# yester31/Monocular_Depth_Estimation_TRT

Measured on AMD Instinct MI355X. Metric: depth FPS (images/s) at 518x518 fp16, DA-V2 ViT-S, MI355X, higher is better.
Workload: dtype fp16; 1 GPU; Depth Anything V2 vits 518x518 metric head, forward, batch 48 per GPU, inputs resident in HBM, hipGraph replay; encoder=vits, batch_per_gpu=48, global_batch=48, parallelism=replica x1 (batch shards, no collectives), weights=synthetic seeded (seed 1234), fan-in scaled, physical_gpus=1

## Files before the change

### include/mde.h

```cpp
#ifndef MDE_H_
#define MDE_H_

#include <stddef.h>
#include <stdint.h>

#ifdef __cplusplus
extern "C" {
#endif

#define MDE_ABI_VERSION 11

typedef enum {
  MDE_OK = 0,
  MDE_ERR_ARG = 1,
  MDE_ERR_FILE = 2,
  MDE_ERR_FORMAT = 3,
  MDE_ERR_HIP = 4,
  MDE_ERR_NAME = 5,
  MDE_ERR_SHAPE = 6,
  MDE_ERR_STATE = 7
} mde_status;

typedef enum { MDE_FLOAT32 = 0, MDE_FLOAT16 = 1, MDE_UINT8 = 5 } mde_dtype;

typedef struct mde_engine mde_engine;
typedef struct mde_context mde_context;

typedef struct {
  char name[64];
  int32_t dtype;
  int32_t is_input;
  int32_t rank;
  int64_t dims[8];
} mde_io_desc;

typedef struct {
  char encoder[16];
  int32_t embed_dim, depth, num_heads, mlp_hidden, patch;
  int32_t img_h, img_w, features, head_hidden, metric;
  int32_t out_channels[4], taps[4];
  float max_depth, ln_eps;
  int32_t max_batch_hint;
  int64_t weight_bytes;
  int32_t input_format;
  int32_t family;
} mde_engine_info;

typedef void (*mde_layer_cb)(const char* layer_name, float ms, void* user);

int mde_version(void);
const char* mde_last_error(void);
int mde_tuning_set(const char* name, int value);
int mde_tuning_get(const char* name, int* value);
int mde_debug_last_gemm_route(char* buf, size_t n);

int mde_engine_load(const char* packed_path, int device, mde_engine** out);
int mde_engine_load_memory(const void* data, size_t nbytes, int device, mde_engine** out);
int mde_engine_destroy(mde_engine* eng);
int mde_engine_get_info(const mde_engine* eng, mde_engine_info* out);
int mde_engine_num_io(const mde_engine* eng, int* n);
int mde_engine_io_desc(const mde_engine* eng, int index, mde_io_desc* out);
int mde_engine_profile_shape(const mde_engine* eng, const char* name, int which, int64_t* dims, int* rank);

int mde_context_create(mde_engine* eng, int max_batch, mde_context** out);
int mde_context_destroy(mde_context* ctx);
int mde_context_set_tensor_address(mde_context* ctx, const char* name, void* device_ptr);
int mde_context_set_input_shape(mde_context* ctx, const char* name, const int64_t* dims, int rank);
int mde_context_get_tensor_shape(const mde_context* ctx, const char* name, int64_t* dims, int* rank);
int mde_context_enqueue(mde_context* ctx, void* stream);
int mde_context_set_graph_mode(mde_context* ctx, int enable);
int mde_context_set_profiler(mde_context* ctx, mde_layer_cb cb, void* user);
int mde_context_workspace_bytes(const mde_context* ctx, size_t* bytes);

int mde_rt_device_count(int* n);
int mde_rt_set_device(int device);
int mde_rt_device_name(int device, char* buf, int buflen);
int mde_rt_malloc(void** ptr, size_t bytes);
int mde_rt_free(void* ptr);
int mde_rt_malloc_host(void** ptr, size_t bytes);
int mde_rt_free_host(void* ptr);
int mde_rt_memcpy_htod_async(void* dst, const void* src, size_t bytes, void* stream);
int mde_rt_memcpy_dtoh_async(void* dst, const void* src, size_t bytes, void* stream);
int mde_rt_memcpy_dtod_async(void* dst, const void* src, size_t bytes, void* stream);
int mde_rt_memset_async(void* dst, int value, size_t bytes, void* stream);
int mde_rt_stream_create(void** stream);
int mde_rt_stream_destroy(void* stream);
int mde_rt_stream_synchronize(void* stream);
int mde_rt_device_synchronize(void);
int mde_rt_event_create(void** event);
int mde_rt_event_destroy(void* event);
int mde_rt_event_record(void* event, void* stream);
int mde_rt_event_elapsed_ms(float* ms, void* start, void* end);

int mde_op_layernorm_f16(const void* x_f16, void* y_f16, const float* gamma, const float* beta, int rows, int dim,
                         float eps, int tokens, int skip_cls, void* stream);
int mde_op_layernorm(const float* x, void* y_f16, const float* gamma, const float* beta, int rows, int dim,
                     float eps, int tokens, int skip_cls, void* stream);
int mde_op_linear(const void* a_f16, int lda, const void* w_f16, int ldw, int m, int n, int k,
                  const float* bias, int act, void* out_f16, int ldo, void* stream);
int mde_op_linear_residual(const void* a_f16, int lda, const void* w_f16, int ldw, int m, int n, int k,
                           const float* bias, const float* layer_scale, float* x32, int ldx, void* stream);
int mde_op_qkv(const void* a_f16, const void* w_f16, int ldw, const float* bias, int batch, int tokens,
               int heads, int tokens_pad, float q_scale, void* q_f16, void* k_f16, void* vt_f16, void* stream);
int mde_op_linear_residual_f16(const void* a_f16, int lda, const void* w_f16, int ldw, int m, int n, int k,
                               const float* bias, const float* layer_scale, void* xh_f16, int ldx, float* ln_partials,
                               void* stream);
int mde_op_linear_lnfold(const void* x_f16, const float* ln_partials, float eps, const void* wg_f16, int ldw,
                         const float* c1, const float* c2, int m, int n, int k, int act, void* out_f16, int ldo,
                         void* stream);
int mde_op_qkv_lnfold(const void* x_f16, const float* ln_partials, float eps, const void* wg_f16, int ldw,
                      const float* c1, const float* c2, int batch, int tokens, int heads, int tokens_pad,
                      float q_scale, void* q_f16, void* k_f16, void* vt_f16, void* stream);
int mde_op_attention(const void* q_f16, const void* k_f16, const void* vt_f16, void* o_f16, int batch, int heads,
                     int tokens, int tokens_pad, int ldo, void* stream);
int mde_op_attention_ws(const void* q_f16, const void* k_f16, const void* vt_f16, void* o_f16, int batch, int heads,
                        int tokens, int tokens_pad, int ldo, void* ws, size_t ws_bytes, void* stream);
size_t mde_op_attention_ws_bytes(int batch, int heads, int tokens);
int mde_op_attention_cfg(const void* q_f16, const void* k_f16, const void* vt_f16, void* o_f16, int batch, int heads,
                         int tokens, int tokens_pad, int ldo, const char* cfg, void* ws, size_t ws_bytes,
                         void* stream);
int mde_op_linear32(const float* a, int lda, const float* w, int ldw, int m, int n, int k, const float* bias, int act,
                    float* out, int ldo, void* stream);
int mde_op_linear_residual32(const float* a, int lda, const float* w, int ldw, int m, int n, int k,
                             const float* bias, const float* layer_scale, float* x32, int ldx, void* stream);
int mde_op_qkv32(const float* a, const float* w, int ldw, const float* bias, int batch, int tokens, int heads,
                 int tokens_pad, float q_scale, float* q, float* k, float* v, void* stream);
int mde_op_attention32(const float* q, const float* k, const float* v, float* o, int batch, int heads, int tokens,
                       int tokens_pad, int ldo, void* stream);
int mde_op_conv3x3_32(const float* in, int batch, int h, int w, int cin, const float* wt, int ldw, int cout,
                      int stride, int relu_in, const float* bias, int act, const float* res0, const float* res1,
                      float* out, void* stream);
int mde_op_conv_transpose32(const float* in, int batch, int h, int w, int cin, const float* wt, int ldw, int cout,
                            int stride, const float* bias, float* out, void* stream);
int mde_op_resize32(const float* in, int batch, int h, int w, int c, int oh, int ow, float* out, void* stream);
int mde_op_patch_embed(const float* img, int batch, int h, int w, const void* w_f16, int ldw, const float* bias,
                       const float* pos_patch, const float* cls_pos, int dim, void* patch_scratch_f16,
                       float* x32, void* stream);
int mde_op_conv3x3(const void* in_f16, int batch, int h, int w, int cin, const void* w_f16, int ldw, int cout,
                   int stride, int relu_in, const float* bias, int act, const void* res0_f16,
                   const void* res1_f16, void* out_f16, void* stream);
int mde_op_conv3x3_ws(const void* in_f16, int batch, int h, int w, int cin, const void* w_f16, int ldw, int cout,
                      int stride, int relu_in, const float* bias, int act, const void* res0_f16,
                      const void* res1_f16, void* out_f16, float* ws, size_t ws_floats, int* slices, void* stream);
int mde_op_linear_ws(const void* a_f16, int lda, const void* w_f16, int ldw, int m, int n, int k, const float* bias,
                     int act, void* out_f16, int ldo, float* ws, size_t ws_floats, int* slices, void* stream);
int mde_op_conv3x3_up(const void* in_f16, int batch, int sh, int sw, int cin, int uh, int uw, const void* w_f16,
                      int ldw, int cout, const float* bias, int act, void* out_f16, void* stream);
int mde_op_conv_transpose(const void* in_f16, int batch, int h, int w, int cin, const void* w_f16, int ldw,
                          int cout, int stride, const float* bias, void* out_f16, void* stream);
int mde_op_resize_bilinear(const void* in_f16, int batch, int ih, int iw, int c, int oh, int ow, void* out_f16,
                           void* stream);
int mde_op_depth_head(const void* in_f16, int batch, int sh, int sw, int cin, int uh, int uw, const void* w_f16,
                      int ldw, const float* bias, const float* w2, float b2, int metric, float max_depth,
                      float* out_f32, void* stream);
int mde_op_linear_res(const void* a_f16, int lda, const void* w_f16, int ldw, int m, int n, int k, const float* bias,
                      int act, const void* res0_f16, int res0_rows, int res0_relu, const void* res1_f16,
                      void* out_f16, int ldo, float* ws, size_t ws_floats, int* slices, int* tile_cnt,
                      int tile_cnt_cap, size_t slot_floats, void* stream);
int mde_op_conv3x3_res(const void* in_f16, int batch, int h, int w, int cin, const void* w_f16, int ldw, int cout,
                       int stride, int relu_in, const float* bias, int act, const void* res0_f16, int res0_relu,
                       const void* res1_f16, const void* res1_up_f16, int res1_uh, int res1_uw, void* out_f16,
                       float* ws, size_t ws_floats, int* slices, int* tile_cnt, int tile_cnt_cap, size_t slot_floats,
                       void* stream);
int mde_op_linear_lnfold_tok(const void* x_f16, const float* ln_partials, float eps, const void* wg_f16, int ldw,
                             const float* c1, const float* c2, int seqs, int tokens, int n, int k, int act,
                             void* out_f16, int ldo, void* stream);
int mde_op_depth_head_pe(const void* in_f16, int batch, int sh, int sw, int cin, int uh, int uw, const void* w_f16,
                         int ldw, const float* bias, const float* w2, float b2, int metric, float max_depth,
                         const void* hpe_f16, int hpe_pix, float* out_f32, void* stream);
int mde_op_conv_transpose_ld(const void* in_f16, int batch, int h, int w, int cin, const void* w_f16, int ldw,
                             int cout, int stride, const float* bias, void* out_f16, int ldo, void* stream);
int mde_op_linear_residual_split(const void* a_f16, int lda, const void* w_f16, int ldw, int m, int n, int k,
                                 const float* bias, const float* layer_scale, float* x32, void* xh_f16, int ldx,
                                 float* ln_partials, int splitk, float* ws, size_t ws_floats, int* tile_cnt,
                                 int tile_cnt_cap, size_t slot_floats, void* stream);
int mde_op_patch_prep_u8(const unsigned char* img_u8, int batch, int h, int w, float scale, const float* mean3,
                         const float* std3, void* patches_f16, void* stream);
int mde_op_depth_postprocess(const float* depth, int batch, int ih, int iw, float* out, int oh, int ow, float lo,
                             float hi, void* stream);
int mde_op_resize_u8(const unsigned char* src, int batch, int sh, int sw, int pitch, int swap_rb,
                     unsigned char* dst_u8, int oh, int ow, void* stream);
int mde_op_resize_u8_norm(const unsigned char* src, int batch, int sh, int sw, int pitch, int swap_rb,
                          const float* lut3x256, float* dst_f32_nchw, int oh, int ow, void* stream);
int mde_op_dp_preprocess(const unsigned char* src, int batch, int sh, int sw, int pitch, int swap_rb,
                         const float* lut256, float* dst_f32_nchw, int oh, int ow, void* stream);
int mde_op_dp_postprocess(const float* inv, int batch, int ih, int iw, const float* fov_deg, float f_px,
                          float* f_px_out, float* depth, int oh, int ow, void* stream);
size_t mde_op_point_cloud_ws_bytes(int batch, int h, int w, int step);
int mde_op_point_cloud(const float* depth, int batch, int h, int w, int step, const unsigned char* photo, int pitch,
                       int swap_rb, const float* f_px_dev, float fx, float fy, float cx, float cy, int compact,
                       float z_lo, float z_hi, void* records, size_t records_bytes, int* counts, void* ws,
                       size_t ws_bytes, void* stream);
#define MDE_DEPTH_EVAL_TILE 1024
size_t mde_op_depth_eval_ws_bytes(int batch, int h, int w);
int mde_op_depth_eval(const float* pred, const float* gt, const unsigned char* mask, int batch, int h, int w,
                      int policy, int pred_is_inverse, int fit_finite_only, float max_depth, double* out, void* ws,
                      size_t ws_bytes, void* stream);
int mde_op_dp_pyramid_patches(const float* img, int batch, int size, void* patches_f16, void* stream);
int mde_op_merge_tokens(const float* x32, int batch, int tokens, int dim, int n, int g, int pad, int base,
                        const float* gamma, const float* beta, float eps, void* out_f16, void* stream);
int mde_op_qk_norm_rope(void* q_f16, void* k_f16, const float* q_gamma, const float* q_beta, const float* k_gamma,
                        const float* k_beta, int bh, int tokens, int tokens_pad, int frame_tokens, int npre,
                        int grid_w, const float* rope_cos, const float* rope_sin, float q_scale, float eps,
                        void* stream);
int mde_op_tap_concat_ln(const float* xa, const float* xb, int nseq, int tokens, int npre, int dim,
                         const float* gamma, const float* beta, float eps, void* out_f16, void* stream);
#ifdef __cplusplus
}
#endif

#endif
```

### monocular_depth_estimation_trt_amd/_lib.py

```python

from __future__ import annotations

import contextlib
import ctypes as C
import os
import threading

HERE = os.path.dirname(os.path.abspath(__file__))
LIB_PATH = os.path.join(HERE, "libmde_hip.so")


def use_library(path: str) -> None:
    global LIB_PATH
    if _lib is not None and os.path.abspath(path) != os.path.abspath(LIB_PATH):
        raise RuntimeError(f"libmde_hip already loaded from {LIB_PATH}")
    LIB_PATH = path

c_void_p, c_int, c_float, c_size_t, c_char_p = C.c_void_p, C.c_int, C.c_float, C.c_size_t, C.c_char_p
c_int64 = C.c_int64
P = C.POINTER

MDE_OK = 0
STATUS = {1: "MDE_ERR_ARG", 2: "MDE_ERR_FILE", 3: "MDE_ERR_FORMAT", 4: "MDE_ERR_HIP", 5: "MDE_ERR_NAME",
          6: "MDE_ERR_SHAPE", 7: "MDE_ERR_STATE"}


class mde_io_desc(C.Structure):
    _fields_ = [("name", C.c_char * 64), ("dtype", C.c_int32), ("is_input", C.c_int32),
                ("rank", C.c_int32), ("dims", C.c_int64 * 8)]


class mde_engine_info(C.Structure):
    _fields_ = [("encoder", C.c_char * 16),
                ("embed_dim", C.c_int32), ("depth", C.c_int32), ("num_heads", C.c_int32),
                ("mlp_hidden", C.c_int32), ("patch", C.c_int32),
                ("img_h", C.c_int32), ("img_w", C.c_int32), ("features", C.c_int32),
                ("head_hidden", C.c_int32), ("metric", C.c_int32),
                ("out_channels", C.c_int32 * 4), ("taps", C.c_int32 * 4),
                ("max_depth", C.c_float), ("ln_eps", C.c_float),
                ("max_batch_hint", C.c_int32), ("weight_bytes", C.c_int64),
                ("input_format", C.c_int32), ("family", C.c_int32)]


LAYER_CB = C.CFUNCTYPE(None, c_char_p, c_float, c_void_p)

PROTOTYPES = {
    "mde_version": [],
    "mde_last_error": [],
    "mde_tuning_set": [c_char_p, c_int],
    "mde_tuning_get": [c_char_p, P(c_int)],
    "mde_debug_last_gemm_route": [c_char_p, c_size_t],
    "mde_engine_load": [c_char_p, c_int, P(c_void_p)],
    "mde_engine_load_memory": [c_void_p, c_size_t, c_int, P(c_void_p)],
    "mde_engine_destroy": [c_void_p],
    "mde_engine_get_info": [c_void_p, P(mde_engine_info)],
    "mde_engine_num_io": [c_void_p, P(c_int)],
    "mde_engine_io_desc": [c_void_p, c_int, P(mde_io_desc)],
    "mde_engine_profile_shape": [c_void_p, c_char_p, c_int, P(c_int64), P(c_int)],
    "mde_context_create": [c_void_p, c_int, P(c_void_p)],
    "mde_context_destroy": [c_void_p],
    "mde_context_set_tensor_address": [c_void_p, c_char_p, c_void_p],
    "mde_context_set_input_shape": [c_void_p, c_char_p, P(c_int64), c_int],
    "mde_context_get_tensor_shape": [c_void_p, c_char_p, P(c_int64), P(c_int)],
    "mde_context_enqueue": [c_void_p, c_void_p],
    "mde_context_set_graph_mode": [c_void_p, c_int],
    "mde_context_set_profiler": [c_void_p, LAYER_CB, c_void_p],
    "mde_context_workspace_bytes": [c_void_p, P(c_size_t)],
    "mde_rt_device_count": [P(c_int)],
    "mde_rt_set_device": [c_int],
    "mde_rt_device_name": [c_int, c_char_p, c_int],
    "mde_rt_malloc": [P(c_void_p), c_size_t],
    "mde_rt_free": [c_void_p],
    "mde_rt_malloc_host": [P(c_void_p), c_size_t],
    "mde_rt_free_host": [c_void_p],
    "mde_rt_memcpy_htod_async": [c_void_p, c_void_p, c_size_t, c_void_p],
    "mde_rt_memcpy_dtoh_async": [c_void_p, c_void_p, c_size_t, c_void_p],
    "mde_rt_memcpy_dtod_async": [c_void_p, c_void_p, c_size_t, c_void_p],
    "mde_rt_memset_async": [c_void_p, c_int, c_size_t, c_void_p],
    "mde_rt_stream_create": [P(c_void_p)],
    "mde_rt_stream_destroy": [c_void_p],
    "mde_rt_stream_synchronize": [c_void_p],
    "mde_rt_device_synchronize": [],
    "mde_rt_event_create": [P(c_void_p)],
    "mde_rt_event_destroy": [c_void_p],
    "mde_rt_event_record": [c_void_p, c_void_p],
    "mde_rt_event_elapsed_ms": [P(c_float), c_void_p, c_void_p],
    "mde_op_layernorm": [c_void_p, c_void_p, c_void_p, c_void_p, c_int, c_int, c_float, c_int, c_int, c_void_p],
    "mde_op_layernorm_f16": [c_void_p, c_void_p, c_void_p, c_void_p, c_int, c_int, c_float, c_int, c_int, c_void_p],
    "mde_op_linear": [c_void_p, c_int, c_void_p, c_int, c_int, c_int, c_int, c_void_p, c_int, c_void_p, c_int,
                      c_void_p],
    "mde_op_linear_residual": [c_void_p, c_int, c_void_p, c_int, c_int, c_int, c_int, c_void_p, c_void_p,
                               c_void_p, c_int, c_void_p],
    "mde_op_qkv": [c_void_p, c_void_p, c_int, c_void_p, c_int, c_int, c_int, c_int, c_float, c_void_p, c_void_p,
                   c_void_p, c_void_p],
    "mde_op_linear_residual_f16": [c_void_p, c_int, c_void_p, c_int, c_int, c_int, c_int, c_void_p, c_void_p,
                                   c_void_p, c_int, c_void_p, c_void_p],
    "mde_op_linear_lnfold": [c_void_p, c_void_p, c_float, c_void_p, c_int, c_void_p, c_void_p, c_int, c_int, c_int,
                             c_int, c_void_p, c_int, c_void_p],
    "mde_op_qkv_lnfold": [c_void_p, c_void_p, c_float, c_void_p, c_int, c_void_p, c_void_p, c_int, c_int, c_int,
                          c_int, c_float, c_void_p, c_void_p, c_void_p, c_void_p],
    "mde_op_attention_ws": [c_void_p, c_void_p, c_void_p, c_void_p, c_int, c_int, c_int, c_int, c_int, c_void_p,
                            c_size_t, c_void_p],
    "mde_op_attention_ws_bytes": [c_int, c_int, c_int],
    "mde_op_attention_cfg": [c_void_p, c_void_p, c_void_p, c_void_p, c_int, c_int, c_int, c_int, c_int, c_char_p,
                             c_void_p, c_size_t, c_void_p],
    "mde_op_attention": [c_void_p, c_void_p, c_void_p, c_void_p, c_int, c_int, c_int, c_int, c_int, c_void_p],
    "mde_op_linear32": [c_void_p, c_int, c_void_p, c_int, c_int, c_int, c_int, c_void_p, c_int, c_void_p, c_int,
                        c_void_p],
    "mde_op_linear_residual32": [c_void_p, c_int, c_void_p, c_int, c_int, c_int, c_int, c_void_p, c_void_p,
                                 c_void_p, c_int, c_void_p],
    "mde_op_qkv32": [c_void_p, c_void_p, c_int, c_void_p, c_int, c_int, c_int, c_int, c_float, c_void_p, c_void_p,
                     c_void_p, c_void_p],
    "mde_op_attention32": [c_void_p, c_void_p, c_void_p, c_void_p, c_int, c_int, c_int, c_int, c_int, c_void_p],
    "mde_op_conv3x3_32": [c_void_p, c_int, c_int, c_int, c_int, c_void_p, c_int, c_int, c_int, c_int, c_void_p,
                          c_int, c_void_p, c_void_p, c_void_p, c_void_p],
    "mde_op_conv_transpose32": [c_void_p, c_int, c_int, c_int, c_int, c_void_p, c_int, c_int, c_int, c_void_p,
                                c_void_p, c_void_p],
    "mde_op_resize32": [c_void_p, c_int, c_int, c_int, c_int, c_int, c_int, c_void_p, c_void_p],
    "mde_op_patch_embed": [c_void_p, c_int, c_int, c_int, c_void_p, c_int, c_void_p, c_void_p, c_void_p, c_int,
                           c_void_p, c_void_p, c_void_p],
    "mde_op_conv3x3": [c_void_p, c_int, c_int, c_int, c_int, c_void_p, c_int, c_int, c_int, c_int, c_void_p,
                       c_int, c_void_p, c_void_p, c_void_p, c_void_p],
    "mde_op_conv3x3_ws": [c_void_p, c_int, c_int, c_int, c_int, c_void_p, c_int, c_int, c_int, c_int, c_void_p,
                          c_int, c_void_p, c_void_p, c_void_p, c_void_p, c_size_t, P(c_int), c_void_p],
    "mde_op_linear_ws": [c_void_p, c_int, c_void_p, c_int, c_int, c_int, c_int, c_void_p, c_int, c_void_p, c_int,
                         c_void_p, c_size_t, P(c_int), c_void_p],
    "mde_op_conv3x3_up": [c_void_p, c_int, c_int, c_int, c_int, c_int, c_int, c_void_p, c_int, c_int, c_void_p,
                          c_int, c_void_p, c_void_p],
    "mde_op_conv_transpose": [c_void_p, c_int, c_int, c_int, c_int, c_void_p, c_int, c_int, c_int, c_void_p,
                              c_void_p, c_void_p],
    "mde_op_resize_bilinear": [c_void_p, c_int, c_int, c_int, c_int, c_int, c_int, c_void_p, c_void_p],
    "mde_op_depth_head": [c_void_p, c_int, c_int, c_int, c_int, c_int, c_int, c_void_p, c_int, c_void_p,
                          c_void_p, c_float, c_int, c_float, c_void_p, c_void_p],
    "mde_op_linear_res": [c_void_p, c_int, c_void_p, c_int, c_int, c_int, c_int, c_void_p, c_int, c_void_p, c_int,
                          c_int, c_void_p, c_void_p, c_int, c_void_p, c_size_t, P(c_int), c_void_p, c_int, c_size_t,
                          c_void_p],
    "mde_op_conv3x3_res": [c_void_p, c_int, c_int, c_int, c_int, c_void_p, c_int, c_int, c_int, c_int, c_void_p,
                           c_int, c_void_p, c_int, c_void_p, c_void_p, c_int, c_int, c_void_p, c_void_p, c_size_t,
                           P(c_int), c_void_p, c_int, c_size_t, c_void_p],
    "mde_op_linear_lnfold_tok": [c_void_p, c_void_p, c_float, c_void_p, c_int, c_void_p, c_void_p, c_int, c_int,
                                 c_int, c_int, c_int, c_void_p, c_int, c_void_p],
    "mde_op_depth_head_pe": [c_void_p, c_int, c_int, c_int, c_int, c_int, c_int, c_void_p, c_int, c_void_p,
                             c_void_p, c_float, c_int, c_float, c_void_p, c_int, c_void_p, c_void_p],
    "mde_op_conv_transpose_ld": [c_void_p, c_int, c_int, c_int, c_int, c_void_p, c_int, c_int, c_int, c_void_p,
                                 c_void_p, c_int, c_void_p],
    "mde_op_linear_residual_split": [c_void_p, c_int, c_void_p, c_int, c_int, c_int, c_int, c_void_p, c_void_p,
                                     c_void_p, c_void_p, c_int, c_void_p, c_int, c_void_p, c_size_t, c_void_p,
                                     c_int, c_size_t, c_void_p],
    "mde_op_patch_prep_u8": [c_void_p, c_int, c_int, c_int, c_float, c_void_p, c_void_p, c_void_p, c_void_p],
    "mde_op_dp_pyramid_patches": [c_void_p, c_int, c_int, c_void_p, c_void_p],
    "mde_op_merge_tokens": [c_void_p, c_int, c_int, c_int, c_int, c_int, c_int, c_int, c_void_p, c_void_p, c_float,
                            c_void_p, c_void_p],
    "mde_op_depth_postprocess": [c_void_p, c_int, c_int, c_int, c_void_p, c_int, c_int, c_float, c_float,
                                 c_void_p],
    "mde_op_resize_u8": [c_void_p, c_int, c_int, c_int, c_int, c_int, c_void_p, c_int, c_int, c_void_p],
    "mde_op_resize_u8_norm": [c_void_p, c_int, c_int, c_int, c_int, c_int, c_void_p, c_void_p, c_int, c_int,
                              c_void_p],
    "mde_op_dp_preprocess": [c_void_p, c_int, c_int, c_int, c_int, c_int, c_void_p, c_void_p, c_int, c_int,
                             c_void_p],
    "mde_op_dp_postprocess": [c_void_p, c_int, c_int, c_int, c_void_p, c_float, c_void_p, c_void_p, c_int, c_int,
                              c_void_p],
    "mde_op_point_cloud_ws_bytes": [c_int, c_int, c_int, c_int],
    "mde_op_point_cloud": [c_void_p, c_int, c_int, c_int, c_int, c_void_p, c_int, c_int, c_void_p, c_float, c_float,
                           c_float, c_float, c_int, c_float, c_float, c_void_p, c_size_t, c_void_p, c_void_p,
                           c_size_t, c_void_p],
    "mde_op_depth_eval_ws_bytes": [c_int, c_int, c_int],
    "mde_op_depth_eval": [c_void_p, c_void_p, c_void_p, c_int, c_int, c_int, c_int, c_int, c_int, c_float, c_void_p,
                          c_void_p, c_size_t, c_void_p],
    "mde_op_qk_norm_rope": [c_void_p] * 6 + [c_int] * 6 + [c_void_p, c_void_p, c_float, c_float, c_void_p],
    "mde_op_tap_concat_ln": [c_void_p, c_void_p, c_int, c_int, c_int, c_int, c_void_p, c_void_p, c_float, c_void_p,
                             c_void_p],
}
_RESTYPE = {"mde_last_error": c_char_p, "mde_op_attention_ws_bytes": c_size_t,
             "mde_op_point_cloud_ws_bytes": c_size_t, "mde_op_depth_eval_ws_bytes": c_size_t}

_lib = None
_lock = threading.Lock()


class MDEError(RuntimeError):

    def __init__(self, fn: str, code: int, msg: str):
        self.code = code
        super().__init__(f"{fn} failed ({STATUS.get(code, code)}): {msg}")


def hip_runtimes() -> list:
    paths = set()
    try:
        with open("/proc/self/maps") as f:
            for line in f:
                parts = line.split(None, 5)
                if len(parts) == 6 and "libamdhip64" in os.path.basename(parts[5].strip()):
                    paths.add(os.path.realpath(parts[5].strip()))
    except OSError:
        return []
    return sorted(paths)


def check_single_runtime() -> None:
    rts = hip_runtimes()
    if len(rts) > 1:
        raise ImportError(
            "two HIP runtimes are loaded in this process (" + ", ".join(rts) + "): libmde_hip.so was loaded "
            "before PyTorch's bundled HIP runtime.  Import torch (and call torch.cuda.is_available()) before "
            "loading libmde_hip.so, or do not load torch in a process that uses libmde_hip.so directly.")


def lib() -> C.CDLL:
    global _lib
    if _lib is not None:
        return _lib
    with _lock:
        if _lib is None:
            if not os.path.exists(LIB_PATH):
                raise ImportError(
                    f"libmde_hip.so not found at {LIB_PATH}. Build it first: "
                    f"python -c 'import __graft_entry__ as g; g.build()' (or "
                    f"python -m monocular_depth_estimation_trt_amd._build). There is no CPU fallback.")
            try:
                import torch
                torch.cuda.is_available()
            except ImportError:
                pass
            L = C.CDLL(LIB_PATH)
            check_single_runtime()
            for name, args in PROTOTYPES.items():
                f = getattr(L, name)
                f.argtypes = args
                f.restype = _RESTYPE.get(name, c_int)
            _lib = L
    return _lib


def last_error() -> str:
    m = lib().mde_last_error()
    return m.decode(errors="replace") if m else ""


def call(name: str, *args) -> None:
    rc = getattr(lib(), name)(*args)
    if rc != MDE_OK:
        raise MDEError(name, rc, last_error())


TUNING = ("splitk", "lnfold", "conv_narrow", "upconv", "gemm256", "deep64", "w8small", "conv_persist", "panel",
          "panel32", "narrow_resid", "attn16", "splitk_fused", "attn_tail", "resize_fold")
TUNING_DEFAULT = {"panel32": 0, "splitk_fused": 0, "attn_tail": 2}


def get_tuning(name: str) -> int:
    v = c_int()
    call("mde_tuning_get", name.encode(), C.byref(v))
    return v.value


def set_tuning(name: str, value: int) -> None:
    rc = lib().mde_tuning_set(name.encode(), int(value))
    if rc != MDE_OK:
        raise ValueError(f"mde_tuning_set({name!r}, {value}) failed ({STATUS.get(rc, rc)}): "
                         f"known switches {TUNING}")


@contextlib.contextmanager
def tuning(**switches):
    old = {k: get_tuning(k) for k in switches}
    try:
        for k, v in switches.items():
            set_tuning(k, v)
        yield
    finally:
        for k, v in old.items():
            set_tuning(k, v)


def last_gemm_route() -> dict:
    buf = C.create_string_buffer(256)
    call("mde_debug_last_gemm_route", buf, len(buf))
    fields = dict(f.split("=", 1) for f in buf.value.decode().split())
    return {k: v if k == "kind" else int(v) for k, v in fields.items()}


def exported_symbols():
    return list(PROTOTYPES)
```

### monocular_depth_estimation_trt_amd/csrc/conv.hip

```cpp
#include <cstdlib>
#include <type_traits>

#include "mde_device.h"
#include "mde_ops.h"
#include "tile_epilogue.h"
#include "tuning.h"

#ifndef MDE_EPI_LDS
#define MDE_EPI_LDS 1
#endif
#ifndef MDE_UP_BLEND_F16
#define MDE_UP_BLEND_F16 1
#endif
#ifndef MDE_CONVP_RELU_PASS
#define MDE_CONVP_RELU_PASS 1
#endif
#ifndef MDE_CONV_BRES
#define MDE_CONV_BRES 2
#endif

namespace mde {

namespace {

__device__ __attribute__((aligned(64))) f16 g_zero_conv[64];

MDE_DEV void glds16c(const void* src, void* lds_wave_base) {
  __builtin_amdgcn_global_load_lds(src, lds_wave_base, 16, 0, 0);
}
MDE_DEV void wait_vmc() { asm volatile("s_waitcnt vmcnt(0)" ::: "memory"); }
MDE_DEV void glds16_asm(const void* src, unsigned lds_dst) {
  unsigned keep;
  asm volatile("s_mov_b32 %0, m0\n\ts_mov_b32 m0, %2\n\ts_nop 0\n\tglobal_load_lds_dwordx4 %1, off\n\ts_mov_b32 m0, %0"
               : "=&s"(keep)
               : "v"(src), "s"(lds_dst)
               : "memory");
}
MDE_DEV void lds_sync() {
  asm volatile("s_waitcnt lgkmcnt(0)" ::: "memory");
  __builtin_amdgcn_s_barrier();
  asm volatile("" ::: "memory");
}

typedef f16 f16x2c __attribute__((ext_vector_type(2)));

template <int J>
MDE_DEV f16x2c lerp2(const f16x8& a, const f16x8& b, f16x2c w2) {
  const f16x2c a2 = __builtin_shufflevector(a, a, 2 * J, 2 * J + 1);
  const f16x2c b2 = __builtin_shufflevector(b, b, 2 * J, 2 * J + 1);
  unsigned dd;
  asm("v_pk_add_f16 %0, %1, %2 neg_lo:[0,1] neg_hi:[0,1]"
      : "=v"(dd)
      : "v"(__builtin_bit_cast(unsigned, b2)), "v"(__builtin_bit_cast(unsigned, a2)));
  return a2 + __builtin_bit_cast(f16x2c, dd) * w2;
}

MDE_DEV f16x8 lerp8(const f16x8& a, const f16x8& b, f16 w) {
  const f16x2c w2 = {w, w};
  const f16x2c r0 = lerp2<0>(a, b, w2), r1 = lerp2<1>(a, b, w2), r2 = lerp2<2>(a, b, w2), r3 = lerp2<3>(a, b, w2);
  return __builtin_shufflevector(__builtin_shufflevector(r0, r1, 0, 1, 2, 3), __builtin_shufflevector(r2, r3, 0, 1, 2, 3),
                                 0, 1, 2, 3, 4, 5, 6, 7);
}

template <int CK>
MDE_DEV int cpch(int pix, int lc) {
  if constexpr (CK == 64) return lc ^ (pix & 7);
  else return lc ^ ((pix >> 1) & 3);
}

constexpr int TH = 8, TW = 16;

template <int BN, int WM, int WN, int CK, int S, bool UP, int EM, bool BRES = false, int TY = TH>
__global__ void __launch_bounds__(WM * WN * 64)
    __attribute__((amdgpu_waves_per_eu((WM * WN == 4 || WM * WN == 8) && !UP ? 4 : 1))) conv3_kernel(const GemmParams p) {
  constexpr int NW = WM * WN, NT = NW * 64;
  constexpr int BM = TY * TW;
  constexpr int TM = BM / (WM * 16), TN = BN / (WN * 16);
  static_assert(TM * WM * 16 == BM && TN * WN * 16 == BN, "tile");
  static_assert(EM != E_HEAD || (BN == 32 && WN == 1), "head epilogue");
  constexpr int ROWB = CK * 2, CH = CK / 8, RWP = 64 / CH;
  constexpr int PH = (TY - 1) * S + 3, PW = (TW - 1) * S + 3, PHW = PH * PW;
  constexpr int PINS = (PHW + RWP - 1) / RWP;
  constexpr int PPAD = PINS * RWP;
  constexpr int PATCH = PPAD * ROWB;
  constexpr int BSTAGE = BN * ROWB;
  constexpr int BINS = BN / RWP;
  static_assert(BINS * RWP == BN, "B tile rows");
  constexpr int MAIN = PATCH + (BRES ? 9 : 2) * BSTAGE, EPI = MDE_EPI_LDS ? BM * BN * 4 : 0;
  __shared__ __attribute__((aligned(16))) char smem[MAIN > EPI ? MAIN : EPI];
  char* sP = smem;
  char* sB0 = smem + PATCH;

  const int tid = threadIdx.x, lane = tid & 63;
  const int wave = __builtin_amdgcn_readfirstlane(tid >> 6);
  const int wm = wave / WN, wn = wave - (wave / WN) * WN;

  const int Ho = p.oh, Wo = p.ow;
  const int tiles_x = (Wo + TW - 1) / TW, tiles_y = (Ho + TY - 1) / TY;
  const int ntn = (p.N + BN - 1) / BN;
  int bid = xcd_remap(blockIdx.x, gridDim.x);
  const int tn = bid % ntn;
  bid /= ntn;
  const int tx = bid % tiles_x;
  bid /= tiles_x;
  const int ty = bid % tiles_y;
  const int b = bid / tiles_y;
  const int n0 = tn * BN;
  const int IH = UP ? p.uh : p.ch, IW = UP ? p.uw : p.cw;
  const int iy0 = ty * TY * S - 1, ix0 = tx * TW * S - 1;
  const f16* img = reinterpret_cast<const f16*>(p.A) + (size_t)b * p.ch * p.cw * p.cc;

  const int lrow = lane / CH;
  const int lch = cpch<CK>(lrow, lane % CH);
  const f16* wbase = reinterpret_cast<const f16*>(p.W) + (size_t)(n0 + lrow) * p.ldw + lch * 8;

  float usy = 0.f, usx = 0.f;
  if constexpr (UP) {
    usy = ac_scale(p.ch, p.uh);
    usx = ac_scale(p.cw, p.uw);
  }

  auto load_patch = [&](int chunk) {
    const int cbase = chunk * CK;
    if constexpr (!UP) {
      for (int q = wave; q < PINS; q += NW) {
        const int pp = q * RWP + lrow;
        const int py = pp / PW, px = pp - (pp / PW) * PW;
        const int iy = iy0 + py, ix = ix0 + px;
        const bool ok = pp < PHW && iy >= 0 && iy < IH && ix >= 0 && ix < IW;
        const f16* src = ok ? img + ((size_t)iy * p.cw + ix) * p.cc + cbase + lch * 8 : g_zero_conv;
        glds16c(src, sP + q * RWP * ROWB);
      }
    } else {
      const unsigned rowstride = (unsigned)p.cw * (unsigned)p.cc;
      constexpr int CG = CH < 4 ? CH : 4, NG = CH / CG;
      for (int it = tid; it < PHW * NG; it += NT) {
        const int pp = it / NG, g0 = (it - (it / NG) * NG) * CG;
        const int py = pp / PW, px = pp - (pp / PW) * PW;
        const int iy = iy0 + py, ix = ix0 + px;
        const bool inside = iy >= 0 && iy < IH && ix >= 0 && ix < IW;
        int y0 = 0, y1 = 0, x0 = 0, x1 = 0;
        float ly0 = 0.f, ly1 = 0.f, lx0 = 0.f, lx1 = 0.f;
        if (inside) {
          ac_index(usy, iy, p.ch, y0, y1, ly0, ly1);
          ac_index(usx, ix, p.cw, x0, x1, lx0, lx1);
        }
        const unsigned r0 = (unsigned)y0 * rowstride + (unsigned)cbase, r1 = (unsigned)y1 * rowstride + (unsigned)cbase;
        const unsigned o0 = (unsigned)x0 * (unsigned)p.cc, o1 = (unsigned)x1 * (unsigned)p.cc;
#pragma unroll
        for (int q = 0; q < CG; ++q) {
          const int lc = g0 + q;
          f16x8 v = zero8();
          if (inside) {
            const f16x8 a = *reinterpret_cast<const f16x8*>(img + (r0 + o0 + lc * 8));
            const f16x8 bq = *reinterpret_cast<const f16x8*>(img + (r0 + o1 + lc * 8));
            const f16x8 c = *reinterpret_cast<const f16x8*>(img + (r1 + o0 + lc * 8));
            const f16x8 d = *reinterpret_cast<const f16x8*>(img + (r1 + o1 + lc * 8));
#if MDE_UP_BLEND_F16
            v = lerp8(lerp8(a, bq, (f16)lx1), lerp8(c, d, (f16)lx1), (f16)ly1);
#else
#pragma unroll
            for (int j = 0; j < 8; ++j)
              v[j] = (f16)(ly0 * (lx0 * (float)a[j] + lx1 * (float)bq[j]) + ly1 * (lx0 * (float)c[j] + lx1 * (float)d[j]));
#endif
          }
          if (p.relu_in) v = relu8(v);
          *reinterpret_cast<f16x8*>(sP + pp * ROWB + cpch<CK>(pp, lc) * 16) = v;
        }
// ... 5 lines not shown
    const int k0 = t * p.cc + chunk * CK;
    char* dst = sB0 + buf * BSTAGE;
    for (int q = wave; q < BINS; q += NW) glds16c(wbase + (size_t)q * RWP * p.ldw + k0, dst + q * RWP * ROWB);
  };

  auto relu_patch = [&] {
    if constexpr (!UP) {
      if (p.relu_in) {
        for (int c = tid; c < PATCH / 16; c += NT) {
          f16x8* q = reinterpret_cast<f16x8*>(sP + c * 16);
          *q = relu8(*q);
        }
      }
    }
  };
  f32x4 acc[TM][TN];
#pragma unroll
  for (int i = 0; i < TM; ++i)
#pragma unroll
    for (int j = 0; j < TN; ++j) acc[i][j] = f32x4{0.f, 0.f, 0.f, 0.f};

  const int nchunk = p.cc / CK;
  const int nsteps = 9 * nchunk;
  if constexpr (BRES) {
    load_patch(0);
#pragma unroll
    for (int t = 0; t < 9; ++t) load_b(t, t);
    wait_vmc();
    __syncthreads();
    if (!UP && p.relu_in) {
      relu_patch();
      __syncthreads();
    }
#pragma unroll
    for (int t = 0; t < 9; ++t) {
      const char* sB = sB0 + t * BSTAGE;
      const int ky = t / 3, kx = t - (t / 3) * 3;
#pragma unroll
      for (int s = 0; s < CK / 32; ++s) {
        const int lc = 4 * s + (lane >> 4);
        f16x8 fa[TM], fb[TN];
#pragma unroll
        for (int i = 0; i < TM; ++i) {
          const int pp = ((wm * TM + i) * S + ky) * PW + (lane & 15) * S + kx;
          fa[i] = *reinterpret_cast<const f16x8*>(sP + pp * ROWB + cpch<CK>(pp, lc) * 16);
        }
#pragma unroll
        for (int j = 0; j < TN; ++j) {
          const int r = wn * TN * 16 + j * 16 + (lane & 15);
          fb[j] = *reinterpret_cast<const f16x8*>(sB + r * ROWB + cpch<CK>(r, lc) * 16);
        }
#pragma unroll
        for (int i = 0; i < TM; ++i)
#pragma unroll
          for (int j = 0; j < TN; ++j) acc[i][j] = mfma16x16x32(fb[j], fa[i], acc[i][j]);
      }
    }
    __syncthreads();
  }
  for (int chunk = 0; chunk < (BRES ? 0 : nchunk); ++chunk) {
    if (chunk > 0) __syncthreads();
    load_patch(chunk);
    const int step0 = chunk * 9;
    load_b(step0, step0 & 1);
    wait_vmc();
    __syncthreads();
    if (!UP && p.relu_in) {
      relu_patch();
      __syncthreads();
    }
    for (int t = 0; t < 9; ++t) {
      const int step = step0 + t;
      if (t + 1 < 9) load_b(step + 1, (step + 1) & 1);
      const char* sB = sB0 + (step & 1) * BSTAGE;
      const int ky = t / 3, kx = t - (t / 3) * 3;
#pragma unroll
      for (int s = 0; s < CK / 32; ++s) {
        const int lc = 4 * s + (lane >> 4);
        f16x8 fa[TM], fb[TN];
#pragma unroll
        for (int i = 0; i < TM; ++i) {
          const int py = wm * TM + i;
          const int pp = (py * S + ky) * PW + (lane & 15) * S + kx;
          fa[i] = *reinterpret_cast<const f16x8*>(sP + pp * ROWB + cpch<CK>(pp, lc) * 16);
        }
#pragma unroll
        for (int j = 0; j < TN; ++j) {
          const int r = wn * TN * 16 + j * 16 + (lane & 15);
          fb[j] = *reinterpret_cast<const f16x8*>(sB + r * ROWB + cpch<CK>(r, lc) * 16);
        }
#pragma unroll
        for (int i = 0; i < TM; ++i)
#pragma unroll
          for (int j = 0; j < TN; ++j) acc[i][j] = mfma16x16x32(fb[j], fa[i], acc[i][j]);
      }
      wait_vmc();
      __syncthreads();
    }
  }
  (void)nsteps;

  int mrow[TM];
#pragma unroll
  for (int i = 0; i < TM; ++i) {
    const int oy = ty * TY + wm * TM + i, ox = tx * TW + (lane & 15);
    mrow[i] = (oy < Ho && ox < Wo) ? ((b * Ho + oy) * Wo + ox) : -1;
  }
#if MDE_EPI_LDS
  if (!store_tile_lds<EM, TM, TN, 0, true>(
          p, acc,
          [&](int row) {
            const int oy = ty * TY + wm * TM + (row >> 4), ox = tx * TW + (row & 15);
            return (oy < Ho && ox < Wo) ? ((b * Ho + oy) * Wo + ox) : -1;
          },
          n0 + wn * TN * 16, lane, smem + wave * (TM * 16) * (TN * 16) * 4))
#endif
    store_tile<EM, TM, TN, true>(p, acc, mrow, n0 + wn * TN * 16 + (lane >> 4) * 4, lane);
}

template <int BN, int WM, int WN, int CK, int S, bool UP, int EM, int TY = TH>
hipError_t run_conv(const GemmParams& p, hipStream_t st) {
  const long long blocks =
      (long long)p.cb * ((p.oh + TY - 1) / TY) * ((p.ow + TW - 1) / TW) * ((p.N + BN - 1) / BN);
  if (blocks <= 0) return hipSuccess;
  constexpr bool BRES_OK = BN == 32 && (CK == 32 ? MDE_CONV_BRES >= 1 : MDE_CONV_BRES >= 2);
  if (BRES_OK && p.cc == CK)
    hipLaunchKernelGGL((conv3_kernel<BN, WM, WN, CK, S, UP, EM, BRES_OK, TY>), dim3((unsigned)blocks),
                       dim3(WM * WN * 64), 0, st, p);
  else
    hipLaunchKernelGGL((conv3_kernel<BN, WM, WN, CK, S, UP, EM, false, TY>), dim3((unsigned)blocks),
                       dim3(WM * WN * 64), 0, st, p);
  return hipGetLastError();
}

bool conv_narrow_tiles() { return knob(KNOB_CONV_NARROW) != 0; }

template <int CK, int S, bool UP, int EM>
hipError_t conv_tiles(const GemmParams& p, hipStream_t st) {
  if constexpr (EM == E_HEAD) {
    return run_conv<32, 4, 1, CK, S, UP, EM>(p, st);
  } else {
    if (p.N <= 32) return run_conv<32, 4, 1, CK, S, UP, EM>(p, st);
    if (p.N <= 64) {
      const long long wg64 = (long long)p.cb * ((p.oh + TH - 1) / TH) * ((p.ow + TW - 1) / TW);
      if (!UP && p.N == 64 && conv_narrow_tiles() && wg64 < 256) return run_conv<32, 4, 1, CK, S, UP, EM>(p, st);
      return run_conv<64, 4, 1, CK, S, UP, EM>(p, st);
    }
    const long long wg128 = (long long)p.cb * ((p.oh + TH - 1) / TH) * ((p.ow + TW - 1) / TW) * ((p.N + 127) / 128);
    if (!UP && conv_narrow_tiles() && wg128 < 512) return run_conv<64, 4, 1, CK, S, UP, EM>(p, st);
    return run_conv<128, 2, 2, CK, S, UP, EM>(p, st);
  }
}

template <int TYP, int MODE>
__global__ void __launch_bounds__(TYP * 32) __attribute__((amdgpu_waves_per_eu(1)))
conv64p_kernel(const GemmParams p) {
  constexpr int NW = TYP / 2, NT = NW * 64, TM = 2, TN = 4;
  constexpr int ROWB = 128, RWP = 8;
  constexpr int PH = TYP + 2, PW = TW + 2, PHW = PH * PW;
  constexpr int PINS = (PHW + RWP - 1) / RWP;
  constexpr int PATCH = PINS * RWP * ROWB;
  constexpr int WOFF = 2 * PATCH;
  constexpr int WB = 9 * 64 * ROWB;
  constexpr int EPIW = 16 * 64 * 4;
  constexpr int NRES = MODE == 3 ? 0 : MODE;
  constexpr bool F16STAGE = MODE == 0 || MODE == 3;
  static_assert(NW * EPIW <= PATCH, "epilogue staging fits the consumed patch buffer");
  static_assert(PATCH + ((TM + 1) * PW + 2) * ROWB < 65536 && 7 * 8192 + 3 * 2048 < 65536, "ds_read immediate offsets");
  static_assert(PW % 8 == 2, "pixel row stride = 2 mod 8 (the swizzle table below)");
  __shared__ __attribute__((aligned(16))) char smem[2 * PATCH + WB];

  const int tid = threadIdx.x, lane = tid & 63;
  const int wave = __builtin_amdgcn_readfirstlane(tid >> 6);
  const int Ho = p.oh, Wo = p.ow;
  const int tiles_x = (Wo + TW - 1) / TW, tiles_y = (Ho + TYP - 1) / TYP;
  const int ntiles = p.cb * tiles_x * tiles_y;
  const int x8 = blockIdx.x & 7, g8 = (int)gridDim.x >> 3;
  int t = (int)((long long)x8 * ntiles / 8) + (int)(blockIdx.x >> 3);
  const int tend = (int)((long long)(x8 + 1) * ntiles / 8);
  if (t >= tend) return;

  const int lrow = lane >> 3;
  const int lch = cpch<64>(lrow, lane & 7);
  const size_t imgsz = (size_t)p.ch * p.cw * 64;

  for (int q = wave; q < 9 * 64 / RWP; q += NW) {
    const int tap = q >> 3, n = (q & 7) * RWP + lrow;
    glds16c(reinterpret_cast<const f16*>(p.W) + (size_t)n * p.ldw + tap * 64 + lch * 8, smem + WOFF + q * RWP * ROWB);
  }
  auto load_patch = [&](int tt, int buf, auto asm_tag) {
    const int tx = tt % tiles_x, r = tt / tiles_x;
    const int ty = r % tiles_y, b = r / tiles_y;
    const int iy0 = ty * TYP - 1, ix0 = tx * TW - 1;
    const f16* img = reinterpret_cast<const f16*>(p.A) + (size_t)b * imgsz;
    char* dst = smem + buf * PATCH;
    for (int q = wave; q < PINS; q += NW) {
      const int pp = q * RWP + lrow;
      const int py = pp / PW, px = pp - (pp / PW) * PW;
      const int iy = iy0 + py, ix = ix0 + px;
      const bool ok = pp < PHW && iy >= 0 && iy < p.ch && ix >= 0 && ix < p.cw;
      const f16* src = ok ? img + ((size_t)iy * p.cw + ix) * 64 + lch * 8 : g_zero_conv;
      if constexpr (decltype(asm_tag)::value)
        glds16_asm(src, __builtin_amdgcn_readfirstlane((unsigned)(uintptr_t)(dst + q * RWP * ROWB)));
      else
        glds16c(src, dst + q * RWP * ROWB);
    }
  };
  auto relu_patch = [&](int buf) {
    for (int c = tid; c < PATCH / 16; c += NT) {
      f16x8* q = reinterpret_cast<f16x8*>(smem + buf * PATCH + c * 16);
      *q = relu8(*q);
    }
  };

  int pa[8][2], wa[2], wa8[2];
  {
    const int u = 2 * wave * TM + (lane & 15);
    const int rowbase = ((wave * TM) * PW + (lane & 15)) * ROWB;
#pragma unroll
    for (int e = 0; e < 8; ++e)
#pragma unroll
      for (int s2 = 0; s2 < 2; ++s2) pa[e][s2] = rowbase + ((((4 * s2 + (lane >> 4)) ^ ((u + e) & 7))) << 4);
#pragma unroll
    for (int s2 = 0; s2 < 2; ++s2) {
      wa[s2] = WOFF + (lane & 15) * ROWB + (((4 * s2 + (lane >> 4)) ^ (lane & 7)) << 4);
      wa8[s2] = wa[s2] + 8 * 64 * ROWB;
    }
  }

  const int rr = lane >> 3, c8 = lane & 7;
  float4 bias[TN];
#pragma unroll
  for (int j = 0; j < TN; ++j)
    bias[j] = p.bias ? *reinterpret_cast<const float4*>(p.bias + j * 16 + (lane >> 4) * 4) : float4{0.f, 0.f, 0.f, 0.f};

  load_patch(t, 0, std::false_type{});
  wait_vmc();
  __syncthreads();
  if constexpr (MODE == 0) {
    if (MDE_CONVP_RELU_PASS) relu_patch(0);
    lds_sync();
  }

  auto step = [&](auto buf_tag) -> bool {
    constexpr int BUF = decltype(buf_tag)::value;
    const int tn = t + g8;
    if (tn < tend) load_patch(tn, BUF ^ 1, std::true_type{});

    const int tx = t % tiles_x, r = t / tiles_x;
    const int ty = r % tiles_y, b = r / tiles_y;
    int mo[4];
#pragma unroll
    for (int it = 0; it < 4; ++it) {
      const int row = it * 8 + rr;
      const int oy = ty * TYP + wave * TM + (row >> 4), ox = tx * TW + (row & 15);
      mo[it] = (oy < Ho && ox < Wo) ? ((b * Ho + oy) * Wo + ox) : -1;
    }
    f16x8 res[NRES > 0 ? NRES : 1][4];
    if constexpr (NRES > 0) {
#pragma unroll
      for (int it = 0; it < 4; ++it) {
        const size_t o = (size_t)(mo[it] < 0 ? 0 : mo[it]) * p.ldo + c8 * 8;
        res[0][it] = *reinterpret_cast<const f16x8*>(reinterpret_cast<const f16*>(p.res0) + o);
        if constexpr (NRES > 1) res[1][it] = *reinterpret_cast<const f16x8*>(reinterpret_cast<const f16*>(p.res1) + o);
      }
    }
    __builtin_amdgcn_sched_barrier(0);

    f32x4 acc[TM][TN];
#pragma unroll
    for (int i = 0; i < TM; ++i)
#pragma unroll
      for (int j = 0; j < TN; ++j) acc[i][j] = f32x4{0.f, 0.f, 0.f, 0.f};
#pragma unroll
    for (int tap = 0; tap < 9; ++tap) {
      const int ky = tap / 3, kx = tap - (tap / 3) * 3;
#pragma unroll
      for (int s2 = 0; s2 < 2; ++s2) {
        f16x8 fa[TM], fb[TN];
#pragma unroll
        for (int i = 0; i < TM; ++i) {
          const int e = 2 * (i + ky) + kx;
          fa[i] = *reinterpret_cast<const f16x8*>(smem + pa[e & 7][s2] + (BUF * PATCH + ((i + ky) * PW + kx) * ROWB));
          if constexpr (MODE == 0 && !MDE_CONVP_RELU_PASS) fa[i] = relu8(fa[i]);
        }
#pragma unroll
        for (int j = 0; j < TN; ++j)
          fb[j] = *reinterpret_cast<const f16x8*>(smem + (tap < 8 ? wa[s2] + tap * 64 * ROWB : wa8[s2]) + j * 16 * ROWB);
#pragma unroll
        for (int i = 0; i < TM; ++i)
#pragma unroll
          for (int j = 0; j < TN; ++j) acc[i][j] = mfma16x16x32(fb[j], fa[i], acc[i][j]);
      }
    }
    __builtin_amdgcn_sched_barrier(0);
    wait_vmc();
    lds_sync();
    if constexpr (MODE == 0) {
      if (MDE_CONVP_RELU_PASS && tn < tend) relu_patch(BUF ^ 1);
    }

    char* stage = smem + BUF * PATCH + wave * EPIW;
    f16* const out = reinterpret_cast<f16*>(p.out16);
    if constexpr (F16STAGE) {
#pragma unroll
      for (int i = 0; i < TM; ++i)
#pragma unroll
        for (int j = 0; j < TN; ++j) {
          const float4 bn = bias[j];
          const float v0 = acc[i][j][0] + bn.x, v1 = acc[i][j][1] + bn.y;
          const float v2 = acc[i][j][2] + bn.z, v3 = acc[i][j][3] + bn.w;
          const f16x4 h = MODE == 0 ? f16x4{(f16)(v0 > 0.f ? v0 : 0.f), (f16)(v1 > 0.f ? v1 : 0.f),
                                            (f16)(v2 > 0.f ? v2 : 0.f), (f16)(v3 > 0.f ? v3 : 0.f)}
                                    : f16x4{(f16)v0, (f16)v1, (f16)v2, (f16)v3};
          const int row = i * 16 + (lane & 15), q = j * 4 + (lane >> 4);
          *reinterpret_cast<f16x4*>(stage + row * 128 + ((((q >> 1) ^ (row & 7)) << 4) | ((q & 1) << 3))) = h;
        }
      asm volatile("s_waitcnt lgkmcnt(0)" ::: "memory");
      __builtin_amdgcn_wave_barrier();
#pragma unroll
      for (int it = 0; it < 4; ++it) {
        const int row = it * 8 + rr;
        const f16x8 h = *reinterpret_cast<const f16x8*>(stage + row * 128 + ((c8 ^ (row & 7)) << 4));
        if (mo[it] >= 0) *reinterpret_cast<f16x8*>(out + (size_t)mo[it] * p.ldo + c8 * 8) = h;
      }
    } else {
#pragma unroll
      for (int i = 0; i < TM; ++i) {
        if (i > 0) __builtin_amdgcn_wave_barrier();
#pragma unroll
        for (int j = 0; j < TN; ++j) {
          const float4 bn = bias[j];
          const f32x4 v = {acc[i][j][0] + bn.x, acc[i][j][1] + bn.y, acc[i][j][2] + bn.z, acc[i][j][3] + bn.w};
          const int row = lane & 15, q = j * 4 + (lane >> 4);
          *reinterpret_cast<f32x4*>(stage + row * 256 + ((q ^ (row & 7)) << 4)) = v;
        }
        asm volatile("s_waitcnt lgkmcnt(0)" ::: "memory");
        __builtin_amdgcn_wave_barrier();
#pragma unroll
        for (int h2 = 0; h2 < 2; ++h2) {
          const int it = i * 2 + h2, row = h2 * 8 + rr;
          const f32x4 a = *reinterpret_cast<const f32x4*>(stage + row * 256 + (((2 * c8) ^ (row & 7)) << 4));
          const f32x4 bb = *reinterpret_cast<const f32x4*>(stage + row * 256 + (((2 * c8 + 1) ^ (row & 7)) << 4));
          float v[8] = {a[0], a[1], a[2], a[3], bb[0], bb[1], bb[2], bb[3]};
          const f16x8 r0 = res[0][it];
          if (p.res0_relu) {
#pragma unroll
            for (int e = 0; e < 8; ++e) v[e] += fmaxf((float)r0[e], 0.f);
          } else {
#pragma unroll
            for (int e = 0; e < 8; ++e) v[e] += (float)r0[e];
          }
          if constexpr (NRES > 1) {
            const f16x8 r1 = res[NRES - 1][it];
#pragma unroll
            for (int e = 0; e < 8; ++e) v[e] += (float)r1[e];
          }
          f16x8 h;
#pragma unroll
          for (int e = 0; e < 8; ++e) h[e] = (f16)v[e];
          if (mo[it] >= 0) *reinterpret_cast<f16x8*>(out + (size_t)mo[it] * p.ldo + c8 * 8) = h;
        }
      }
    }
    if (tn >= tend) return true;
    lds_sync();
    t = tn;
    return false;
  };
  for (;;) {
    if (step(std::integral_constant<int, 0>{})) break;
    if (step(std::integral_constant<int, 1>{})) break;
  }
}

int conv64p_mode(const GemmParams& p) {
  const int mode = knob(KNOB_CONV_PERSIST);
  if (!mode || p.amode != A_CONV3 || p.emode != E_STORE || p.stride != 1 || p.N != 64 || p.cc != 64 ||
      p.ch != p.oh || p.cw != p.ow || p.ldo < 64 || (p.ldo & 7) || p.res0_rows > 0)
    return -1;
  const bool r1 = p.res1 || p.res1_up;
  int m;
  if (p.relu_in && p.act == ACT_RELU && !p.res0 && !r1) m = 0;
  else if (!p.relu_in && p.act == ACT_NONE && !p.res0 && !r1) m = 3;
  else if (!p.relu_in && p.act == ACT_NONE && p.res0) m = r1 ? 2 : 1;
  else return -1;
  const int typ = mode == 2 ? 8 : 16;
  const long long tiles = (long long)p.cb * ((p.oh + typ - 1) / typ) * ((p.ow + TW - 1) / TW);
  if (tiles < 4 * 256 || tiles >= (1ll << 31)) return -1;
  return m;
}

bool conv64p_launch(const GemmParams& p, hipStream_t st, hipError_t& err) {
  const int m = conv64p_mode(p);
  if (m < 0) return false;
  const int typ = knob(KNOB_CONV_PERSIST) == 2 ? 8 : 16;
  const dim3 grid(256), block(typ * 32);
  if (typ == 16) {
    if (m == 0) hipLaunchKernelGGL((conv64p_kernel<16, 0>), grid, block, 0, st, p);
    else if (m == 1) hipLaunchKernelGGL((conv64p_kernel<16, 1>), grid, block, 0, st, p);
    else if (m == 2) hipLaunchKernelGGL((conv64p_kernel<16, 2>), grid, block, 0, st, p);
    else hipLaunchKernelGGL((conv64p_kernel<16, 3>), grid, block, 0, st, p);
  } else {
    if (m == 0) hipLaunchKernelGGL((conv64p_kernel<8, 0>), grid, block, 0, st, p);
    else if (m == 1) hipLaunchKernelGGL((conv64p_kernel<8, 1>), grid, block, 0, st, p);
    else if (m == 2) hipLaunchKernelGGL((conv64p_kernel<8, 2>), grid, block, 0, st, p);
    else hipLaunchKernelGGL((conv64p_kernel<8, 3>), grid, block, 0, st, p);
  }
  err = hipGetLastError();
  return true;
}

constexpr int UTH = 16, UTW = 16;
constexpr int UPH = UTH + 2, UPW = UTW + 2;
constexpr int USR = 12;
constexpr int UPATCH = UPH * UPW * 64, UHBUF = USR * UPW * 64;
MDE_DEV int uoff(int row, int col, int lc) { return row * (UPW * 64) + col * 64 + ((lc ^ ((col >> 1) & 3)) << 4); }

template <int NCH, int EM, bool PERSIST>
__global__ void __launch_bounds__(512) __attribute__((amdgpu_waves_per_eu(NCH == 1 ? 6 : 4)))
upconv_kernel(const GemmParams p) {
  static_assert(EM == E_STORE || EM == E_HEAD, "upconv epilogues");
  constexpr int NT = 512, TM = 2, TN = 2;
  constexpr bool SW = NCH > 1;
  constexpr int WROWS = 9 * (SW ? 1 : NCH) * 32;
  __shared__ __attribute__((aligned(16))) char smem[UPATCH + UHBUF + WROWS * 64 + 256];
  char* const sP = smem;
  char* const sH = smem + UPATCH;
  char* const sW = sH + UHBUF;
  float* const sBias = reinterpret_cast<float*>(sW + WROWS * 64);

  const int tid = threadIdx.x, lane = tid & 63;
  const int wave = __builtin_amdgcn_readfirstlane(tid >> 6);
  const int Ho = p.oh, Wo = p.ow;
  const int tiles_x = (Wo + UTW - 1) / UTW, tiles_y = (Ho + UTH - 1) / UTH;
  const int ntiles = p.cb * tiles_x * tiles_y;
  int t, tstep, tend;
  if constexpr (PERSIST) {
    const int x = blockIdx.x & 7, g8 = (int)gridDim.x >> 3;
    t = (int)((long long)x * ntiles / 8) + (int)(blockIdx.x >> 3);
    tend = (int)((long long)(x + 1) * ntiles / 8);
    tstep = g8;
  } else {
    t = xcd_remap(blockIdx.x, gridDim.x);
    tend = t + 1;
    tstep = 1;
  }
  if (t >= tend) return;
  const float usy = ac_scale(p.ch, p.uh), usx = ac_scale(p.cw, p.uw);
  const unsigned rowstride = (unsigned)p.cw * (unsigned)p.cc;

  if constexpr (!SW) {
    const int lrow = lane >> 2, lch = cpch<32>(lrow, lane & 3);
    for (int q = wave; q < WROWS / 16; q += 8) {
      const int tc = q >> 1, n = (q & 1) * 16 + lrow;
      const int tp = tc / NCH, c = tc - (tc / NCH) * NCH;
      glds16c(reinterpret_cast<const f16*>(p.W) + (size_t)n * p.ldw + tp * p.cc + c * 32 + lch * 8, sW + q * 16 * 64);
    }
  }

  if (tid < 64) {
    const float* src = tid < 32 ? p.bias : p.w2;
    sBias[tid] = (src && (tid < 32 || EM == E_HEAD)) ? src[tid & 31] : 0.f;
  }

  struct Geo {
    int b, ty, tx, iy0, ix0, sy0, nsr;
  };
  auto geo = [&](int tt) {
    Geo g;
    g.tx = tt % tiles_x;
    const int r = tt / tiles_x;
    g.ty = r % tiles_y;
    g.b = r / tiles_y;
    g.iy0 = g.ty * UTH - 1;
    g.ix0 = g.tx * UTW - 1;
    int a0, a1, b0, b1;
    float l0, l1;
    ac_index(usy, g.iy0 < 0 ? 0 : g.iy0, p.ch, a0, a1, l0, l1);
    const int last = g.iy0 + UPH - 1 < p.uh - 1 ? g.iy0 + UPH - 1 : p.uh - 1;
    ac_index(usy, last, p.ch, b0, b1, l0, l1);
    g.sy0 = a0;
    g.nsr = b1 - a0 + 1 < USR ? b1 - a0 + 1 : USR;
    return g;
  };

  constexpr int CL = UPW * 4, RG = NT / CL;
  static_assert(RG * 2 >= USR && RG * 3 >= UPH, "row groups cover the H rows (2 each) and the patch rows (3)");
  constexpr int HI = 2;
  f16x8 ha[HI], hb[HI];
  f16 hw = (f16)0.0f;
  bool hs[HI], hin = false;
  auto h_issue = [&](const Geo& g, int c, int tid) {
    const f16* img = reinterpret_cast<const f16*>(p.A) + (size_t)g.b * p.ch * p.cw * p.cc;
    const int cl = tid % CL, rg = tid / CL;
    const int lc = cl & 3, col = cl >> 2;
    const int ix = g.ix0 + col;
    hin = rg < RG && ix >= 0 && ix < p.uw;
    int x0 = 0, x1 = 0;
    float lx0, lx1 = 0.f;
    if (hin) ac_index(usx, ix, p.cw, x0, x1, lx0, lx1);
    hw = (f16)lx1;
    const unsigned o0 = (unsigned)x0 * (unsigned)p.cc + (unsigned)(c * 32 + lc * 8);
    const unsigned o1 = (unsigned)x1 * (unsigned)p.cc + (unsigned)(c * 32 + lc * 8);
#pragma unroll
    for (int k = 0; k < HI; ++k) {
      const int sr = rg + k * RG;
      hs[k] = rg < RG && sr < g.nsr;
      const unsigned r = (unsigned)(g.sy0 + (hin && hs[k] ? sr : 0)) * rowstride;
      ha[k] = *reinterpret_cast<const f16x8*>(img + (r + o0));
      hb[k] = *reinterpret_cast<const f16x8*>(img + (r + o1));
    }
  };
  auto h_commit = [&](int tid) {
    const int cl = tid % CL, rg = tid / CL;
    const int lc = cl & 3, col = cl >> 2;
#pragma unroll
    for (int k = 0; k < HI; ++k) {
      if (hs[k]) {
        *reinterpret_cast<f16x8*>(sH + uoff(rg + k * RG, col, lc)) =
            hin ? lerp8(ha[k], hb[k], hw) : zero8();
      }
    }
  };

  f32x4 acc[TM][TN];
#pragma unroll
  for (int i = 0; i < TM; ++i)
#pragma unroll
    for (int j = 0; j < TN; ++j) acc[i][j] = f32x4{0.f, 0.f, 0.f, 0.f};

  Geo g = geo(t);
  int c = 0;
  h_issue(g, 0, tid);
  for (;;) {
    int vt;
    asm volatile("v_mov_b32 %0, %1" : "=v"(vt) : "v"(tid));
    const int vl = vt & 63;
    wait_vmc();
    h_commit(vt);
    __syncthreads();
    if constexpr (SW) {
      const int lrow = vl >> 2, lch = cpch<32>(lrow, vl & 3);
      for (int q = wave; q < WROWS / 16; q += 8) {
        const int n = (q & 1) * 16 + lrow;
        glds16_asm(reinterpret_cast<const f16*>(p.W) + (size_t)n * p.ldw + (q >> 1) * p.cc + c * 32 + lch * 8,
                   __builtin_amdgcn_readfirstlane((unsigned)(uintptr_t)(sW + q * 16 * 64)));
      }
    }
    int tn = t, cn = c + 1;
    if (cn == NCH) {
      cn = 0;
      tn = t + tstep;
    }
    Geo gn = g;
    if (tn < tend) {
      gn = geo(tn);
      h_issue(gn, cn, vt);
    }
    {
// ... 31 lines not shown
#pragma unroll
        for (int i = 0; i < TM; ++i) {
          fa[i] = *reinterpret_cast<const f16x8*>(sP + uoff(wave * TM + i + ky, (lane & 15) + kx, lc));
        }
#pragma unroll
        for (int j = 0; j < TN; ++j) {
          const int r = j * 16 + (lane & 15);
          fb[j] = *reinterpret_cast<const f16x8*>(sW + ((SW ? tp : tp * NCH + c) * 32 + r) * 64 + cpch<32>(r, lc) * 16);
        }
#pragma unroll
        for (int i = 0; i < TM; ++i)
#pragma unroll
          for (int j = 0; j < TN; ++j) acc[i][j] = mfma16x16x32(fb[j], fa[i], acc[i][j]);
        if constexpr (PERSIST) __builtin_amdgcn_sched_barrier(0);
      }
    }
    if (c == NCH - 1) {
#pragma unroll
      for (int i = 0; i < TM; ++i) {
        const int oy = g.ty * UTH + wave * TM + i, ox = g.tx * UTW + (vl & 15);
        const int m = (oy < Ho && ox < Wo) ? ((g.b * Ho + oy) * Wo + ox) : -1;
        if constexpr (EM == E_HEAD) {
          auto hidden = [&](auto pe_tag) {
            constexpr bool PE = decltype(pe_tag)::value;
            float part = 0.f;
#pragma unroll
            for (int j = 0; j < TN; ++j) {
              const int n0 = j * 16 + (vl >> 4) * 4;
              const float4 bn = *reinterpret_cast<const float4*>(sBias + n0);
              const float4 w2 = *reinterpret_cast<const float4*>(sBias + 32 + n0);
              float h0 = acc[i][j][0] + bn.x, h1 = acc[i][j][1] + bn.y;
              float h2 = acc[i][j][2] + bn.z, h3 = acc[i][j][3] + bn.w;
              if constexpr (PE) {
                float pv[4] = {0.f, 0.f, 0.f, 0.f};
                if (m >= 0) {
                  const f16x4 q = *reinterpret_cast<const f16x4*>(reinterpret_cast<const f16*>(p.hpe) +
                                                                  (size_t)(m % p.hpe_pix) * 32 + n0);
#pragma unroll
                  for (int r = 0; r < 4; ++r) pv[r] = (float)q[r];
                }
                h0 += pv[0];
                h1 += pv[1];
                h2 += pv[2];
                h3 += pv[3];
              }
              part = fmaf(h0 > 0.f ? h0 : 0.f, w2.x, part);
              part = fmaf(h1 > 0.f ? h1 : 0.f, w2.y, part);
              part = fmaf(h2 > 0.f ? h2 : 0.f, w2.z, part);
              part = fmaf(h3 > 0.f ? h3 : 0.f, w2.w, part);
            }
            return part;
          };
          float part = p.hpe ? hidden(std::true_type{}) : hidden(std::false_type{});
          part += __shfl_xor(part, 16, 64);
          part += __shfl_xor(part, 32, 64);
          if ((vl >> 4) == 0 && m >= 0) {
            const float z = part + p.b2;
            p.out32[m] = p.head_metric == 2 ? __expf(z)
                         : p.head_metric ? p.max_depth / (1.f + __expf(-z)) : (z > 0.f ? z : 0.f);
          }
        } else {
          if (m < 0) continue;
#pragma unroll
          for (int j = 0; j < TN; ++j) {
            const int n0 = j * 16 + (vl >> 4) * 4;
            const float4 bn = *reinterpret_cast<const float4*>(sBias + n0);
            float v[4] = {acc[i][j][0] + bn.x, acc[i][j][1] + bn.y, acc[i][j][2] + bn.z, acc[i][j][3] + bn.w};
            if (p.act == ACT_RELU) {
#pragma unroll
              for (int r = 0; r < 4; ++r) v[r] = v[r] > 0.f ? v[r] : 0.f;
            } else if (p.act == ACT_GELU) {
#pragma unroll
              for (int r = 0; r < 4; ++r) v[r] = gelu_erf(v[r]);
            }
            const f16x4 h = {(f16)v[0], (f16)v[1], (f16)v[2], (f16)v[3]};
            *reinterpret_cast<f16x4*>(reinterpret_cast<f16*>(p.out16) + (size_t)m * p.ldo + n0) = h;
          }
        }
      }
#pragma unroll
      for (int i = 0; i < TM; ++i)
#pragma unroll
        for (int j = 0; j < TN; ++j) acc[i][j] = f32x4{0.f, 0.f, 0.f, 0.f};
    }
    if (tn >= tend) break;
    t = tn;
    c = cn;
    g = gn;
  }
}

bool upconv_enabled() { return knob(KNOB_UPCONV) != 0; }

bool upconv_eligible(const GemmParams& p) {
#pragma clang fp contract(off)
  if (p.amode != A_CONV3_UP || p.N != 32 || p.stride != 1 || (p.cc & 31) || p.cc > 128) return false;
  if (p.emode != E_STORE && p.emode != E_HEAD) return false;
  if (p.emode == E_STORE && ((p.ldo & 3) || p.res0 || p.res1)) return false;
  if (p.uh < 2 || p.uw < 1 || p.ch < 1 || p.cw < 1 || p.oh != p.uh) return false;
  if (!upconv_enabled()) return false;
  const float sy = (float)(p.ch - 1) / (float)(p.uh - 1);
  const int tiles_y = (p.oh + UTH - 1) / UTH;
  for (int ty = 0; ty < tiles_y; ++ty) {
    const int iy0 = ty * UTH - 1;
    const int first = iy0 < 0 ? 0 : iy0;
    const int last = iy0 + UPH - 1 < p.uh - 1 ? iy0 + UPH - 1 : p.uh - 1;
    const int a0 = (int)(sy * (float)first);
    const int l0 = (int)(sy * (float)last);
    const int b1 = l0 + (l0 < p.ch - 1 ? 1 : 0);
    if (b1 - a0 + 1 > USR) return false;
  }
  return true;
}

template <int NCH>
int upconv_grid() {
  constexpr int lds = UPATCH + UHBUF + 9 * (NCH > 1 ? 1 : NCH) * 32 * 64;
  const int per_cu = 163840 / lds < 4 ? 163840 / lds : 4;
  return 256 * (per_cu > 0 ? per_cu : 1);
}
template <int NCH, int EM>
void launch_upconv_n(const GemmParams& p, long long tiles, hipStream_t st) {
  const int grid = upconv_grid<NCH>();
  if (tiles > grid)
    hipLaunchKernelGGL((upconv_kernel<NCH, EM, true>), dim3((unsigned)grid), dim3(512), 0, st, p);
  else
    hipLaunchKernelGGL((upconv_kernel<NCH, EM, false>), dim3((unsigned)tiles), dim3(512), 0, st, p);
}

template <int EM>
hipError_t launch_upconv(const GemmParams& p, hipStream_t st) {
  const long long tiles = (long long)p.cb * ((p.oh + UTH - 1) / UTH) * ((p.ow + UTW - 1) / UTW);
  if (tiles <= 0) return hipSuccess;
  if (tiles >= (1ll << 31)) return hipErrorInvalidValue;
  switch (p.cc / 32) {
    case 1: launch_upconv_n<1, EM>(p, tiles, st); break;
    case 2: launch_upconv_n<2, EM>(p, tiles, st); break;
    case 3: launch_upconv_n<3, EM>(p, tiles, st); break;
    case 4: launch_upconv_n<4, EM>(p, tiles, st); break;
    default: return hipErrorInvalidValue;
  }
  return hipGetLastError();
}

}

bool conv_direct_supported(const GemmParams& p) {
  if (p.cc % 32) return false;
  if (p.amode == A_CONV3_UP) return p.stride == 1;
  return p.stride == 1 || p.stride == 2;
}

bool conv3_takes_res1_up(const GemmParams& p) {
  return knob(KNOB_RESIZE_FOLD) && p.amode == A_CONV3 && p.emode == E_STORE && p.stride == 1 && p.N <= 64 &&
         conv_direct_supported(p) && conv64p_mode(p) < 0 && p.ldo == p.N && (p.N & 7) == 0 && p.res1_uh > 0 &&
         p.res1_uw > 0;
}

hipError_t launch_conv3(const GemmParams& p, hipStream_t st) {
  if (p.M <= 0 || p.N <= 0) return hipSuccess;
  if (!conv_direct_supported(p) || (p.N & 7) || (p.ldw & 63) || p.ldw < 9 * p.cc) return hipErrorInvalidValue;
  const bool up = p.amode == A_CONV3_UP;
  if (up && upconv_eligible(p)) return p.emode == E_HEAD ? launch_upconv<E_HEAD>(p, st) : launch_upconv<E_STORE>(p, st);
  const bool ck64 = (p.cc % 64) == 0 && p.stride == 1;
  if (p.emode == E_HEAD) {
    if (p.N != 32 || p.stride != 1) return hipErrorInvalidValue;
    if (up) return ck64 ? conv_tiles<64, 1, true, E_HEAD>(p, st) : conv_tiles<32, 1, true, E_HEAD>(p, st);
    return ck64 ? conv_tiles<64, 1, false, E_HEAD>(p, st) : conv_tiles<32, 1, false, E_HEAD>(p, st);
  }
  if (p.emode != E_STORE) return hipErrorInvalidValue;
  hipError_t err;
  if (!up && conv64p_launch(p, st, err)) return err;
  if (up) return ck64 ? conv_tiles<64, 1, true, E_STORE>(p, st) : conv_tiles<32, 1, true, E_STORE>(p, st);
  if (p.stride == 2) return conv_tiles<32, 2, false, E_STORE>(p, st);
  return ck64 ? conv_tiles<64, 1, false, E_STORE>(p, st) : conv_tiles<32, 1, false, E_STORE>(p, st);
}

}
```

### monocular_depth_estimation_trt_amd/csrc/engine.hip

```cpp
#include <hip/hip_runtime.h>

#include <algorithm>
#include <cstdio>
#include <cstring>

#include "engine_internal.h"

using namespace mde;

namespace {
thread_local std::string g_err;
}

int mde::fail(int code, const std::string& msg) {
  g_err = msg;
  return code;
}

int mde::hip_fail(hipError_t e, const char* what) {
  g_err = std::string(what) + ": " + hipGetErrorString(e);
  return MDE_ERR_HIP;
}

namespace {
// ... 105 lines not shown
  if (!bad.empty()) {
    delete e;
    return fail(MDE_ERR_FORMAT, bad);
  }
  hipError_t he = hipSetDevice(device);
  if (he != hipSuccess) {
    delete e;
    return hip_fail(he, "hipSetDevice");
  }
  e->wbytes = hd.data_bytes;
  he = hipMalloc(&e->wmem, std::max<size_t>(hd.data_bytes, 256));
  if (he != hipSuccess) {
    delete e;
    return hip_fail(he, "hipMalloc(weights)");
  }
  he = hipMemcpy(e->wmem, data + hd.data_offset, hd.data_bytes, hipMemcpyHostToDevice);
  if (he != hipSuccess) {
    hipFree(e->wmem);
    delete e;
    return hip_fail(he, "hipMemcpy(weights)");
  }
  for (auto& kv : e->t) kv.second.ptr = (uint8_t*)e->wmem + (uintptr_t)kv.second.ptr;
  *out = e;
  return MDE_OK;
}

}

namespace mde {

bool lnfold_off() { return knob(KNOB_LNFOLD) == 0; }

DptMaps plan_dpt_maps(ArenaPlan& a, size_t n, const mde_engine& e) {
  const size_t F = e.F, np = e.np;
  const int* oc = e.cfg.out_channels;
  const size_t s0 = (size_t)(8 * e.ph) * (8 * e.pw), s1 = (size_t)(4 * e.ph) * (4 * e.pw),
               s2 = (size_t)(2 * e.ph) * (2 * e.pw), s3 = np, s4 = (size_t)e.h4 * e.w4;
  const size_t ss[4] = {s1, s2, s3, s4};
  DptMaps m{};
  for (int i = 0; i < 4; ++i) m.pj[i] = a.h(n * np * oc[i]);
  m.l1 = a.h(n * s1 * e.c1p);
  m.l2 = a.h(n * s2 * oc[1]);
  m.l4 = a.h(n * s4 * oc[3]);
  for (int i = 0; i < 4; ++i) m.rn[i] = a.h(n * ss[i] * F);
  m.tb = a.h(n * s1 * F);
  m.sb = a.h(n * s1 * F);
  m.ub = a.h(n * s1 * F);
  m.vb = a.h(n * s1 * F);
  m.p4 = a.h(n * s3 * F);
  m.p3 = a.h(n * s2 * F);
  m.p2 = a.h(n * s1 * F);
  m.c1 = a.h(n * s0 * (F / 2));
  return m;
}

size_t plan_arena_dav2(const mde_engine& e, int B, DAV2Buf* b, uint8_t* base) {
  ArenaPlan a(base);
  const size_t bb = (size_t)B;
  const int D = e.D, F = e.F, np = e.np;
  const int* oc = e.cfg.out_channels;
  const size_t s1 = (size_t)(4 * e.ph) * (4 * e.pw), s2 = (size_t)(2 * e.ph) * (2 * e.pw), s3 = np,
               s4 = (size_t)e.h4 * e.w4;
  const size_t s0 = (size_t)(8 * e.ph) * (8 * e.pw);
  DAV2Buf t{};
  if (e.cfg.enc_f32) {
    const size_t rows = bb * e.T;
    t.X = a.f(rows * D);
    t.P32 = a.f(bb * np * 672);
    t.Hn32 = a.f(rows * D);
    t.Q32 = a.f(bb * e.H * e.Tpad * 64);
    t.K32 = a.f(bb * e.H * e.Tpad * 64);
    t.V32 = a.f(bb * e.H * e.Tpad * 64);
    t.O32 = a.f(rows * D);
    t.Mh32 = a.f(rows * e.cfg.mlp_hidden);
  }
  t.P = e.cfg.enc_f32 ? nullptr : a.h(bb * np * 672);
  if (e.cfg.enc_f32) {
    t.Xh = nullptr;
  } else if (e.cfg.resid_f16) {
    t.X = nullptr;
    t.Xh = a.h(bb * e.T * D);
  } else {
    t.X = a.f(bb * e.T * D);
    t.Xh = nullptr;
  }
  const bool h16enc = !e.cfg.enc_f32;
  t.Hn = h16enc ? a.h(bb * e.T * D) : nullptr;
  const bool fold = h16enc && e.cfg.resid_f16 && D % 128 == 0 && D <= 1024 && e.get("pos.cls.st") && !lnfold_off();
  t.st = fold ? a.f(bb * e.T * (D / 16)) : nullptr;
  t.Q = h16enc ? a.h(bb * e.H * e.Tpad * 64) : nullptr;
  t.K = h16enc ? a.h(bb * e.H * e.Tpad * 64) : nullptr;
  t.Vt = h16enc ? a.h(bb * e.H * e.Tpad * 64) : nullptr;
  t.O = h16enc ? a.h(bb * e.T * D) : nullptr;
  t.Mh = h16enc ? a.h(bb * e.T * e.cfg.mlp_hidden) : nullptr;
  const bool fold_taps = fold && e.get("proj0.wf");
  const size_t ss[4] = {s1, s2, s3, s4};
  if (!e.head_f32) {
    for (int i = 0; i < 4; ++i) t.tap[i] = fold_taps ? nullptr : a.h(bb * np * D);
    t.m = plan_dpt_maps(a, bb, e);
  } else {
    const size_t sout = (size_t)e.cfg.img_h * e.cfg.img_w;
    for (int i = 0; i < 4; ++i) t.tap32[i] = a.f(bb * np * D);
    for (int i = 0; i < 4; ++i) t.pj32[i] = a.f(bb * np * oc[i]);
    t.l1_32 = a.f(bb * s1 * oc[0]);
    t.l2_32 = a.f(bb * s2 * oc[1]);
    t.l4_32 = a.f(bb * s4 * oc[3]);
    for (int i = 0; i < 4; ++i) t.rn32[i] = a.f(bb * ss[i] * F);
    t.tb32 = a.f(bb * s1 * F);
    t.sb32 = a.f(bb * s1 * F);
    t.ub32 = a.f(bb * s1 * F);
    t.vb32 = a.f(bb * s1 * F);
    t.p4_32 = a.f(bb * s3 * F);
    t.p3_32 = a.f(bb * s2 * F);
    t.p2_32 = a.f(bb * s1 * F);
    t.up1_32 = a.f(bb * s0 * F);
    t.c1_32 = a.f(bb * s0 * (F / 2));
    t.up2_32 = a.f(bb * sout * (F / 2));
    t.hid32 = a.f(bb * sout * 32);
  }
  t.ws = h16enc && bb * e.T <= 4096 ? a.f(fc2_ws_floats(bb * e.T, D)) : nullptr;
  const int bsplit = std::min<int>(B, (256 + ((e.T + 127) / 128) * e.H - 1) / (((e.T + 127) / 128) * e.H));
  t.aws_bytes = h16enc && bsplit >= 1 ? attention_split_ws_bytes(bsplit, e.H, e.T) : 0;
  t.aws = t.aws_bytes ? a.f(t.aws_bytes / sizeof(float)) : nullptr;
  t.sws = a.f(kSplitWsAlloc);
  if (b) *b = t;
  return a.off;
}

}

namespace {

size_t plan_arena(const mde_engine& e, int B, mde_context* c, uint8_t* base) {
  if (e.family == FAMILY_DEPTH_PRO) return plan_arena_dp(e, B, c ? &c->d : nullptr, base);
  if (e.family == FAMILY_VGGT) return plan_arena_vggt(e, B, c ? &c->v : nullptr, base);
  return plan_arena_dav2(e, B, c ? &c->b : nullptr, base);
}

}

namespace mde {

bool Runner::dpt_fusion(DptMaps& m, int n, int r, bool relu_res, bool fold_resize, const h16* x0_up, int uh, int uw) {
  const std::string p = "rf" + std::to_string(r);
  const int F = c.e->F, h = dpt_h(r - 1), w = dpt_w(r - 1);
  const h16* x0 = r == 4 ? m.rn[3] : r == 3 ? m.p4 : r == 2 ? m.p3 : m.p2;
  const h16* x1 = r == 4 ? nullptr : m.rn[r - 1];
  h16* dst = r == 4 ? m.p4 : r == 3 ? m.p3 : r == 2 ? m.p2 : nullptr;
  const h16* s = x0;
  if (x1) {
    rcu(p + ".rcu1", x1, x0, m.sb, m.tb, n, h, w, F, relu_res, x0_up, uh, uw);
    s = m.sb;
  }
  rcu(p + ".rcu2", s, nullptr, m.ub, m.tb, n, h, w, F, relu_res);
  GemmParams g = dense(m.ub, F, p + ".out.w", n * h * w, F, F);
  g.emode = E_STORE;
  g.bias = w32(p + ".out.b");
  g.out16 = m.vb;
  g.ldo = F;
  gemm((p + ".out").c_str(), g);
  if (!dst) return false;
  if (fold_resize) return true;
  step((p + ".resize").c_str(), [&] { return launch_resize(m.vb, dst, n, h, w, F, dpt_h(r - 2), dpt_w(r - 2), st); });
  return false;
}

void Runner::dpt_resize_layer(DptMaps& m, int n, int i) {
  const mde_engine& e = *c.e;
  const int* oc = e.cfg.out_channels;
  if (i == 0 || i == 1) {
    const char* wn = i == 0 ? "rs0.w" : "rs1.w";
    GemmParams g = gemm_convt(m.pj[i], n, e.ph, e.pw, oc[i], w16(wn), ldw(wn), oc[i], i == 0 ? 4 : 2,
                              i == 0 ? m.l1 : m.l2, i == 0 ? e.c1p : oc[1]);
    g.bias = w32(i == 0 ? "rs0.b" : "rs1.b");
    gemm(i == 0 ? "reassemble0.convT4" : "reassemble1.convT2", g);
  } else if (i == 3) {
    GemmParams g = conv(m.pj[3], n, e.ph, e.pw, oc[3], "rs3.w", oc[3], 2);
    g.bias = w32("rs3.b");
    g.out16 = m.l4;
    gemm("reassemble3.conv_s2", g);
  }
}

void Runner::dpt_layer_rn(DptMaps& m, int n, int i) {
  const mde_engine& e = *c.e;
  const int* oc = e.cfg.out_channels;
  const h16* lay[4] = {m.l1, m.l2, m.pj[2], m.l4};
  const int cin[4] = {e.c1p, oc[1], oc[2], oc[3]};
  GemmParams g = conv(lay[i], n, dpt_h(i), dpt_w(i), cin[i], "rn" + std::to_string(i + 1) + ".w", e.F, 1);
  g.out16 = m.rn[i];
  gemm(("layer" + std::to_string(i + 1) + "_rn").c_str(), g);
}

void Runner::dpt_head_conv1(DptMaps& m, int n) {
  const int F = c.e->F, h = dpt_h(0), w = dpt_w(0);
  GemmParams g = gemm_conv3_up(m.vb, n, h, w, F, 2 * h, 2 * w, w16("head.c1.w"), ldw("head.c1.w"), F / 2);
  g.bias = w32("head.c1.b");
  g.out16 = m.c1;
  g.ldo = F / 2;
  gemm("head.output_conv1", g);
}

void Runner::dpt_head_conv2(DptMaps& m, int n, int metric, float max_depth, const h16* hpe, int hpe_pix, float* out) {
  const mde_engine& e = *c.e;
  const int OH = e.cfg.img_h, OW = e.cfg.img_w;
  GemmParams g = gemm_conv3_up(m.c1, n, 2 * dpt_h(0), 2 * dpt_w(0), e.F / 2, OH, OW, w16("head.c2.w"),
                               ldw("head.c2.w"), e.cfg.head_hidden);
  g.bias = w32("head.c2.b");
  set_head(g, w32("head.c3.w"), e.head_b2, metric, max_depth, hpe, hpe_pix, out);
  gemm("head.output_conv2", g);
}

void Runner::vit_block(const VitBlock& b) {
  const mde_engine& e = *c.e;
  const int D = e.D, T = b.T, rows = b.seqs * T, mlp = e.cfg.mlp_hidden;
  const std::string& p = b.w;
  auto name = [&](const char* s) { return b.name + s; };
  const bool fold = b.st != nullptr;
  auto normed = [&](const char* norm, const char* ln, const char* lin, int N) {
    if (fold) {
      GemmParams g = dense(b.Xh, D, p + lin + ".wf", rows, N, D);
      set_ln_consumer(g, b.st, w32(p + lin + ".c1"), w32(p + lin + ".c2"), rows, b.eps);
      return g;
    }
    step(name(norm).c_str(), [&] {
      return launch_layernorm(b.X, b.Hn, w32(p + ln + ".g"), w32(p + ln + ".b"), rows, D, b.eps, T, 0, st, b.Xh);
    });
    GemmParams g = dense(b.Hn, D, p + lin + ".w", rows, N, D);
    g.bias = w32(p + lin + ".b");
    return g;
  };
  {
    GemmParams g = normed("norm1", "ln1", "qkv", 3 * D);
    set_qkv(g, b.Q, b.K, b.Vt, T, b.Tpad, e.H, b.qscale);
    gemm(name("qkv").c_str(), g);
  }
  if (b.after_qkv) b.after_qkv();
  step(name("attn").c_str(),
       [&] { return launch_attention(b.Q, b.K, b.Vt, b.O, b.seqs, e.H, T, b.Tpad, D, st, b.aws, b.aws_bytes); });
  {
    GemmParams g = dense(b.O, D, p + "proj.w", rows, D, D);
    set_resid(g, w32(p + "proj.b"), w32(p + "ls1"), b.X, b.Xh, D);
    if (fold) set_ln_producer(g, b.st, rows);
    gemm(name("proj").c_str(), g);
  }
  {
    GemmParams g = normed("norm2", "ln2", "fc1", mlp);
    g.emode = E_STORE;
    g.act = ACT_GELU;
    g.out16 = b.Mh;
    g.ldo = mlp;
    gemm(name("fc1").c_str(), g);
  }
  {
    GemmParams g = dense(b.Mh, mlp, p + "fc2.w", rows, D, mlp);
    set_resid(g, w32(p + "fc2.b"), w32(p + "ls2"), b.X, b.Xh, D);
    const long long t64 = (long long)((rows + 63) / 64) * ((D + 63) / 64);
    if (b.ws && (size_t)rows <= b.ws_rows && t64 < 512 && mlp >= 1024 && knob(KNOB_SPLITK))
      set_resid_splitk(g, b.ws, t64 < 256 ? 4 : 2, fc2_ws_floats(rows, D), b.counters, kTileCnt);
    if (fold) set_ln_producer(g, b.st, rows);
    gemm(name("fc2").c_str(), g);
  }
}

void Runner::dav2_head32(int B, float* out) {
  mde_engine& e = *c.e;
  const PackConfig& cf = e.cfg;
  const int D = e.D, np = e.np, F = e.F;
  const int* oc = cf.out_channels;
  DAV2Buf& b = c.b;
  const int hs[4] = {4 * e.ph, 2 * e.ph, e.ph, e.h4};
  const int ws[4] = {4 * e.pw, 2 * e.pw, e.pw, e.w4};
  const float* lay[4] = {b.l1_32, b.l2_32, b.pj32[2], b.l4_32};
  char nm[64];
  for (int i = 0; i < 4; ++i) {
    {
      Gemm32Params g = dense32(b.tap32[i], D, "proj" + std::to_string(i) + ".w32", B * np, oc[i], D);
      g.bias = w32("proj" + std::to_string(i) + ".b");
      g.out32 = b.pj32[i];
      g.ldo = oc[i];
      snprintf(nm, sizeof nm, "reassemble%d.project", i);
      gemm32(nm, g);
    }
    if (i == 0 || i == 1) {
      const int sc = i == 0 ? 4 : 2;
      Gemm32Params g = dense32(b.pj32[i], oc[i], i == 0 ? "rs0.w32" : "rs1.w32", B * np, sc * sc * oc[i], oc[i]);
      g.emode = E_CONVT;
      g.bias = w32(i == 0 ? "rs0.b" : "rs1.b");
      g.out32 = i == 0 ? b.l1_32 : b.l2_32;
      g.s = sc;
      g.cout = oc[i];
      g.ldo = oc[i];
      g.cb = B;
      g.ih = e.ph;
      g.iw = e.pw;
      gemm32(i == 0 ? "reassemble0.convT4" : "reassemble1.convT2", g);
    } else if (i == 3) {
      Gemm32Params g = conv32(b.pj32[3], B, e.ph, e.pw, oc[3], "rs3.w32", oc[3], 2);
      g.bias = w32("rs3.b");
      g.out32 = b.l4_32;
      gemm32("reassemble3.conv_s2", g);
    }
    Gemm32Params g = conv32(lay[i], B, hs[i], ws[i], oc[i], "rn" + std::to_string(i + 1) + ".w32", F, 1);
    g.out32 = b.rn32[i];
    snprintf(nm, sizeof nm, "layer%d_rn", i + 1);
    gemm32(nm, g);
  }
  auto fusion = [&](int r, const float* x0, const float* x1, int h, int w, float* dst, int oh, int ow) {
    const std::string p = "rf" + std::to_string(r);
    const float* s = x0;
    if (x1) {
      rcu32(p + ".rcu1", x1, x0, b.sb32, b.tb32, B, h, w, F);
      s = b.sb32;
// ... 716 lines not shown
```

### monocular_depth_estimation_trt_amd/csrc/engine_internal.h

```cpp
#pragma once
#include <hip/hip_runtime.h>

#include <functional>
#include <map>
#include <string>
#include <tuple>
#include <unordered_map>
#include <utility>
#include <vector>

#include "../../include/mde.h"
#include "gemm_params.h"
#include "mde_ops.h"
#include "pack_format.h"
#include "tuning.h"

namespace mde {

struct DevTensor {
  void* ptr = nullptr;
  int dtype = 0;
  int ndim = 0;
  int dims[4] = {0, 0, 0, 0};
};
// ... 129 lines not shown
namespace mde {

struct ArenaPlan {
  uint8_t* base;
  size_t off = 0;
  explicit ArenaPlan(uint8_t* b) : base(b) {}
  void* take(size_t bytes) {
    void* p = base ? (void*)(base + off) : nullptr;
    off += align_up(bytes, 256);
    return p;
  }
  h16* h(size_t elems) { return (h16*)take(elems * 2); }
  float* f(size_t elems) { return (float*)take(elems * 4); }
};

size_t plan_arena_dav2(const mde_engine& e, int B, DAV2Buf* b, uint8_t* base);
size_t plan_arena_dp(const mde_engine& e, int B, DPBuf* b, uint8_t* base);
size_t plan_arena_vggt(const mde_engine& e, int B, VGBuf* b, uint8_t* base);
DptMaps plan_dpt_maps(ArenaPlan& a, size_t n, const mde_engine& e);
std::string setup_depth_pro(mde_engine* e);
std::string setup_vggt(mde_engine* e);

struct VitBlock {
  std::string w;
  std::string name;
  int seqs = 0, T = 0, Tpad = 0;
  float eps = 1e-6f, qscale = kQScale;
  float* X = nullptr;
  h16* Xh = nullptr;
  h16 *Hn = nullptr, *Q = nullptr, *K = nullptr, *Vt = nullptr, *O = nullptr, *Mh = nullptr;
  float* st = nullptr;
  float* aws = nullptr;
  size_t aws_bytes = 0;
  float* ws = nullptr;
  size_t ws_rows = 0;
  int* counters = nullptr;
  std::function<void()> after_qkv;
};

struct Runner {
  mde_context& c;
  hipStream_t st;
  bool prof;
  hipError_t err = hipSuccess;

  template <class Fn>
  void step(const char* name, Fn&& fn) {
    if (err != hipSuccess) return;
    hipEvent_t e0 = nullptr, e1 = nullptr;
    if (prof) {
      if (c.prof_used >= c.prof_events.size()) {
        hipEvent_t a, b;
        if ((err = hipEventCreate(&a)) != hipSuccess) return;
        if ((err = hipEventCreate(&b)) != hipSuccess) return;
        c.prof_events.push_back({std::string(), {a, b}});
      }
      auto& slot = c.prof_events[c.prof_used++];
      slot.first = name;
      e0 = slot.second.first;
      e1 = slot.second.second;
      if ((err = hipEventRecord(e0, st)) != hipSuccess) return;
    }
    err = fn();
    if (err == hipSuccess && prof) err = hipEventRecord(e1, st);
  }

  const DevTensor& W(const std::string& n) { return *c.e->get(n); }
  const h16* w16(const std::string& n) { return (const h16*)W(n).ptr; }
  const float* w32(const std::string& n) { return (const float*)W(n).ptr; }
  const float* w32_opt(const std::string& n) {
    const DevTensor* t = c.e->get(n);
    return t ? (const float*)t->ptr : nullptr;
  }
  int ldw(const std::string& n) { return W(n).dims[W(n).ndim - 1]; }

  GemmParams dense(const h16* A, int lda, const std::string& w, int M, int N, int K) {
    return gemm_dense(A, lda, w16(w), ldw(w), M, N, K);
  }

  GemmParams conv(const h16* in, int B, int h, int w, int cin, const std::string& wn, int cout, int stride) {
    return gemm_conv3(in, B, h, w, cin, w16(wn), ldw(wn), cout, stride);
  }

  GemmParams convt2(const h16* in, int B, int h, int w, int cin, const std::string& wn, int cout, h16* out,
                    int ldo) {
    return gemm_convt(in, B, h, w, cin, w16(wn), ldw(wn), cout, 2, out, ldo);
  }

  float* split_ws = nullptr;

  Gemm32Params dense32(const float* A, int lda, const std::string& w, int M, int N, int K) {
    Gemm32Params g;
    g.A = A;
    g.lda = lda;
    g.W = w32(w);
    g.ldw = ldw(w);
    g.M = M;
    g.N = N;
    g.K = K;
    return g;
  }
  void gemm32(const char* name, const Gemm32Params& g) {
    step(name, [&] { return launch_gemm32(g, st); });
  }
  Gemm32Params conv32(const float* in, int B, int h, int w, int cin, const std::string& wn, int cout, int stride) {
    Gemm32Params g;
    g.amode = A_CONV3;
    g.emode = E_STORE;
    g.A = in;
    g.cb = B;
    g.ch = h;
    g.cw = w;
    g.cc = cin;
    g.stride = stride;
    g.oh = (h - 1) / stride + 1;
    g.ow = (w - 1) / stride + 1;
    g.W = w32(wn);
    g.ldw = ldw(wn);
    g.M = B * g.oh * g.ow;
    g.N = cout;
    g.K = 9 * cin;
    g.ldo = cout;
    return g;
  }
  void rcu32(const std::string& pfx, const float* x, const float* extra, float* out, float* tmp, int B, int h, int w,
             int F) {
    Gemm32Params g1 = conv32(x, B, h, w, F, pfx + ".c1.w32", F, 1);
    g1.relu_in = 1;
    g1.bias = w32_opt(pfx + ".c1.b");
    g1.act = ACT_RELU;
    g1.out32 = tmp;
    gemm32((pfx + ".c1").c_str(), g1);
    Gemm32Params g2 = conv32(tmp, B, h, w, F, pfx + ".c2.w32", F, 1);
    g2.bias = w32_opt(pfx + ".c2.b");
    g2.res0 = x;
    g2.res1 = extra;
    g2.out32 = out;
    gemm32((pfx + ".c2").c_str(), g2);
  }
  void dav2_head32(int B, float* out);

  void gemm(const char* name, const GemmParams& g) {
    GemmParams q = g;
    if (split_ws && g.emode == E_STORE && !g.partial) {
      q.partial = split_ws;
      q.partial_cap = kSplitWsFloats;
      q.slot_cap = kSplitSlotFloats;
      q.tile_cnt = split_counters(split_ws);
      q.tile_cnt_cap = kTileCnt;
    }
    step(name, [&] { return launch_gemm(q, st); });
  }

  void rcu(const std::string& pfx, const h16* x, const h16* extra, h16* out, h16* tmp, int B, int h, int w, int F,
           bool relu_res = false, const h16* extra_up = nullptr, int uh = 0, int uw = 0) {
    GemmParams g1 = conv(x, B, h, w, F, pfx + ".c1.w", F, 1);
    g1.relu_in = 1;
    g1.bias = w32_opt(pfx + ".c1.b");
    g1.act = ACT_RELU;
    g1.out16 = tmp;
    gemm((pfx + ".c1").c_str(), g1);
    GemmParams g2 = conv(tmp, B, h, w, F, pfx + ".c2.w", F, 1);
    g2.bias = w32_opt(pfx + ".c2.b");
    g2.res0 = x;
    g2.res0_relu = relu_res ? 1 : 0;
    g2.res1 = extra;
    g2.res1_up = extra_up;
    g2.res1_uh = uh;
    g2.res1_uw = uw;
    g2.out16 = out;
    gemm((pfx + ".c2").c_str(), g2);
  }

  void vit_block(const VitBlock& b);

  int dpt_h(int i) const { return i == 0 ? 4 * c.e->ph : i == 1 ? 2 * c.e->ph : i == 2 ? c.e->ph : c.e->h4; }
  int dpt_w(int i) const { return i == 0 ? 4 * c.e->pw : i == 1 ? 2 * c.e->pw : i == 2 ? c.e->pw : c.e->w4; }
  void dpt_resize_layer(DptMaps& m, int n, int i);
  void dpt_layer_rn(DptMaps& m, int n, int i);
  bool dpt_fusion(DptMaps& m, int n, int r, bool relu_res, bool fold_resize, const h16* x0_up = nullptr, int uh = 0,
                  int uw = 0);
  void dpt_head_conv1(DptMaps& m, int n);
  void dpt_head_conv2(DptMaps& m, int n, int metric, float max_depth, const h16* hpe, int hpe_pix, float* out);

  hipError_t forward_dav2(int B, const void* img, float* out);
  hipError_t forward_dp(int B, const float* img, float* out, float* fov);
  void dp_encoder(const std::string& pfx, float* X, const h16* P, int nseq, int hook_seqs);
  hipError_t forward_vggt(int B, const float* img, float* out);
};

int fail(int code, const std::string& msg);
int hip_fail(hipError_t e, const char* what);

}
```

### monocular_depth_estimation_trt_amd/csrc/gemm.hip

```cpp
#include <cstdlib>
#include <cstring>
#include <type_traits>
#include <utility>

#include "gemm_route.h"
#include "mde_device.h"
#include "mde_ops.h"
#include "tile_epilogue.h"
#include "tuning.h"

#ifndef MDE_GEMM_BK
#define MDE_GEMM_BK 64
#endif
#ifndef MDE_XCD_REMAP
#define MDE_XCD_REMAP 1
#endif
#ifndef MDE_EPI_LDS
#define MDE_EPI_LDS 1
#endif
#ifndef MDE_BK32_STAGES
#define MDE_BK32_STAGES 3
#endif
#ifndef MDE_GEMM_STAGES
#define MDE_GEMM_STAGES 2
// ... 435 lines not shown
  bool staged = false;
  if constexpr (EPI_LDS) {
    if constexpr (SG > 2) lds_barrier();
    const int m0w = m0 + wm * TM * 16;
    staged = store_tile_lds<EM, TM, TN, STG_HALF>(
        p, acc, [&](int row) { return m0w + row < p.M ? m0w + row : -1; }, n0 + wn * TN * 16, lane,
        smem + wave * (TM * 16) * (TN * 16) * (STG_HALF ? 2 : 4));
  }
  if (!staged) store_tile<EM, TM, TN>(p, acc, mrow, n0 + wn * TN * 16 + (lane >> 4) * 4, lane, slice);
}


struct TileCfg {
  int bm, bn, wm, wn, bk, stg, modes[3], fsplit[2];
};
enum : int { mS = 1 << E_STORE, mQ = 1 << E_QKV, mR = 1 << E_RESID, mP = 1 << E_PATCH, mC = 1 << E_CONVT,
             mH = 1 << E_HEAD, mX = 1 << E_PARTIAL, mAll = mS | mQ | mR | mP | mC };
enum Tile : int { T128x32, T128x64, T64, T64_DEEP, T32x64_DEEP, T128, T128_BK32, T128_W8, T256x128_BK32, T_COUNT };
constexpr TileCfg kTiles[T_COUNT] = {
    {128, 32, 4, 1, MDE_GEMM_BK, 0, {mS, mS, mS | mH}, {0, 0}},
    {128, 64, 4, 1, MDE_GEMM_BK, 0, {mS | mR, mS, mS}, {0, 0}},
    {64, 64, 2, 2, MDE_GEMM_BK, 0, {mAll | mX, mS | mX, mS}, {mS | mR, mS}},
    {64, 64, 2, 2, MDE_GEMM_BK, 4, {mAll | mX, mX, 0}, {mS | mR, mS}},
    {32, 64, 2, 2, 64, 4, {mR, 0, 0}, {0, 0}},
    {128, 128, 2, 2, MDE_GEMM_BK, 0, {mAll | mX, mS, mS}, {mR, 0}},
    {128, 128, 2, 2, 32, 0, {mS | mQ | mP | mC, 0, 0}, {0, 0}},
    {128, 128, 2, 4, MDE_GEMM_BK, 0, {mS | mQ | mX, 0, 0}, {mR, 0}},
    {256, 128, 4, 2, 32, 0, {mR, 0, 0}, {0, 0}},
};
constexpr int ring_stages(const TileCfg& c) { return c.stg ? c.stg : (c.bk == 32 ? MDE_BK32_STAGES : MDE_GEMM_STAGES); }
constexpr bool tile_has(int t, int am, int em, bool split) {
  if (t < 0 || t >= T_COUNT || am < 0 || am > (split ? A_CONV3 : A_CONV3_UP) || em < 0 || em > E_PARTIAL) return false;
  return ((split ? kTiles[t].fsplit[am] : kTiles[t].modes[am]) >> em) & 1;
}

long long tiles(int M, int N, int bm, int bn) { return (long long)((M + bm - 1) / bm) * ((N + bn - 1) / bn); }

int even_slices(int nk, int S) {
  const int per = (nk + S - 1) / S;
  return (nk + per - 1) / per;
}

constexpr int kBk32Kmax = 768;
constexpr long long kBigTileMin = 240;

bool deep64(long long wgs) { return knob(KNOB_DEEP64) && wgs <= 512; }

bool w8small(long long wgs) { return knob(KNOB_W8SMALL) && wgs < 512; }

bool narrow_resid(const GemmParams& p) {
  if (!knob(KNOB_NARROW_RESID) || p.amode != A_DENSE || p.emode != E_RESID) return false;
  const long long t32 = tiles(p.M, p.N, 32, 64);
  return tiles(p.M, p.N, 64, 64) < 256 && t32 >= 192 && t32 <= 512;
}

Tile pick_tile(const GemmParams& p) {
  const int em = p.emode;
  const bool dense = p.amode == A_DENSE;
  if (em == E_HEAD) return T128x32;
  if (em == E_STORE) {
    if (p.N <= 32) return T128x32;
    if (p.N <= 64) return p.M >= 128 * 256 ? T128x64 : T64;
  }
  const long long big = tiles(p.M, p.N, 128, 128);
  if (dense && em == E_RESID) {
    if (tiles(p.M, p.N, 256, 128) >= 512) return T256x128_BK32;
    if (p.K <= 384 && big >= kBigTileMin) return T128x64;
    if (narrow_resid(p)) return T32x64_DEEP;
  }
  if (big >= kBigTileMin) {
    if (dense && em != E_RESID && p.K <= kBk32Kmax) return T128_BK32;
    return dense && (em == E_STORE || em == E_QKV) && w8small(big) ? T128_W8 : T128;
  }
  return dense && deep64(tiles(p.M, p.N, 64, 64)) ? T64_DEEP : T64;
}

bool prefer_im2col(const GemmParams& p) {
  if (p.amode != A_CONV3 || p.emode != E_STORE) return false;
  if (p.stride == 2) return true;
  const double tiles = (double)((p.oh + 7) / 8 * 8) * (double)((p.ow + 15) / 16 * 16);
  return p.cc >= 256 && (double)p.oh * p.ow < 0.6 * tiles;
}

long long unsplit_wgs_estimate(const GemmParams& p) {
  if (p.amode == A_CONV3 && conv_direct_supported(p) && !prefer_im2col(p)) {
    const int bn = p.N <= 32 ? 32 : (p.N <= 64 ? 64 : 128);
    return (long long)p.cb * ((p.oh + 7) / 8) * ((p.ow + 15) / 16) * ((p.N + bn - 1) / bn);
  }
  const long long big = tiles(p.M, p.N, 128, 128);
  return big >= kBigTileMin ? big : tiles(p.M, p.N, 64, 64);
}

int store_split_slices(const GemmParams& p) {
  if (p.emode != E_STORE || !p.partial || p.partial_cap == 0 || p.lnst_in || p.lnst_out) return 1;
  if (p.amode != A_DENSE && p.amode != A_CONV3) return 1;
  if (p.amode == A_CONV3 && p.stride != 1 && p.stride != 2) return 1;
  if (!knob(KNOB_SPLITK)) return 1;
  const int nk = (p.K + 63) / 64;
  const long long t64 = tiles(p.M, p.N, 64, 64);
  const long long wgs = unsplit_wgs_estimate(p);
  if (nk < 12) return 1;
  int S;
  if (wgs >= 256) {
    if (wgs >= 384 || nk < 48) return 1;
    S = 2;
  } else {
    S = (int)((512 + t64 - 1) / t64);
    if (512 / t64 >= 2) S = (int)(512 / t64);
  }
  S = S < nk / 4 ? S : nk / 4;
  S = S < 16 ? S : 16;
  while (S > 1 && (size_t)S * p.M * p.N > p.partial_cap) --S;
  return S <= 1 ? 1 : even_slices(nk, S);
}

bool fused_split(const GemmParams& p, long long tiles, int S, int BM, int BN) {
  return knob(KNOB_SPLITK_FUSED) && p.tile_cnt && tiles <= p.tile_cnt_cap &&
         (size_t)S * (size_t)tiles * (size_t)BM * BN <= p.slot_cap && ((uintptr_t)p.partial & 15) == 0;
}

bool lnst_valid(const GemmParams& p) {
  if (p.lnst_out && !MDE_EPI_LDS) return false;
  return !((p.lnst_ns * 32 != (p.lnst_out ? p.N : p.K)) ||
           (p.lnst_in && (p.lnst_ns > 32 || (p.lnst_ns & 3) ||
                          p.lnst_rows != (p.a_tok > 1 ? p.M / (p.a_tok - 1) * p.a_tok : p.M) ||
                          (p.a_tok > 1 && p.M % (p.a_tok - 1)))) ||
           (p.lnst_out && p.lnst_rows < (p.emode == E_PATCH ? p.M / p.npatch * p.T : p.M)) ||
           (p.lnst_in && (!p.lnc1 || p.amode != A_DENSE)) || (p.lnst_out && !p.xh));
}

GemmRoute tile_route(int kind, Tile t, int slices, bool fused) {
  const TileCfg& c = kTiles[t];
  return {kind, c.bm, c.bn, c.wm, c.wn, c.bk, ring_stages(c), slices, fused, 0};
}

GemmRoute split_resid_route(const GemmParams& p) {
  const int nk = (p.K + 63) / 64;
  const long long t128 = tiles(p.M, p.N, 128, 128), t64 = tiles(p.M, p.N, 64, 64);
  const bool big = t128 * 4 >= 320 && nk >= 16;
  int S = big ? 4 : (p.splitk < nk ? p.splitk : nk);
  while (!big && S > 2 && t64 * S > 512) --S;
  S = even_slices(nk, S);
  const Tile t = big ? (w8small(t128 * S) ? T128_W8 : T128) : (deep64(t64 * S) ? T64_DEEP : T64);
  return tile_route(ROUTE_SPLIT_RESID, t, S, fused_split(p, big ? t128 : t64, S, kTiles[t].bm, kTiles[t].bn));
}

thread_local GemmRoute t_last_route;

}

hipError_t gemm_route(const GemmParams& p, GemmRoute& r) {
  const auto take = [&r](const GemmRoute& x) { r = x; return hipSuccess; };
  if (p.M <= 0 || p.N <= 0) return take({ROUTE_NONE});
  if (p.res1_up) {
    if (!p.res1 || p.amode != A_CONV3 || p.emode != E_STORE || p.res1_uh <= 0 || p.res1_uw <= 0 || (p.N & 7))
      return hipErrorInvalidValue;
    if (store_split_slices(p) <= 1 && !prefer_im2col(p) && conv3_takes_res1_up(p)) return take({ROUTE_CONV_DIRECT});
    GemmParams q = p;
    q.res1_up = nullptr;
    const hipError_t e = gemm_route(q, r);
    r.resize_first = 1;
    return e;
  }
  if (p.K <= 0 || (p.K & 7) || (p.N & 7) || (p.ldw & 63) || p.ldw < ((p.K + 63) / 64) * 64)
    return hipErrorInvalidValue;
  if (p.amode == A_DENSE && ((p.lda & 7) || p.lda < p.K)) return hipErrorInvalidValue;
  if (p.a_tok == 1 || p.a_tok < 0 || (p.a_tok > 1 && (p.amode != A_DENSE || p.emode != E_STORE || !p.lnst_in)))
    return hipErrorInvalidValue;
  if (p.amode != A_DENSE && (p.cc & 7)) return hipErrorInvalidValue;
  if ((p.emode == E_STORE || p.emode == E_RESID || p.emode == E_PATCH) && (p.ldo & 7)) return hipErrorInvalidValue;
  if (p.emode == E_CONVT && ((p.cout & 7) || (p.ldo & 7) || p.ldo < p.cout || ((uintptr_t)p.out16 & 15)))
    return hipErrorInvalidValue;
  if (p.emode == E_HEAD && (p.N != 32 || p.amode == A_DENSE)) return hipErrorInvalidValue;
  if (const int S = store_split_slices(p); S > 1) {
    if ((p.ldo & 7) || ((uintptr_t)p.partial & 15)) return hipErrorInvalidValue;
    const long long t64 = tiles(p.M, p.N, 64, 64);
    return take(tile_route(ROUTE_SPLIT_STORE, deep64(t64 * S) ? T64_DEEP : T64, S, fused_split(p, t64, S, 64, 64)));
  }
  if (p.amode != A_DENSE && conv_direct_supported(p) && !prefer_im2col(p)) return take({ROUTE_CONV_DIRECT});
  if ((p.emode == E_RESID || p.emode == E_PATCH) && p.xh && ((uintptr_t)p.xh & 15)) return hipErrorInvalidValue;
  if (p.emode == E_RESID && p.splitk > 1 && p.partial && p.amode == A_DENSE && !narrow_resid(p))
    return take(split_resid_route(p));
  const bool lnfold = p.lnst_out || p.lnst_in;
  if (lnfold && !lnst_valid(p)) return hipErrorInvalidValue;
  if (panel_gemm_eligible(p)) return take({ROUTE_PANEL});
  if (!lnfold && gemm256_eligible(p)) return take({ROUTE_GEMM256});
  const Tile t = pick_tile(p);
  if (p.emode == E_PARTIAL || !tile_has(t, p.amode, p.emode, false)) return hipErrorInvalidValue;
  return take(tile_route(ROUTE_TILE, t, 1, false));
}

const GemmRoute& gemm_last_route() { return t_last_route; }

namespace {

template <int N, class F>
hipError_t with_constant(int x, F&& f) {
  if constexpr (N == 0) return hipErrorInvalidValue;
  else return x == N - 1 ? f(std::integral_constant<int, N - 1>{}) : with_constant<N - 1>(x, f);
}

hipError_t launch_tiles(const GemmRoute& r, const GemmParams& p, bool fused, hipStream_t st) {
  int t = 0;
  for (const TileCfg& c : kTiles) {
    if (c.bm == r.bm && c.bn == r.bn && c.wm == r.wm && c.wn == r.wn && c.bk == r.bk && ring_stages(c) == r.stages) break;
    ++t;
  }
  const dim3 grid((unsigned)tiles(p.M, p.N, r.bm, r.bn), (unsigned)r.slices);
  return with_constant<T_COUNT>(t, [&](auto T) {
    return with_constant<A_CONV3_UP + 1>(p.amode, [&](auto AM) {
      return with_constant<E_PARTIAL + 1>(p.emode, [&](auto EM) {
        return with_constant<2>(fused, [&](auto FUSED) {
          constexpr int am = decltype(AM)::value, em = decltype(EM)::value, fs = decltype(FUSED)::value;
          if constexpr (tile_has(decltype(T)::value, am, em, fs)) {
            constexpr TileCfg c = kTiles[decltype(T)::value];
            hipLaunchKernelGGL((gemm_kernel<c.bm, c.bn, c.bk, c.wm, c.wn, am, em, c.stg, fs != 0>), grid,
                               dim3(c.wm * c.wn * 64), 0, st, p);
            return hipGetLastError();
          } else {
            return hipErrorInvalidValue;
          }
        });
      });
    });
  });
}

hipError_t launch_split(const GemmRoute& r, const GemmParams& p, hipStream_t st) {
  if (r.fused) return launch_tiles(r, p, true, st);
  GemmParams q = p;
  q.emode = E_PARTIAL, q.x32 = p.partial, q.ldo = p.N;
  q.bias = q.ls = nullptr, q.lnst_out = nullptr;
  const hipError_t e = launch_tiles(r, q, false, st);
  if (e != hipSuccess) return e;
  if (r.kind == ROUTE_SPLIT_STORE) return launch_splitk_store(p.partial, r.slices, p, st);
  return launch_splitk_resid(p.partial, r.slices, p.M, p.N, p.bias, p.ls, p.x32, p.xh, p.ldo, st, p.lnst_out);
}

}

hipError_t launch_gemm(const GemmParams& p, hipStream_t st) {
  GemmRoute r;
  hipError_t e = gemm_route(p, r);
  if (e != hipSuccess) return e;
  t_last_route = r;
  GemmParams q = p;
  if (r.resize_first) {
    e = launch_resize(p.res1_up, const_cast<h16*>(p.res1), p.cb, p.res1_uh, p.res1_uw, p.N, p.oh, p.ow, st);
    if (e != hipSuccess) return e;
    q.res1_up = nullptr;
  }
  switch (r.kind) {
    case ROUTE_NONE: return hipSuccess;
    case ROUTE_TILE: return launch_tiles(r, q, false, st);
    case ROUTE_SPLIT_STORE:
    case ROUTE_SPLIT_RESID: return launch_split(r, q, st);
    case ROUTE_CONV_DIRECT:
      if (q.res1_up) q.res1 = nullptr;
      return launch_conv3(q, st);
    case ROUTE_PANEL: return launch_panel_gemm(q, st);
    case ROUTE_GEMM256: return launch_gemm256(q, st);
    default: return hipErrorInvalidValue;
  }
}

}
```

### monocular_depth_estimation_trt_amd/csrc/mde_device.h

```cpp
#pragma once
#include <hip/hip_runtime.h>
#include <stdint.h>

namespace mde {

typedef _Float16 f16;
typedef f16 f16x8 __attribute__((ext_vector_type(8)));
typedef f16 f16x4 __attribute__((ext_vector_type(4)));
typedef float f32x4 __attribute__((ext_vector_type(4)));

#define MDE_DEV __device__ __forceinline__

MDE_DEV f32x4 mfma16x16x32(const f16x8& a, const f16x8& b, const f32x4& c) {
  return __builtin_amdgcn_mfma_f32_16x16x32_f16(a, b, c, 0, 0, 0);
}

MDE_DEV float wave_sum(float v) {
#pragma unroll
  for (int o = 32; o >= 1; o >>= 1) v += __shfl_xor(v, o, 64);
  return v;
}

MDE_DEV float gelu_erf(float x) {
  const float xc = __builtin_amdgcn_fmed3f(x, -8.f, 8.f);
  const float x2 = xc * xc;
  const float z = xc * fmaf(fmaf(0.001014263055f, x2, -0.106775724f), x2, -2.301121339f);
  return x * __builtin_amdgcn_rcpf(1.f + __builtin_amdgcn_exp2f(z));
}

typedef float f32x2 __attribute__((ext_vector_type(2)));
MDE_DEV f32x2 gelu_erf2(f32x2 x) {
  const f32x2 xc = {__builtin_amdgcn_fmed3f(x[0], -8.f, 8.f), __builtin_amdgcn_fmed3f(x[1], -8.f, 8.f)};
  const f32x2 x2 = xc * xc;
  const f32x2 c = {0.001014263055f, 0.001014263055f}, b = {-0.106775724f, -0.106775724f},
              a = {-2.301121339f, -2.301121339f};
  const f32x2 z = xc * __builtin_elementwise_fma(__builtin_elementwise_fma(c, x2, b), x2, a);
  const f32x2 d = {1.f + __builtin_amdgcn_exp2f(z[0]), 1.f + __builtin_amdgcn_exp2f(z[1])};
  const f32x2 r = {__builtin_amdgcn_rcpf(d[0]), __builtin_amdgcn_rcpf(d[1])};
  return x * r;
}

MDE_DEV void ln_merge_stats(const float2 (&t)[8], int kp, float invd, float& mean, float& var) {
#pragma clang fp contract(off)
  float s1 = 0.f;
#pragma unroll
  for (int k = 0; k < 8; ++k) s1 = s1 + (k < kp ? t[k].x : 0.f);
  s1 = s1 + __shfl_xor(s1, 16);
  s1 = s1 + __shfl_xor(s1, 32);
  mean = s1 * invd;
  float m2 = 0.f;
#pragma unroll
  for (int k = 0; k < 8; ++k) {
    const float d = t[k].x * (1.f / 32.f) - mean;
    m2 = m2 + (k < kp ? t[k].y + (32.f * d) * d : 0.f);
  }
  m2 = m2 + __shfl_xor(m2, 16);
  m2 = m2 + __shfl_xor(m2, 32);
  var = m2 * invd;
}

MDE_DEV float ac_scale(int in_size, int out_size) {
#pragma clang fp contract(off)
  return out_size > 1 ? (float)(in_size - 1) / (float)(out_size - 1) : 0.f;
}

MDE_DEV void ac_index(float scale, int dst, int in_size, int& i0, int& i1, float& l0, float& l1) {
#pragma clang fp contract(off)
  const float f = scale * (float)dst;
  i0 = (int)f;
  i1 = i0 + (i0 < in_size - 1 ? 1 : 0);
  l1 = f - (float)i0;
  l0 = 1.f - l1;
}

typedef f16 f16x2u __attribute__((ext_vector_type(2)));
MDE_DEV f16x8 upsample8(const f16* __restrict__ in, int b, int ih, int iw, int C, int oh, int ow, int oy, int ox,
                        int c0) {
  int y0, y1, x0, x1;
  float ly0, ly1, lx0, lx1;
  ac_index(ac_scale(ih, oh), oy, ih, y0, y1, ly0, ly1);
  ac_index(ac_scale(iw, ow), ox, iw, x0, x1, lx0, lx1);
  (void)lx0;
  (void)ly0;
  const f16* base = in + (size_t)b * ih * iw * C + c0;
  const f16x8 a = *reinterpret_cast<const f16x8*>(base + ((size_t)y0 * iw + x0) * C);
  const f16x8 bb = *reinterpret_cast<const f16x8*>(base + ((size_t)y0 * iw + x1) * C);
  const f16x8 c = *reinterpret_cast<const f16x8*>(base + ((size_t)y1 * iw + x0) * C);
  const f16x8 d = *reinterpret_cast<const f16x8*>(base + ((size_t)y1 * iw + x1) * C);
  const f16x2u wx1 = {(f16)lx1, (f16)lx1}, wy1 = {(f16)ly1, (f16)ly1};
  f16x8 v;
#pragma unroll
  for (int j = 0; j < 8; j += 2) {
    const f16x2u a2 = {a[j], a[j + 1]}, b2 = {bb[j], bb[j + 1]}, c2 = {c[j], c[j + 1]}, d2 = {d[j], d[j + 1]};
    const f16x2u t0 = a2 + (b2 - a2) * wx1, t1 = c2 + (d2 - c2) * wx1;
    const f16x2u r = t0 + (t1 - t0) * wy1;
    v[j] = r[0];
    v[j + 1] = r[1];
  }
  return v;
}

MDE_DEV int vt_pos(int t) { return (t & ~12) | ((t & 4) << 1) | ((t & 8) >> 1); }

MDE_DEV int xcd_remap(int bid, int nwg) {
  const int q8 = nwg / 8, r8 = nwg % 8, x = bid % 8;
  return (x < r8 ? x * (q8 + 1) : r8 * (q8 + 1) + (x - r8) * q8) + bid / 8;
}

MDE_DEV void tile_of(int bid, int ntm, int ntn, int gm, int& tm, int& tn) {
  if (gm <= 1) {
    tm = bid / ntn;
    tn = bid - tm * ntn;
    return;
  }
  const int per = gm * ntn;
  const int g = bid / per, r = bid - g * per;
  const int mb = g * gm;
  const int gs = ntm - mb < gm ? ntm - mb : gm;
  tn = r / gs;
  tm = mb + (r - tn * gs);
}

MDE_DEV int tile_group_m(int n, int k, int bm) {
  if ((long long)n * k * 2 <= (2ll << 20)) return 1;
  const long long per = (long long)bm * k * 2;
  if (per >= (1ll << 20)) return 1;
  const int g = (int)((2ll << 20) / per);
  return g < 1 ? 1 : (g > 8 ? 8 : g);
}

MDE_DEV f16x8 zero8() {
  f16x8 z;
#pragma unroll
  for (int i = 0; i < 8; ++i) z[i] = (f16)0.0f;
  return z;
}

MDE_DEV f16x8 relu8(f16x8 v) {
#pragma unroll
  for (int i = 0; i < 8; ++i) v[i] = v[i] > (f16)0.0f ? v[i] : (f16)0.0f;
  return v;
}

}
```

### monocular_depth_estimation_trt_amd/csrc/mde_ops.h

```cpp
#pragma once
#include <hip/hip_runtime.h>
#include <stdint.h>

namespace mde {

typedef _Float16 h16;

enum AMode : int {
  A_DENSE = 0,
  A_CONV3 = 1,
  A_CONV3_UP = 2
};

enum EMode : int {
  E_STORE = 0,
  E_QKV = 1,
  E_RESID = 2,
  E_PATCH = 3,
  E_CONVT = 4,
  E_HEAD = 5,
  E_PARTIAL = 6
};

enum Act : int { ACT_NONE = 0, ACT_RELU = 1, ACT_GELU = 2 };

struct GemmParams {
  int amode = A_DENSE, emode = E_STORE;
  int M = 0, N = 0, K = 0;
  const h16* A = nullptr; int lda = 0;
  const h16* W = nullptr; int ldw = 0;
  int cb = 0, ch = 0, cw = 0, cc = 0;
  int uh = 0, uw = 0;
  int oh = 0, ow = 0, stride = 1;
  int relu_in = 0;
  const float* bias = nullptr; int act = ACT_NONE;
  h16* out16 = nullptr; int ldo = 0;
  const h16* res0 = nullptr; const h16* res1 = nullptr;
  int res0_relu = 0; int res0_rows = 0;
  const h16* res1_up = nullptr; int res1_uh = 0, res1_uw = 0;
  float* x32 = nullptr; const float* ls = nullptr;
  h16* xh = nullptr;
  h16 *q = nullptr, *k = nullptr, *vt = nullptr;
  int T = 0, Tpad = 0, heads = 0; float qscale = 1.0f;
  const float* pos = nullptr; int npatch = 0; int tok0 = 1;
  int s = 0, cout = 0, ih = 0, iw = 0;
  const float* w2 = nullptr; float b2 = 0.f; int head_metric = 1; float max_depth = 1.f;
  float* out32 = nullptr;
  const h16* hpe = nullptr; int hpe_pix = 0;
  int splitk = 1; float* partial = nullptr;
  size_t partial_cap = 0;
  int* tile_cnt = nullptr; int tile_cnt_cap = 0; size_t slot_cap = 0;
  float* lnst_out = nullptr;
  const float* lnst_in = nullptr; const float* lnc1 = nullptr;
  int lnst_ns = 0, lnst_rows = 0; float ln_eps = 1e-6f;
  int a_tok = 0;
};

struct Gemm32Params {
  int emode = E_STORE;
  int amode = A_DENSE;
  int M = 0, N = 0, K = 0;
  const float* A = nullptr; int lda = 0;
  const float* W = nullptr; int ldw = 0;
  const float* bias = nullptr; int act = ACT_NONE;
  float* out32 = nullptr; h16* out16 = nullptr; int ldo = 0;
  float* x32 = nullptr; const float* ls = nullptr;
  float *q = nullptr, *k = nullptr, *v = nullptr; int T = 0, Tpad = 0, heads = 0; float qscale = 1.f;
  const float* pos = nullptr; int npatch = 0;
  int cb = 0, ch = 0, cw = 0, cc = 0, stride = 1, oh = 0, ow = 0, relu_in = 0;
  const float* res0 = nullptr; const float* res1 = nullptr;
  int s = 0, cout = 0, ih = 0, iw = 0;
};
hipError_t launch_gemm32(const Gemm32Params& p, hipStream_t st);
hipError_t launch_resize32(const float* in, float* out, int B, int ih, int iw, int C, int oh, int ow, hipStream_t st);
hipError_t launch_head32(const float* hid, const float* w2, float b2, int M, int metric, float max_depth, float* out,
                         hipStream_t st);
hipError_t launch_attention32(const float* q, const float* k, const float* v, float* o, int B, int H, int T,
                              int Tpad, int ldo, hipStream_t st);


hipError_t launch_splitk_resid(const float* P, int S, int M, int N, const float* bias, const float* ls, float* x32,
                               h16* xh, int ldo, hipStream_t st, float* lnst_out = nullptr);

hipError_t launch_splitk_store(const float* P, int S, const GemmParams& p, hipStream_t st);

hipError_t launch_gemm(const GemmParams& p, hipStream_t st);

bool conv_direct_supported(const GemmParams& p);
bool conv3_takes_res1_up(const GemmParams& p);
hipError_t launch_conv3(const GemmParams& p, hipStream_t st);

bool panel_gemm_eligible(const GemmParams& p);
int cu_count();
hipError_t launch_panel_gemm(const GemmParams& p, hipStream_t st);

bool gemm256_eligible(const GemmParams& p);
hipError_t launch_gemm256(const GemmParams& p, hipStream_t st);

hipError_t launch_attention(const h16* q, const h16* k, const h16* vt, h16* o, int B, int H, int T,
                            int Tpad, int ldo, hipStream_t st, float* ws = nullptr, size_t ws_bytes = 0,
                            const char* cfg = nullptr);
size_t attention_split_ws_bytes(int B, int H, int T);

hipError_t launch_layernorm(const float* x, h16* y, const float* g, const float* b, int rows, int D,
                            float eps, int T, int skip_cls, hipStream_t st, const h16* xh = nullptr);

hipError_t launch_patch_prep_u8(const unsigned char* img, h16* P, float* X, const float* cls_pos, int B, int H, int W,
                                int ph, int pw, int T, int D, float scale, const float* mean3, const float* std3,
                                hipStream_t st, h16* Xh = nullptr, float* lnst = nullptr,
                                const float* cls_st = nullptr, float* P32 = nullptr);
hipError_t launch_depth_postprocess(const float* in, int B, int ih, int iw, float* out, int oh, int ow, float lo,
                                    float hi, hipStream_t st);
hipError_t launch_resize_u8(const unsigned char* src, int B, int sh, int sw, int pitch, int swap_rb, const float* lut,
                            void* dst, int oh, int ow, hipStream_t st);
hipError_t launch_dp_preprocess(const unsigned char* src, int B, int sh, int sw, int pitch, int swap_rb,
                                const float* lut, float* dst, int oh, int ow, hipStream_t st);
hipError_t launch_dp_postprocess(const float* inv, int B, int ih, int iw, const float* fov_deg, float f_px,
                                 float* f_px_out, float* out, int oh, int ow, hipStream_t st);
size_t point_cloud_ws_bytes(int B, int h, int w, int step);
hipError_t launch_point_cloud(const float* depth, int B, int h, int w, int step, const unsigned char* photo, int pitch,
                              int swap_rb, const float* f_px_dev, float fx, float fy, float cx, float cy, int compact,
                              float z_lo, float z_hi, void* records, int* counts, void* ws, hipStream_t st);
size_t depth_eval_ws_bytes(int B, int h, int w);
hipError_t launch_depth_eval(const float* pred, const float* gt, const unsigned char* mask, int B, int h, int w,
                             int policy, int pred_is_inverse, int fit_finite_only, float max_depth, double* out,
                             void* ws, hipStream_t st);
hipError_t launch_patch_prep(const float* img, h16* P, float* X, const float* cls_pos, int B, int H,
                             int W, int ph, int pw, int T, int D, hipStream_t st, h16* Xh = nullptr,
                             float* lnst = nullptr, const float* cls_st = nullptr, float* P32 = nullptr);
hipError_t launch_layernorm32(const float* x, float* y, const float* g, const float* b, int rows, int D, float eps,
                              hipStream_t st, int T = 1, int skip_cls = 0);

hipError_t launch_resize(const h16* in, h16* out, int B, int ih, int iw, int C, int oh, int ow,
                         hipStream_t st);

struct DpPyramid {
  int nlev = 0, nseq = 0;
  int first[3] = {0, 0, 0}, n[3] = {0, 0, 0}, stride[3] = {0, 0, 0}, f[3] = {1, 1, 1};
};
struct DpMerge {
  int B = 0, n = 1, G = 0, pad = 0, base = 0, T = 0;
};
hipError_t launch_dp_patch_prep(const float* img, h16* P, int B, int S, int G, const DpPyramid& pyr,
                                hipStream_t st);
hipError_t launch_cls_rows(float* X, const float* cls, int nseq, int T, int D, hipStream_t st);
hipError_t launch_merge_tokens(const float* x, h16* y, const float* g, const float* b, int D, const DpMerge& m,
                               float eps, hipStream_t st);
hipError_t launch_fov_final(const h16* in, const float* w, float bias, int K, int B, float* out, hipStream_t st);

struct RopeGeom {
  int T = 0, Tpad = 0, P = 1, npre = 0, gw = 1;
  float qscale = 1.f, eps = 1e-5f;
};
hipError_t launch_prefix_rows(float* X, const float* pre, int nseq, int T, int npre, int D, int frames, int sets,
                              hipStream_t st);
hipError_t launch_rows_layernorm(float* X, const float* g, const float* b, int nseq, int T, int row0, int D, float eps,
                                 hipStream_t st);
hipError_t launch_qk_norm_rope(h16* q, h16* k, const float* qg, const float* qb, const float* kg, const float* kb,
                               const float* rope_cos, const float* rope_sin, int BH, const RopeGeom& geo,
                               hipStream_t st);
hipError_t launch_tap_concat_ln(const float* xa, const float* xb, h16* y, const float* g, const float* b, int nseq,
                                int T, int npre, int D, float eps, hipStream_t st);

}
```

### monocular_depth_estimation_trt_amd/csrc/ops_abi.hip

```cpp
#include <hip/hip_runtime.h>

#include <cstdio>
#include <string>

#include "engine_internal.h"
#include "gemm_route.h"

using namespace mde;

extern "C" {

static int op_status(hipError_t e, const char* what) {
  if (e == hipErrorInvalidValue) return fail(MDE_ERR_ARG, std::string(what) + ": invalid shape/argument");
  if (e != hipSuccess) return hip_fail(e, what);
  return MDE_OK;
}
#define OP_RET(call, what) return op_status((call), what)

int mde_debug_last_gemm_route(char* buf, size_t n) {
  static const char* const kKind[] = {"none", "tile", "split_store", "split_resid", "conv_direct", "panel", "gemm256"};
  const GemmRoute& r = gemm_last_route();
  if (!buf) return fail(MDE_ERR_ARG, "mde_debug_last_gemm_route: null buffer");
  int len;
  if (r.kind == ROUTE_TILE || r.kind == ROUTE_SPLIT_STORE || r.kind == ROUTE_SPLIT_RESID)
// ... 112 lines not shown
  if (!why && compact) {
    if (!(z_lo <= z_hi)) why = "z_lo > z_hi (or NaN)";
    else if (!ws || ws_bytes < point_cloud_ws_bytes(batch, h, w, step))
      why = "compact mode needs ws of mde_op_point_cloud_ws_bytes()";
  }
  if (why) return fail(MDE_ERR_ARG, std::string("mde_op_point_cloud: ") + why);
  OP_RET(launch_point_cloud(depth, batch, h, w, step, photo, pitch, swap_rb, f_px_dev, fx, fy, cx, cy, compact, z_lo,
                            z_hi, records, counts, ws, (hipStream_t)st),
         "mde_op_point_cloud");
}

namespace {
const char* depth_eval_geometry_error(int batch, int h, int w) {
  if (batch < 1 || h < 1 || w < 1) return "batch and sizes must be positive";
  if ((long long)h * w >= 0x80000000LL - 256) return "a plane of 2^31 - 256 pixels or more";
  if (batch > 65535) return "batch > 65535";
  return nullptr;
}
}

size_t mde_op_depth_eval_ws_bytes(int batch, int h, int w) {
  if (depth_eval_geometry_error(batch, h, w)) return 0;
  return depth_eval_ws_bytes(batch, h, w);
}

int mde_op_depth_eval(const float* pred, const float* gt, const unsigned char* mask, int batch, int h, int w,
                      int policy, int pred_is_inverse, int fit_finite_only, float max_depth, double* out, void* ws,
                      size_t ws_bytes, void* st) {
  const char* why = (!pred || !gt || !mask || !out) ? "null pointer" : depth_eval_geometry_error(batch, h, w);
  if (!why && (policy < 0 || policy > 2)) why = "policy must be 0 (none), 1 (scale) or 2 (scale_shift)";
  if (!why && !(max_depth == max_depth)) why = "max_depth is NaN";
  if (!why && (!ws || ws_bytes < depth_eval_ws_bytes(batch, h, w)))
    why = "needs ws of mde_op_depth_eval_ws_bytes()";
  if (!why && ((reinterpret_cast<uintptr_t>(ws) | reinterpret_cast<uintptr_t>(out)) & 7))
    why = "out and ws must be 8-byte aligned";
  if (why) return fail(MDE_ERR_ARG, std::string("mde_op_depth_eval: ") + why);
  OP_RET(launch_depth_eval(pred, gt, mask, batch, h, w, policy, pred_is_inverse != 0, fit_finite_only != 0, max_depth,
                           out, ws, (hipStream_t)st),
         "mde_op_depth_eval");
}

int mde_op_dp_pyramid_patches(const float* img, int batch, int size, void* patches, void* st) {
  if (!img || !patches || batch < 1 || size != 1536) return fail(MDE_ERR_ARG, "mde_op_dp_pyramid_patches: bad argument");
  DpPyramid pyr;
  pyr.nlev = 3;
  const int f[3] = {1, 2, 4}, n[3] = {5, 3, 1}, stride[3] = {288, 192, 384};
  int first = 0;
  for (int i = 0; i < 3; ++i) {
    pyr.first[i] = first;
    pyr.n[i] = n[i];
    pyr.stride[i] = stride[i];
    pyr.f[i] = f[i];
    first += n[i] * n[i];
  }
  pyr.nseq = first;
  OP_RET(launch_dp_patch_prep(img, (h16*)patches, batch, size, 24, pyr, (hipStream_t)st), "dp_pyramid_patches");
}

int mde_op_merge_tokens(const float* x32, int batch, int tokens, int dim, int n, int g, int pad, int base,
                        const float* gamma, const float* beta, float eps, void* out, void* st) {
  if (!x32 || !out || batch < 1 || (gamma == nullptr) != (beta == nullptr))
    return fail(MDE_ERR_ARG, "mde_op_merge_tokens: bad argument");
  DpMerge m;
  m.B = batch;
  m.n = n;
  m.G = g;
  m.pad = pad;
  m.base = base;
  m.T = tokens;
  OP_RET(launch_merge_tokens(x32, (h16*)out, gamma, beta, dim, m, eps, (hipStream_t)st), "merge_tokens");
}

int mde_op_qk_norm_rope(void* q, void* k, const float* qg, const float* qb, const float* kg, const float* kb, int bh,
                        int tokens, int tokens_pad, int frame_tokens, int npre, int grid_w, const float* rope_cos,
                        const float* rope_sin, float q_scale, float eps, void* st) {
  if (!q || !k || !qg || !qb || !kg || !kb || !rope_cos || !rope_sin) return fail(MDE_ERR_ARG, "null argument");
  RopeGeom geo;
  geo.T = tokens;
  geo.Tpad = tokens_pad;
  geo.P = frame_tokens;
  geo.npre = npre;
  geo.gw = grid_w;
  geo.qscale = q_scale;
  geo.eps = eps;
  OP_RET(launch_qk_norm_rope((h16*)q, (h16*)k, qg, qb, kg, kb, rope_cos, rope_sin, bh, geo, (hipStream_t)st),
         "qk_norm_rope");
}

int mde_op_tap_concat_ln(const float* xa, const float* xb, int nseq, int tokens, int npre, int dim, const float* g,
                         const float* b, float eps, void* out, void* st) {
  if (!xa || !xb || !g || !b || !out || nseq < 0) return fail(MDE_ERR_ARG, "null argument");
  OP_RET(launch_tap_concat_ln(xa, xb, (h16*)out, g, b, nseq, tokens, npre, dim, eps, (hipStream_t)st),
         "tap_concat_ln");
}

int mde_op_layernorm_f16(const void* x, void* y, const float* g, const float* b, int rows, int dim, float eps,
                         int tokens, int skip_cls, void* st) {
  if (!x || !y || !g || !b) return fail(MDE_ERR_ARG, "null argument");
  if (skip_cls && tokens < 2) return fail(MDE_ERR_ARG, "skip_cls needs tokens >= 2");
  OP_RET(launch_layernorm(nullptr, (h16*)y, g, b, rows, dim, eps, tokens > 0 ? tokens : 1, skip_cls, (hipStream_t)st,
                          (const h16*)x),
         "layernorm_f16");
}

int mde_op_layernorm(const float* x, void* y, const float* g, const float* b, int rows, int dim, float eps,
                     int tokens, int skip_cls, void* st) {
  if (!x || !y || !g || !b) return fail(MDE_ERR_ARG, "null argument");
  if (skip_cls && tokens < 2) return fail(MDE_ERR_ARG, "skip_cls needs tokens >= 2");
  OP_RET(launch_layernorm(x, (h16*)y, g, b, rows, dim, eps, tokens > 0 ? tokens : 1, skip_cls, (hipStream_t)st),
         "layernorm");
}

namespace {
const char* fused_split_error(const float* ws, size_t ws_floats, const int* tile_cnt, int tile_cnt_cap,
                              size_t slot_floats, int m, int n) {
  if (!tile_cnt) return nullptr;
  if (!ws || slot_floats > ws_floats) return "fused split-K: slot_floats exceeds the workspace";
  const long long t64 = (long long)((m + 63) / 64) * ((n + 63) / 64);
  if (tile_cnt_cap < t64) return "fused split-K: fewer counters than 64^2 tiles";
  return nullptr;
}

void set_store_split(GemmParams& g, float* ws, size_t ws_floats, int* slices, int* tile_cnt, int tile_cnt_cap,
                     size_t slot_floats) {
  g.partial = ws;
  g.partial_cap = ws_floats;
  g.tile_cnt = tile_cnt;
  g.tile_cnt_cap = tile_cnt_cap;
  g.slot_cap = slot_floats;
  if (slices) *slices = gemm_store_split_slices(g);
}

int linear_store(const char* what, const void* a, int lda, const void* wt, int ldw, int m, int n, int k,
                 const float* bias, int act, const void* res0, int res0_rows, int res0_relu, const void* res1,
                 void* out, int ldo, float* ws, size_t ws_floats, int* slices, int* tile_cnt, int tile_cnt_cap,
                 size_t slot_floats, void* st) {
  if (!a || !wt || !out || (!ws && ws_floats)) return fail(MDE_ERR_ARG, "null argument");
  if (res0_rows < 0 || ((res0_rows > 0 || res0_relu) && !res0)) return fail(MDE_ERR_ARG, "res0 options without res0");
  if (const char* why = fused_split_error(ws, ws_floats, tile_cnt, tile_cnt_cap, slot_floats, m, n))
    return fail(MDE_ERR_ARG, why);
  GemmParams g = gemm_dense((const h16*)a, lda, (const h16*)wt, ldw, m, n, k);
  g.bias = bias;
  g.act = act;
  g.res0 = (const h16*)res0;
  g.res0_rows = res0_rows;
  g.res0_relu = res0_relu ? 1 : 0;
  g.res1 = (const h16*)res1;
  g.out16 = (h16*)out;
  g.ldo = ldo;
  set_store_split(g, ws, ws_floats, slices, tile_cnt, tile_cnt_cap, slot_floats);
  return op_status(launch_gemm(g, (hipStream_t)st), what);
}

int conv3x3_store(const char* what, const void* in, int batch, int h, int w, int cin, const void* wt, int ldw,
                  int cout, int stride, int relu_in, const float* bias, int act, const void* res0, int res0_relu,
                  const void* res1, const void* res1_up, int res1_uh, int res1_uw, void* out, float* ws,
                  size_t ws_floats, int* slices, int* tile_cnt, int tile_cnt_cap, size_t slot_floats, void* st) {
  if (!in || !wt || !out || (!ws && ws_floats)) return fail(MDE_ERR_ARG, "null argument");
  if (stride != 1 && stride != 2) return fail(MDE_ERR_ARG, "stride must be 1 or 2");
  if (res0_relu && !res0) return fail(MDE_ERR_ARG, "res0_relu without res0");
  if (res1_up && !res1) return fail(MDE_ERR_ARG, "res1_up needs res1 (a buffer of the output's shape)");
  GemmParams g = gemm_conv3((const h16*)in, batch, h, w, cin, (const h16*)wt, ldw, cout, stride);
  if (const char* why = fused_split_error(ws, ws_floats, tile_cnt, tile_cnt_cap, slot_floats, g.M, g.N))
    return fail(MDE_ERR_ARG, why);
  g.relu_in = relu_in;
  g.bias = bias;
  g.act = act;
  g.res0 = (const h16*)res0;
  g.res0_relu = res0_relu ? 1 : 0;
  g.res1 = (const h16*)res1;
  g.res1_up = (const h16*)res1_up;
  g.res1_uh = res1_uh;
  g.res1_uw = res1_uw;
  g.out16 = (h16*)out;
  set_store_split(g, ws, ws_floats, slices, tile_cnt, tile_cnt_cap, slot_floats);
  return op_status(launch_gemm(g, (hipStream_t)st), what);
}
}

int mde_op_linear(const void* a, int lda, const void* w, int ldw, int m, int n, int k, const float* bias, int act,
                  void* out, int ldo, void* st) {
  return linear_store("linear", a, lda, w, ldw, m, n, k, bias, act, nullptr, 0, 0, nullptr, out, ldo, nullptr, 0,
                      nullptr, nullptr, 0, 0, st);
}

int mde_op_linear_residual(const void* a, int lda, const void* w, int ldw, int m, int n, int k, const float* bias,
                           const float* ls, float* x32, int ldx, void* st) {
  if (!a || !w || !bias || !ls || !x32) return fail(MDE_ERR_ARG, "null argument");
  GemmParams g = gemm_dense((const h16*)a, lda, (const h16*)w, ldw, m, n, k);
  set_resid(g, bias, ls, x32, nullptr, ldx);
  OP_RET(launch_gemm(g, (hipStream_t)st), "linear_residual");
}

static const char* qkv_geometry_error(int batch, int tokens, int heads, int tokens_pad) {
  if (batch <= 0 || tokens <= 0 || heads <= 0) return "batch, tokens and heads must be > 0";
  if (tokens_pad < tokens) return "tokens_pad < tokens";
  if (tokens_pad % 16) return "tokens_pad % 16 != 0 (V^T key permutation works on 16-key groups)";
  return nullptr;
}

int mde_op_qkv(const void* a, const void* w, int ldw, const float* bias, int batch, int tokens, int heads,
               int tokens_pad, float qscale, void* q, void* k, void* vt, void* st) {
  if (!a || !w || !bias || !q || !k || !vt) return fail(MDE_ERR_ARG, "null argument");
  if (const char* why = qkv_geometry_error(batch, tokens, heads, tokens_pad)) return fail(MDE_ERR_ARG, why);
  const int D = heads * 64;
  GemmParams g = gemm_dense((const h16*)a, D, (const h16*)w, ldw, batch * tokens, 3 * D, D);
  g.bias = bias;
  set_qkv(g, (h16*)q, (h16*)k, (h16*)vt, tokens, tokens_pad, heads, qscale);
  OP_RET(launch_gemm(g, (hipStream_t)st), "qkv");
}

int mde_op_linear_residual_f16(const void* a, int lda, const void* w, int ldw, int m, int n, int k, const float* bias,
                               const float* ls, void* xh, int ldx, float* ln_partials, void* st) {
  if (!a || !w || !bias || !ls || !xh) return fail(MDE_ERR_ARG, "null argument");
  if (ln_partials && (n & 31)) return fail(MDE_ERR_ARG, "ln_partials need n % 32 == 0");
  GemmParams g = gemm_dense((const h16*)a, lda, (const h16*)w, ldw, m, n, k);
  set_resid(g, bias, ls, nullptr, (h16*)xh, ldx);
  set_ln_producer(g, ln_partials, m);
  OP_RET(launch_gemm(g, (hipStream_t)st), "linear_residual_f16");
}

namespace {
int linear_lnfold(const char* what, const void* x, const float* ln_partials, float eps, const void* wg, int ldw,
                  const float* c1, const float* c2, int m, int n, int k, int act, void* out, int ldo, int lnst_rows,
                  int a_tok, void* st) {
  GemmParams g = gemm_dense((const h16*)x, k, (const h16*)wg, ldw, m, n, k);
  g.act = act;
  g.out16 = (h16*)out;
  g.ldo = ldo;
  set_ln_consumer(g, ln_partials, c1, c2, lnst_rows, eps);
  g.a_tok = a_tok;
  return op_status(launch_gemm(g, (hipStream_t)st), what);
}
}

int mde_op_linear_lnfold(const void* x, const float* ln_partials, float eps, const void* wg, int ldw, const float* c1,
                         const float* c2, int m, int n, int k, int act, void* out, int ldo, void* st) {
  if (!x || !ln_partials || !wg || !c1 || !c2 || !out) return fail(MDE_ERR_ARG, "null argument");
  if (k & 31) return fail(MDE_ERR_ARG, "k % 32 != 0");
  return linear_lnfold("linear_lnfold", x, ln_partials, eps, wg, ldw, c1, c2, m, n, k, act, out, ldo, m, 0, st);
}

int mde_op_qkv_lnfold(const void* x, const float* ln_partials, float eps, const void* wg, int ldw, const float* c1,
                      const float* c2, int batch, int tokens, int heads, int tokens_pad, float qscale, void* q, void* k,
                      void* vt, void* st) {
  if (!x || !ln_partials || !wg || !c1 || !c2 || !q || !k || !vt) return fail(MDE_ERR_ARG, "null argument");
  if (const char* why = qkv_geometry_error(batch, tokens, heads, tokens_pad)) return fail(MDE_ERR_ARG, why);
  const int D = heads * 64;
  GemmParams g = gemm_dense((const h16*)x, D, (const h16*)wg, ldw, batch * tokens, 3 * D, D);
  set_qkv(g, (h16*)q, (h16*)k, (h16*)vt, tokens, tokens_pad, heads, qscale);
  set_ln_consumer(g, ln_partials, c1, c2, g.M, eps);
  OP_RET(launch_gemm(g, (hipStream_t)st), "qkv_lnfold");
}

int mde_op_attention(const void* q, const void* k, const void* vt, void* o, int batch, int heads, int tokens,
                     int tokens_pad, int ldo, void* st) {
  if (!q || !k || !vt || !o) return fail(MDE_ERR_ARG, "null argument");
  OP_RET(launch_attention((const h16*)q, (const h16*)k, (const h16*)vt, (h16*)o, batch, heads, tokens, tokens_pad,
                          ldo, (hipStream_t)st),
         "attention");
}

int mde_op_attention_ws(const void* q, const void* k, const void* vt, void* o, int batch, int heads, int tokens,
                        int tokens_pad, int ldo, void* ws, size_t ws_bytes, void* st) {
  if (!q || !k || !vt || !o || (!ws && ws_bytes)) return fail(MDE_ERR_ARG, "null argument");
  OP_RET(launch_attention((const h16*)q, (const h16*)k, (const h16*)vt, (h16*)o, batch, heads, tokens, tokens_pad,
                          ldo, (hipStream_t)st, (float*)ws, ws_bytes),
         "attention_ws");
}

int mde_op_attention_cfg(const void* q, const void* k, const void* vt, void* o, int batch, int heads, int tokens,
                         int tokens_pad, int ldo, const char* cfg, void* ws, size_t ws_bytes, void* st) {
  if (!q || !k || !vt || !o || (!ws && ws_bytes)) return fail(MDE_ERR_ARG, "null argument");
  OP_RET(launch_attention((const h16*)q, (const h16*)k, (const h16*)vt, (h16*)o, batch, heads, tokens, tokens_pad,
                          ldo, (hipStream_t)st, (float*)ws, ws_bytes, cfg),
         "attention_cfg");
}

size_t mde_op_attention_ws_bytes(int batch, int heads, int tokens) {
  return batch > 0 && heads > 0 && tokens > 0 ? attention_split_ws_bytes(batch, heads, tokens) : 0;
}

int mde_op_linear32(const float* a, int lda, const float* w, int ldw, int m, int n, int k, const float* bias, int act,
                    float* out, int ldo, void* st) {
  if (!a || !w || !out) return fail(MDE_ERR_ARG, "null argument");
  Gemm32Params g;
  g.A = a;
  g.lda = lda;
  g.W = w;
  g.ldw = ldw;
  g.M = m;
  g.N = n;
  g.K = k;
  g.bias = bias;
  g.act = act;
  g.out32 = out;
  g.ldo = ldo;
  OP_RET(launch_gemm32(g, (hipStream_t)st), "linear32");
}

int mde_op_conv3x3_32(const float* in, int batch, int h, int w, int cin, const float* wt, int ldw, int cout,
                      int stride, int relu_in, const float* bias, int act, const float* res0, const float* res1,
                      float* out, void* st) {
  if (!in || !wt || !out) return fail(MDE_ERR_ARG, "null argument");
  if (stride != 1 && stride != 2) return fail(MDE_ERR_ARG, "stride must be 1 or 2");
  if (batch <= 0 || h <= 0 || w <= 0 || cin <= 0 || cout <= 0) return fail(MDE_ERR_ARG, "bad shape");
  Gemm32Params g;
  g.amode = A_CONV3;
  g.emode = E_STORE;
  g.A = in;
  g.cb = batch;
  g.ch = h;
  g.cw = w;
  g.cc = cin;
  g.stride = stride;
  g.oh = (h - 1) / stride + 1;
  g.ow = (w - 1) / stride + 1;
  g.W = wt;
  g.ldw = ldw;
  g.M = batch * g.oh * g.ow;
  g.N = cout;
  g.K = 9 * cin;
  g.relu_in = relu_in;
  g.bias = bias;
  g.act = act;
  g.res0 = res0;
  g.res1 = res1;
// ... 34 lines not shown
int mde_op_linear_residual32(const float* a, int lda, const float* w, int ldw, int m, int n, int k,
                             const float* bias, const float* ls, float* x32, int ldx, void* st) {
  if (!a || !w || !ls || !x32) return fail(MDE_ERR_ARG, "null argument");
  Gemm32Params g;
  g.emode = E_RESID;
  g.A = a;
  g.lda = lda;
  g.W = w;
  g.ldw = ldw;
  g.M = m;
  g.N = n;
  g.K = k;
  g.bias = bias;
  g.ls = ls;
  g.x32 = x32;
  g.ldo = ldx;
  OP_RET(launch_gemm32(g, (hipStream_t)st), "linear_residual32");
}

int mde_op_qkv32(const float* a, const float* w, int ldw, const float* bias, int batch, int tokens, int heads,
                 int tokens_pad, float q_scale, float* q, float* k, float* v, void* st) {
  if (!a || !w || !q || !k || !v) return fail(MDE_ERR_ARG, "null argument");
  Gemm32Params g;
  g.emode = E_QKV;
  g.A = a;
  g.lda = heads * 64;
  g.W = w;
  g.ldw = ldw;
  g.M = batch * tokens;
  g.N = 3 * heads * 64;
  g.K = heads * 64;
  g.bias = bias;
  g.q = q;
  g.k = k;
  g.v = v;
  g.T = tokens;
  g.Tpad = tokens_pad;
  g.heads = heads;
  g.qscale = q_scale;
  OP_RET(launch_gemm32(g, (hipStream_t)st), "qkv32");
}

int mde_op_attention32(const float* q, const float* k, const float* v, float* o, int batch, int heads, int tokens,
                       int tokens_pad, int ldo, void* st) {
  if (!q || !k || !v || !o) return fail(MDE_ERR_ARG, "null argument");
  OP_RET(launch_attention32(q, k, v, o, batch, heads, tokens, tokens_pad, ldo, (hipStream_t)st), "attention32");
}

int mde_op_patch_embed(const float* img, int batch, int h, int w, const void* wt, int ldw, const float* bias,
                       const float* pos_patch, const float* cls_pos, int dim, void* scratch, float* x32, void* st) {
  if (!img || !wt || !bias || !pos_patch || !cls_pos || !scratch || !x32) return fail(MDE_ERR_ARG, "null argument");
  if (h % 14 || w % 14) return fail(MDE_ERR_ARG, "image size must be a multiple of 14");
  const int ph = h / 14, pw = w / 14, T = ph * pw + 1;
  hipError_t e = launch_patch_prep(img, (h16*)scratch, x32, cls_pos, batch, h, w, ph, pw, T, dim, (hipStream_t)st);
  if (e != hipSuccess) return hip_fail(e, "patch_prep");
  GemmParams g = gemm_dense((const h16*)scratch, 672, (const h16*)wt, ldw, batch * ph * pw, dim, 672);
  g.emode = E_PATCH;
  g.bias = bias;
  g.x32 = x32;
  g.ldo = dim;
  g.T = T;
  g.pos = pos_patch;
  g.npatch = ph * pw;
  OP_RET(launch_gemm(g, (hipStream_t)st), "patch_embed");
}

int mde_op_conv3x3(const void* in, int batch, int h, int w, int cin, const void* wt, int ldw, int cout, int stride,
                   int relu_in, const float* bias, int act, const void* res0, const void* res1, void* out,
                   void* st) {
  return conv3x3_store("conv3x3", in, batch, h, w, cin, wt, ldw, cout, stride, relu_in, bias, act, res0, 0, res1,
                       nullptr, 0, 0, out, nullptr, 0, nullptr, nullptr, 0, 0, st);
}

int mde_op_conv3x3_ws(const void* in, int batch, int h, int w, int cin, const void* wt, int ldw, int cout, int stride,
                      int relu_in, const float* bias, int act, const void* res0, const void* res1, void* out,
                      float* ws, size_t ws_floats, int* slices, void* st) {
  return conv3x3_store("conv3x3_ws", in, batch, h, w, cin, wt, ldw, cout, stride, relu_in, bias, act, res0, 0, res1,
                       nullptr, 0, 0, out, ws, ws_floats, slices, nullptr, 0, 0, st);
}

int mde_op_linear_ws(const void* a, int lda, const void* wt, int ldw, int m, int n, int k, const float* bias, int act,
                     void* out, int ldo, float* ws, size_t ws_floats, int* slices, void* st) {
  return linear_store("linear_ws", a, lda, wt, ldw, m, n, k, bias, act, nullptr, 0, 0, nullptr, out, ldo, ws,
                      ws_floats, slices, nullptr, 0, 0, st);
}

int mde_op_conv3x3_up(const void* in, int batch, int sh, int sw, int cin, int uh, int uw, const void* wt, int ldw,
                      int cout, const float* bias, int act, void* out, void* st) {
  if (!in || !wt || !out) return fail(MDE_ERR_ARG, "null argument");
  GemmParams g = gemm_conv3_up((const h16*)in, batch, sh, sw, cin, uh, uw, (const h16*)wt, ldw, cout);
  g.bias = bias;
  g.act = act;
  g.out16 = (h16*)out;
  g.ldo = cout;
  OP_RET(launch_gemm(g, (hipStream_t)st), "conv3x3_up");
}

namespace {
int conv_transpose(const char* what, const void* in, int batch, int h, int w, int cin, const void* wt, int ldw,
                   int cout, int stride, const float* bias, void* out, int ldo, void* st) {
  if (!in || !wt || !bias || !out) return fail(MDE_ERR_ARG, "null argument");
  GemmParams g = gemm_convt((const h16*)in, batch, h, w, cin, (const h16*)wt, ldw, cout, stride, (h16*)out, ldo);
  g.bias = bias;
  return op_status(launch_gemm(g, (hipStream_t)st), what);
}
}

int mde_op_conv_transpose(const void* in, int batch, int h, int w, int cin, const void* wt, int ldw, int cout,
                          int stride, const float* bias, void* out, void* st) {
  return conv_transpose("conv_transpose", in, batch, h, w, cin, wt, ldw, cout, stride, bias, out, cout, st);
}

int mde_op_resize_bilinear(const void* in, int batch, int ih, int iw, int c, int oh, int ow, void* out, void* st) {
  if (!in || !out) return fail(MDE_ERR_ARG, "null argument");
  OP_RET(launch_resize((const h16*)in, (h16*)out, batch, ih, iw, c, oh, ow, (hipStream_t)st), "resize_bilinear");
}

namespace {
int depth_head(const char* what, const void* in, int batch, int sh, int sw, int cin, int uh, int uw, const void* wt,
               int ldw, const float* bias, const float* w2, float b2, int metric, float max_depth, const void* hpe,
               int hpe_pix, float* out, void* st) {
  if (!in || !wt || !bias || !w2 || !out) return fail(MDE_ERR_ARG, "null argument");
  if (hpe && hpe_pix < 1) return fail(MDE_ERR_ARG, "hpe needs hpe_pix >= 1");
  GemmParams g = gemm_conv3_up((const h16*)in, batch, sh, sw, cin, uh, uw, (const h16*)wt, ldw, 32);
  g.bias = bias;
  set_head(g, w2, b2, metric, max_depth, (const h16*)hpe, hpe ? hpe_pix : 0, out);
  return op_status(launch_gemm(g, (hipStream_t)st), what);
}
}

int mde_op_depth_head(const void* in, int batch, int sh, int sw, int cin, int uh, int uw, const void* wt, int ldw,
                      const float* bias, const float* w2, float b2, int metric, float max_depth, float* out,
                      void* st) {
  return depth_head("depth_head", in, batch, sh, sw, cin, uh, uw, wt, ldw, bias, w2, b2, metric, max_depth, nullptr, 0,
                    out, st);
}

int mde_op_linear_res(const void* a, int lda, const void* wt, int ldw, int m, int n, int k, const float* bias, int act,
                      const void* res0, int res0_rows, int res0_relu, const void* res1, void* out, int ldo, float* ws,
                      size_t ws_floats, int* slices, int* tile_cnt, int tile_cnt_cap, size_t slot_floats, void* st) {
  return linear_store("linear_res", a, lda, wt, ldw, m, n, k, bias, act, res0, res0_rows, res0_relu, res1, out, ldo,
                      ws, ws_floats, slices, tile_cnt, tile_cnt_cap, slot_floats, st);
}

int mde_op_conv3x3_res(const void* in, int batch, int h, int w, int cin, const void* wt, int ldw, int cout, int stride,
                       int relu_in, const float* bias, int act, const void* res0, int res0_relu, const void* res1,
                       const void* res1_up, int res1_uh, int res1_uw, void* out, float* ws, size_t ws_floats,
                       int* slices, int* tile_cnt, int tile_cnt_cap, size_t slot_floats, void* st) {
  return conv3x3_store("conv3x3_res", in, batch, h, w, cin, wt, ldw, cout, stride, relu_in, bias, act, res0, res0_relu,
                       res1, res1_up, res1_uh, res1_uw, out, ws, ws_floats, slices, tile_cnt, tile_cnt_cap,
                       slot_floats, st);
}

int mde_op_linear_lnfold_tok(const void* x, const float* ln_partials, float eps, const void* wg, int ldw,
                             const float* c1, const float* c2, int seqs, int tokens, int n, int k, int act, void* out,
                             int ldo, void* st) {
  if (!x || !ln_partials || !wg || !c1 || !c2 || !out) return fail(MDE_ERR_ARG, "null argument");
  if (k & 31) return fail(MDE_ERR_ARG, "k % 32 != 0");
  if (seqs < 1 || tokens < 2) return fail(MDE_ERR_ARG, "seqs >= 1 and tokens >= 2 (a cls row and at least one more)");
  return linear_lnfold("linear_lnfold_tok", x, ln_partials, eps, wg, ldw, c1, c2, seqs * (tokens - 1), n, k, act, out,
                       ldo, seqs * tokens, tokens, st);
}

int mde_op_depth_head_pe(const void* in, int batch, int sh, int sw, int cin, int uh, int uw, const void* wt, int ldw,
                         const float* bias, const float* w2, float b2, int metric, float max_depth, const void* hpe,
                         int hpe_pix, float* out, void* st) {
  return depth_head("depth_head_pe", in, batch, sh, sw, cin, uh, uw, wt, ldw, bias, w2, b2, metric, max_depth, hpe,
                    hpe_pix, out, st);
}

int mde_op_conv_transpose_ld(const void* in, int batch, int h, int w, int cin, const void* wt, int ldw, int cout,
                             int stride, const float* bias, void* out, int ldo, void* st) {
  return conv_transpose("conv_transpose_ld", in, batch, h, w, cin, wt, ldw, cout, stride, bias, out, ldo, st);
}

int mde_op_linear_residual_split(const void* a, int lda, const void* wt, int ldw, int m, int n, int k,
                                 const float* bias, const float* ls, float* x32, void* xh, int ldx, float* ln_partials,
                                 int splitk, float* ws, size_t ws_floats, int* tile_cnt, int tile_cnt_cap,
                                 size_t slot_floats, void* st) {
  if (!a || !wt || !bias || !ls || (!x32 == !xh) || (!ws && ws_floats))
    return fail(MDE_ERR_ARG, "null argument (one of x32 / xh)");
  if (ln_partials && (!xh || (n & 31))) return fail(MDE_ERR_ARG, "ln_partials need xh and n % 32 == 0");
  if (m < 0 || n < 0 || splitk < 0) return fail(MDE_ERR_ARG, "negative size");
  if (splitk > 1 && (!ws || ws_floats / (size_t)(splitk > 4 ? splitk : 4) < (size_t)m * (size_t)n))
    return fail(MDE_ERR_ARG, "ws must hold max(splitk, 4) * m * n floats");
  if (const char* why = fused_split_error(ws, ws_floats, tile_cnt, tile_cnt_cap, slot_floats, m, n))
    return fail(MDE_ERR_ARG, why);
  GemmParams g = gemm_dense((const h16*)a, lda, (const h16*)wt, ldw, m, n, k);
  set_resid(g, bias, ls, x32, (h16*)xh, ldx);
  if (ln_partials) set_ln_producer(g, ln_partials, m);
  if (splitk > 1) set_resid_splitk(g, ws, splitk, slot_floats, tile_cnt, tile_cnt_cap);
  OP_RET(launch_gemm(g, (hipStream_t)st), "linear_residual_split");
}

}
```

### monocular_depth_estimation_trt_amd/csrc/tuning.h

```cpp
#pragma once

namespace mde {

enum Knob : int {
  KNOB_SPLITK = 0,
  KNOB_LNFOLD,
  KNOB_CONV_NARROW,
  KNOB_UPCONV,
  KNOB_GEMM256,
  KNOB_DEEP64,
  KNOB_W8SMALL,
  KNOB_CONV_PERSIST,
  KNOB_PANEL,
  KNOB_PANEL32,
  KNOB_NARROW_RESID,
  KNOB_ATTN16,
  KNOB_SPLITK_FUSED,
  KNOB_ATTN_TAIL,
  KNOB_RESIZE_FOLD,
  KNOB_COUNT
};

int knob(Knob k);

}
```

### monocular_depth_estimation_trt_amd/csrc/tuning.hip

```cpp
#include <atomic>
#include <cstdio>
#include <cstdlib>
#include <cstring>
#include <mutex>

#include "../../include/mde.h"
#include "tuning.h"

namespace mde {

namespace {

struct KnobDef {
  const char* name;
  const char* env;
  int def;
  int lo, hi;
};

constexpr KnobDef kKnobs[KNOB_COUNT] = {
    {"splitk", "MDE_SPLITK", 1, 0, 1},
    {"lnfold", "MDE_LNFOLD", 1, 0, 1},
    {"conv_narrow", "MDE_CONV_NARROW", 1, 0, 1},
    {"upconv", "MDE_UPCONV", 1, 0, 1},
    {"gemm256", "MDE_GEMM256", 1, 0, 2},
    {"deep64", "MDE_DEEP64", 1, 0, 1},
    {"w8small", "MDE_W8SMALL", 1, 0, 1},
    {"conv_persist", "MDE_CONV_PERSIST", 1, 0, 2},
    {"panel", "MDE_PANEL", 1, 0, 2},
    {"panel32", "MDE_PANEL32", 0, 0, 1},
    {"narrow_resid", "MDE_NARROW_RESID", 1, 0, 1},
    {"attn16", "MDE_ATTN16", 1, 0, 1},
    {"splitk_fused", "MDE_SPLITK_FUSED", 0, 0, 1},
    {"attn_tail", "MDE_ATTN_TAIL", 2, 0, 2},
    {"resize_fold", "MDE_RESIZE_FOLD", 1, 0, 1},
};

std::atomic<int> g_val[KNOB_COUNT];
std::once_flag g_once;

void init_once() {
  std::call_once(g_once, [] {
    for (int i = 0; i < KNOB_COUNT; ++i) {
      int v = kKnobs[i].def;
      if (const char* e = std::getenv(kKnobs[i].env)) {
        char* end = nullptr;
        const long x = std::strtol(e, &end, 10);
        if (end != e && *end == '\0' && x >= kKnobs[i].lo && x <= kKnobs[i].hi)
          v = (int)x;
        else
          std::fprintf(stderr, "[mde] %s=%s ignored (accepted: integer %d..%d); using %d\n", kKnobs[i].env, e,
                       kKnobs[i].lo, kKnobs[i].hi, v);
      }
      g_val[i].store(v, std::memory_order_relaxed);
    }
  });
}

int find(const char* name) {
  if (!name) return -1;
  for (int i = 0; i < KNOB_COUNT; ++i)
    if (std::strcmp(kKnobs[i].name, name) == 0) return i;
  return -1;
}

}

int knob(Knob k) {
  init_once();
  return g_val[k].load(std::memory_order_relaxed);
}

}

extern "C" {

int mde_tuning_set(const char* name, int value) {
  mde::init_once();
  const int i = mde::find(name);
  if (i < 0) return MDE_ERR_NAME;
  if (value < mde::kKnobs[i].lo || value > mde::kKnobs[i].hi) return MDE_ERR_ARG;
  mde::g_val[i].store(value, std::memory_order_relaxed);
  return MDE_OK;
}

int mde_tuning_get(const char* name, int* value) {
  mde::init_once();
  const int i = mde::find(name);
  if (i < 0) return MDE_ERR_NAME;
  if (!value) return MDE_ERR_ARG;
  *value = mde::g_val[i].load(std::memory_order_relaxed);
  return MDE_OK;
}

}
```

Baseline: 5894 images/s.

## Fuse bilinear-upsampled residual and trailing 1x1 conv into persistent conv3x3 kernel

Adds two fusions to the persistent 64-channel conv3x3 kernel, both enabled by a new default-on knob. The upsampled second residual is read as bilinear taps prefetched during the tap loop instead of running a separate path, which lets this conv use the persistent kernel. The fusion block's trailing 1x1 output projection is computed in the conv epilogue from LDS-staged results, removing a separate GEMM launch and a round trip of the intermediate activation through HBM. In exchange the kernel uses more LDS and registers, which could affect occupancy or scheduling.

After: 5943 images/s (median of 6 runs). No clear change (+0.8%).

```diff
diff --git a/include/mde.h b/include/mde.h
--- a/include/mde.h
+++ b/include/mde.h
@@ -162,6 +162,11 @@
                        const void* res1_f16, const void* res1_up_f16, int res1_uh, int res1_uw, void* out_f16,
                        float* ws, size_t ws_floats, int* slices, int* tile_cnt, int tile_cnt_cap, size_t slot_floats,
                        void* stream);
+int mde_op_conv3x3_post(const void* in_f16, int batch, int h, int w, int cin, const void* w_f16, int ldw, int cout,
+                        int stride, int relu_in, const float* bias, int act, const void* res0_f16, int res0_relu,
+                        const void* res1_f16, const void* res1_up_f16, int res1_uh, int res1_uw, void* out_f16,
+                        const void* post_w_f16, int post_ldw, const float* post_bias, void* post_out_f16,
+                        void* stream);
 int mde_op_linear_lnfold_tok(const void* x_f16, const float* ln_partials, float eps, const void* wg_f16, int ldw,
                              const float* c1, const float* c2, int seqs, int tokens, int n, int k, int act,
                              void* out_f16, int ldo, void* stream);
diff --git a/monocular_depth_estimation_trt_amd/_lib.py b/monocular_depth_estimation_trt_amd/_lib.py
--- a/monocular_depth_estimation_trt_amd/_lib.py
+++ b/monocular_depth_estimation_trt_amd/_lib.py
@@ -138,6 +138,9 @@
     "mde_op_conv3x3_res": [c_void_p, c_int, c_int, c_int, c_int, c_void_p, c_int, c_int, c_int, c_int, c_void_p,
                            c_int, c_void_p, c_int, c_void_p, c_void_p, c_int, c_int, c_void_p, c_void_p, c_size_t,
                            P(c_int), c_void_p, c_int, c_size_t, c_void_p],
+    "mde_op_conv3x3_post": [c_void_p, c_int, c_int, c_int, c_int, c_void_p, c_int, c_int, c_int, c_int, c_void_p,
+                            c_int, c_void_p, c_int, c_void_p, c_void_p, c_int, c_int, c_void_p, c_void_p, c_int,
+                            c_void_p, c_void_p, c_void_p],
     "mde_op_linear_lnfold_tok": [c_void_p, c_void_p, c_float, c_void_p, c_int, c_void_p, c_void_p, c_int, c_int,
                                  c_int, c_int, c_int, c_void_p, c_int, c_void_p],
     "mde_op_depth_head_pe": [c_void_p, c_int, c_int, c_int, c_int, c_int, c_int, c_void_p, c_int, c_void_p,
@@ -245,8 +248,8 @@
 
 
 TUNING = ("splitk", "lnfold", "conv_narrow", "upconv", "gemm256", "deep64", "w8small", "conv_persist", "panel",
-          "panel32", "narrow_resid", "attn16", "splitk_fused", "attn_tail", "resize_fold")
-TUNING_DEFAULT = {"panel32": 0, "splitk_fused": 0, "attn_tail": 2}
+          "panel32", "narrow_resid", "attn16", "splitk_fused", "attn_tail", "resize_fold", "convp_fuse")
+TUNING_DEFAULT = {"panel32": 0, "splitk_fused": 0, "attn_tail": 2, "convp_fuse": 3}
 
 
 def get_tuning(name: str) -> int:
diff --git a/monocular_depth_estimation_trt_amd/csrc/conv.hip b/monocular_depth_estimation_trt_amd/csrc/conv.hip
--- a/monocular_depth_estimation_trt_amd/csrc/conv.hip
+++ b/monocular_depth_estimation_trt_amd/csrc/conv.hip
@@ -14,6 +14,9 @@
 #endif
 #ifndef MDE_CONVP_RELU_PASS
 #define MDE_CONVP_RELU_PASS 1
+#endif
+#ifndef MDE_CONVP_RUP_TAP
+#define MDE_CONVP_RUP_TAP 8
 #endif
 #ifndef MDE_CONV_BRES
 #define MDE_CONV_BRES 2
@@ -325,9 +328,11 @@
   }
 }
 
-template <int TYP, int MODE>
+template <int TYP, int MODE, bool RUP = false, bool POST = false>
 __global__ void __launch_bounds__(TYP * 32) __attribute__((amdgpu_waves_per_eu(1)))
 conv64p_kernel(const GemmParams p) {
+  static_assert(!RUP || MODE == 2, "res1_up is the second residual");
+  static_assert(!POST || MODE == 1 || MODE == 2, "the post-1x1 follows a residual epilogue");
   constexpr int NW = TYP / 2, NT = NW * 64, TM = 2, TN = 4;
   constexpr int ROWB = 128, RWP = 8;
   constexpr int PH = TYP + 2, PW = TW + 2, PHW = PH * PW;
@@ -341,7 +346,9 @@
   static_assert(NW * EPIW <= PATCH, "epilogue staging fits the consumed patch buffer");
   static_assert(PATCH + ((TM + 1) * PW + 2) * ROWB < 65536 && 7 * 8192 + 3 * 2048 < 65536, "ds_read immediate offsets");
   static_assert(PW % 8 == 2, "pixel row stride = 2 mod 8 (the swizzle table below)");
-  __shared__ __attribute__((aligned(16))) char smem[2 * PATCH + WB];
+  constexpr int W1OFF = 2 * PATCH + WB, W1LDS = 6;
+  static_assert(!POST || (NW >= W1LDS && W1OFF + W1LDS * 1024 <= 160 * 1024), "the 1x1 weight beside the taps");
+  __shared__ __attribute__((aligned(16))) char smem[2 * PATCH + WB + (POST ? W1LDS * 1024 : 0)];
 
   const int tid = threadIdx.x, lane = tid & 63;
   const int wave = __builtin_amdgcn_readfirstlane(tid >> 6);
@@ -407,9 +414,20 @@
   for (int j = 0; j < TN; ++j)
     bias[j] = p.bias ? *reinterpret_cast<const float4*>(p.bias + j * 16 + (lane >> 4) * 4) : float4{0.f, 0.f, 0.f, 0.f};
 
+  f16x8 w1r[2];
+  if constexpr (POST) {
+    const f16* w1p = reinterpret_cast<const f16*>(p.post_w) + (size_t)(lane & 15) * p.post_ldw + (lane >> 4) * 8;
+    if (wave < W1LDS)
+      *reinterpret_cast<f16x8*>(smem + W1OFF + wave * 1024 + lane * 16) =
+          *reinterpret_cast<const f16x8*>(w1p + (size_t)(wave >> 1) * 16 * p.post_ldw + (wave & 1) * 32);
+#pragma unroll
+    for (int s2 = 0; s2 < 2; ++s2) w1r[s2] = *reinterpret_cast<const f16x8*>(w1p + (size_t)48 * p.post_ldw + s2 * 32);
+  }
+
   load_patch(t, 0, std::false_type{});
   wait_vmc();
   __syncthreads();
+  if constexpr (POST) asm volatile("" : "+v"(w1r[0]), "+v"(w1r[1]));
   if constexpr (MODE == 0) {
     if (MDE_CONVP_RELU_PASS) relu_patch(0);
     lds_sync();
@@ -435,10 +453,19 @@
       for (int it = 0; it < 4; ++it) {
         const size_t o = (size_t)(mo[it] < 0 ? 0 : mo[it]) * p.ldo + c8 * 8;
         res[0][it] = *reinterpret_cast<const f16x8*>(reinterpret_cast<const f16*>(p.res0) + o);
-        if constexpr (NRES > 1) res[1][it] = *reinterpret_cast<const f16x8*>(reinterpret_cast<const f16*>(p.res1) + o);
+        if constexpr (NRES > 1 && !RUP) res[1][it] = *reinterpret_cast<const f16x8*>(reinterpret_cast<const f16*>(p.res1) + o);
       }
     }
     __builtin_amdgcn_sched_barrier(0);
+
+    Up8Taps tp0, tp1;
+    auto load_taps = [&](Up8Taps& t, int it) {
+      const int row = it * 8 + rr;
+      const bool in = mo[it] >= 0;
+      const int oy = in ? ty * TYP + wave * TM + (row >> 4) : 0, ox = in ? tx * TW + (row & 15) : 0;
+      upsample8_taps<unsigned>(t, reinterpret_cast<const f16*>(p.res1_up), b, p.res1_uh, p.res1_uw, 64, Ho, Wo, oy, ox,
+                               c8 * 8);
+    };
 
     f32x4 acc[TM][TN];
 #pragma unroll
@@ -448,6 +475,12 @@
 #pragma unroll
     for (int tap = 0; tap < 9; ++tap) {
       const int ky = tap / 3, kx = tap - (tap / 3) * 3;
+      if constexpr (RUP) {
+        if (tap == MDE_CONVP_RUP_TAP) {
+          load_taps(tp0, 0), load_taps(tp1, 1);
+          __builtin_amdgcn_sched_barrier(0);
+        }
+      }
 #pragma unroll
       for (int s2 = 0; s2 < 2; ++s2) {
         f16x8 fa[TM], fb[TN];
@@ -498,6 +531,11 @@
         if (mo[it] >= 0) *reinterpret_cast<f16x8*>(out + (size_t)mo[it] * p.ldo + c8 * 8) = h;
       }
     } else {
+      if constexpr (RUP && MDE_CONVP_RUP_TAP > 8) {
+        load_taps(tp0, 0), load_taps(tp1, 1);
+        __builtin_amdgcn_sched_barrier(0);
+      }
+      f16x8 fin[POST ? 4 : 1];
 #pragma unroll
       for (int i = 0; i < TM; ++i) {
         if (i > 0) __builtin_amdgcn_wave_barrier();
@@ -510,6 +548,14 @@
         }
         asm volatile("s_waitcnt lgkmcnt(0)" ::: "memory");
         __builtin_amdgcn_wave_barrier();
+        f16x8 up[2];
+        if constexpr (RUP) {
+          up[0] = upsample8_blend(tp0), up[1] = upsample8_blend(tp1);
+          if (i + 1 < TM) {
+            load_taps(tp0, 2 * i + 2), load_taps(tp1, 2 * i + 3);
+            __builtin_amdgcn_sched_barrier(0);
+          }
+        }
 #pragma unroll
         for (int h2 = 0; h2 < 2; ++h2) {
           const int it = i * 2 + h2, row = h2 * 8 + rr;
@@ -525,14 +571,77 @@
             for (int e = 0; e < 8; ++e) v[e] += (float)r0[e];
           }
           if constexpr (NRES > 1) {
-            const f16x8 r1 = res[NRES - 1][it];
+            const f16x8 r1 = RUP ? up[h2] : res[NRES - 1][it];
 #pragma unroll
             for (int e = 0; e < 8; ++e) v[e] += (float)r1[e];
           }
           f16x8 h;
 #pragma unroll
           for (int e = 0; e < 8; ++e) h[e] = (f16)v[e];
-          if (mo[it] >= 0) *reinterpret_cast<f16x8*>(out + (size_t)mo[it] * p.ldo + c8 * 8) = h;
+          if constexpr (POST) fin[it] = h;
+          else if (mo[it] >= 0) *reinterpret_cast<f16x8*>(out + (size_t)mo[it] * p.ldo + c8 * 8) = h;
+        }
+      }
+      if constexpr (POST) {
+        __builtin_amdgcn_wave_barrier();
+#pragma unroll
+        for (int it = 0; it < 4; ++it) {
+          const int row = it * 8 + rr;
+          *reinterpret_cast<f16x8*>(stage + row * 128 + ((c8 ^ (row & 7)) << 4)) = fin[it];
+        }
+        asm volatile("s_waitcnt lgkmcnt(0)" ::: "memory");
+        __builtin_amdgcn_wave_barrier();
+        f16x8 fr[TM][2];
+#pragma unroll
+        for (int i = 0; i < TM; ++i)
+#pragma unroll
+          for (int s2 = 0; s2 < 2; ++s2) {
+            const int row = i * 16 + (lane & 15);
+            fr[i][s2] = *reinterpret_cast<const f16x8*>(stage + row * 128 + (((4 * s2 + (lane >> 4)) ^ (row & 7)) << 4));
+          }
+        f16x8 w1[TN][2];
+#pragma unroll
+        for (int j = 0; j < TN; ++j)
+#pragma unroll
+          for (int s2 = 0; s2 < 2; ++s2)
+            w1[j][s2] = 2 * j + s2 < W1LDS ? *reinterpret_cast<const f16x8*>(smem + W1OFF + (2 * j + s2) * 1024 + lane * 16)
+                                           : w1r[s2];
+        f32x4 acc1[TM][TN];
+#pragma unroll
+        for (int i = 0; i < TM; ++i)
+#pragma unroll
+          for (int j = 0; j < TN; ++j) acc1[i][j] = f32x4{0.f, 0.f, 0.f, 0.f};
+#pragma unroll
+        for (int s2 = 0; s2 < 2; ++s2)
+#pragma unroll
+          for (int i = 0; i < TM; ++i)
+#pragma unroll
+            for (int j = 0; j < TN; ++j) acc1[i][j] = mfma16x16x32(w1[j][s2], fr[i][s2], acc1[i][j]);
+        float4 bias1[TN];
+#pragma unroll
+        for (int j = 0; j < TN; ++j)
+          bias1[j] = p.post_bias ? *reinterpret_cast<const float4*>(p.post_bias + j * 16 + (lane >> 4) * 4)
+                                 : float4{0.f, 0.f, 0.f, 0.f};
+        asm volatile("s_waitcnt lgkmcnt(0)" ::: "memory");
+        __builtin_amdgcn_wave_barrier();
+        f16* const out1 = reinterpret_cast<f16*>(p.post_out);
+#pragma unroll
+        for (int i = 0; i < TM; ++i)
+#pragma unroll
+          for (int j = 0; j < TN; ++j) {
+            const float4 bn = bias1[j];
+            const f16x4 h = {(f16)(acc1[i][j][0] + bn.x), (f16)(acc1[i][j][1] + bn.y), (f16)(acc1[i][j][2] + bn.z),
+                             (f16)(acc1[i][j][3] + bn.w)};
+            const int row = i * 16 + (lane & 15), q = j * 4 + (lane >> 4);
+            *reinterpret_cast<f16x4*>(stage + row * 128 + ((((q >> 1) ^ (row & 7)) << 4) | ((q & 1) << 3))) = h;
+          }
+        asm volatile("s_waitcnt lgkmcnt(0)" ::: "memory");
+        __builtin_amdgcn_wave_barrier();
+#pragma unroll
+        for (int it = 0; it < 4; ++it) {
+          const int row = it * 8 + rr;
+          const f16x8 h = *reinterpret_cast<const f16x8*>(stage + row * 128 + ((c8 ^ (row & 7)) << 4));
+          if (mo[it] >= 0) *reinterpret_cast<f16x8*>(out1 + (size_t)mo[it] * p.ldo + c8 * 8) = h;
         }
       }
     }
@@ -553,32 +662,43 @@
       p.ch != p.oh || p.cw != p.ow || p.ldo < 64 || (p.ldo & 7) || p.res0_rows > 0)
     return -1;
   const bool r1 = p.res1 || p.res1_up;
+  if (p.res1_up && (long long)p.res1_uh * p.res1_uw * 128 >= (1ll << 32)) return -1;
   int m;
   if (p.relu_in && p.act == ACT_RELU && !p.res0 && !r1) m = 0;
   else if (!p.relu_in && p.act == ACT_NONE && !p.res0 && !r1) m = 3;
   else if (!p.relu_in && p.act == ACT_NONE && p.res0) m = r1 ? 2 : 1;
   else return -1;
+  if (p.post_w && (!(knob(KNOB_CONVP_FUSE) & 2) || mode != 1 || (m != 1 && m != 2) || !p.post_out || p.post_ldw < 64 ||
+                   (p.post_ldw & 7) || ((uintptr_t)p.post_w & 15) || ((uintptr_t)p.post_out & 15)))
+    return -1;
   const int typ = mode == 2 ? 8 : 16;
   const long long tiles = (long long)p.cb * ((p.oh + typ - 1) / typ) * ((p.ow + TW - 1) / TW);
   if (tiles < 4 * 256 || tiles >= (1ll << 31)) return -1;
   return m;
 }
 
+template <int TYP>
+void conv64p_launch_typ(int m, const GemmParams& p, hipStream_t st) {
+  const dim3 grid(256), block(TYP * 32);
+  if (m == 0) hipLaunchKernelGGL((conv64p_kernel<TYP, 0>), grid, block, 0, st, p);
+  else if (m == 1) hipLaunchKernelGGL((conv64p_kernel<TYP, 1>), grid, block, 0, st, p);
+  else if (m == 2 && p.res1_up) hipLaunchKernelGGL((conv64p_kernel<TYP, 2, true>), grid, block, 0, st, p);
+  else if (m == 2) hipLaunchKernelGGL((conv64p_kernel<TYP, 2>), grid, block, 0, st, p);
+  else hipLaunchKernelGGL((conv64p_kernel<TYP, 3>), grid, block, 0, st, p);
+}
+
 bool conv64p_launch(const GemmParams& p, hipStream_t st, hipError_t& err) {
   const int m = conv64p_mode(p);
   if (m < 0) return false;
-  const int typ = knob(KNOB_CONV_PERSIST) == 2 ? 8 : 16;
-  const dim3 grid(256), block(typ * 32);
-  if (typ == 16) {
-    if (m == 0) hipLaunchKernelGGL((conv64p_kernel<16, 0>), grid, block, 0, st, p);
-    else if (m == 1) hipLaunchKernelGGL((conv64p_kernel<16, 1>), grid, block, 0, st, p);
-    else if (m == 2) hipLaunchKernelGGL((conv64p_kernel<16, 2>), grid, block, 0, st, p);
-    else hipLaunchKernelGGL((conv64p_kernel<16, 3>), grid, block, 0, st, p);
+  const dim3 grid(256), block(512);
+  if (p.post_w) {
+    if (m == 1) hipLaunchKernelGGL((conv64p_kernel<16, 1, false, true>), grid, block, 0, st, p);
+    else if (p.res1_up) hipLaunchKernelGGL((conv64p_kernel<16, 2, true, true>), grid, block, 0, st, p);
+    else hipLaunchKernelGGL((conv64p_kernel<16, 2, false, true>), grid, block, 0, st, p);
+  } else if (knob(KNOB_CONV_PERSIST) == 2) {
+    conv64p_launch_typ<8>(m, p, st);
   } else {
-    if (m == 0) hipLaunchKernelGGL((conv64p_kernel<8, 0>), grid, block, 0, st, p);
-    else if (m == 1) hipLaunchKernelGGL((conv64p_kernel<8, 1>), grid, block, 0, st, p);
-    else if (m == 2) hipLaunchKernelGGL((conv64p_kernel<8, 2>), grid, block, 0, st, p);
-    else hipLaunchKernelGGL((conv64p_kernel<8, 3>), grid, block, 0, st, p);
+    conv64p_launch_typ<16>(m, p, st);
   }
   err = hipGetLastError();
   return true;
@@ -916,9 +1036,17 @@
 }
 
 bool conv3_takes_res1_up(const GemmParams& p) {
-  return knob(KNOB_RESIZE_FOLD) && p.amode == A_CONV3 && p.emode == E_STORE && p.stride == 1 && p.N <= 64 &&
-         conv_direct_supported(p) && conv64p_mode(p) < 0 && p.ldo == p.N && (p.N & 7) == 0 && p.res1_uh > 0 &&
-         p.res1_uw > 0;
+  if (p.amode != A_CONV3 || p.emode != E_STORE || p.stride != 1 || p.N > 64 || !conv_direct_supported(p) ||
+      p.ldo != p.N || (p.N & 7) || p.res1_uh <= 0 || p.res1_uw <= 0)
+    return false;
+  if (conv64p_mode(p) >= 0) return (knob(KNOB_CONVP_FUSE) & 1) != 0;
+  return knob(KNOB_RESIZE_FOLD) != 0;
+}
+
+bool conv3_takes_post1x1(const GemmParams& p) {
+  if (!(knob(KNOB_CONVP_FUSE) & 2) || knob(KNOB_CONV_PERSIST) != 1) return false;
+  const int m = conv64p_mode(p);
+  return m == 1 || m == 2;
 }
 
 hipError_t launch_conv3(const GemmParams& p, hipStream_t st) {
@@ -935,6 +1063,7 @@
   if (p.emode != E_STORE) return hipErrorInvalidValue;
   hipError_t err;
   if (!up && conv64p_launch(p, st, err)) return err;
+  if (p.post_w) return hipErrorInvalidValue;
   if (up) return ck64 ? conv_tiles<64, 1, true, E_STORE>(p, st) : conv_tiles<32, 1, true, E_STORE>(p, st);
   if (p.stride == 2) return conv_tiles<32, 2, false, E_STORE>(p, st);
   return ck64 ? conv_tiles<64, 1, false, E_STORE>(p, st) : conv_tiles<32, 1, false, E_STORE>(p, st);
diff --git a/monocular_depth_estimation_trt_amd/csrc/engine.hip b/monocular_depth_estimation_trt_amd/csrc/engine.hip
--- a/monocular_depth_estimation_trt_amd/csrc/engine.hip
+++ b/monocular_depth_estimation_trt_amd/csrc/engine.hip
@@ -281,13 +281,14 @@
     rcu(p + ".rcu1", x1, x0, m.sb, m.tb, n, h, w, F, relu_res, x0_up, uh, uw);
     s = m.sb;
   }
-  rcu(p + ".rcu2", s, nullptr, m.ub, m.tb, n, h, w, F, relu_res);
-  GemmParams g = dense(m.ub, F, p + ".out.w", n * h * w, F, F);
-  g.emode = E_STORE;
-  g.bias = w32(p + ".out.b");
-  g.out16 = m.vb;
-  g.ldo = F;
-  gemm((p + ".out").c_str(), g);
+  if (!rcu(p + ".rcu2", s, nullptr, m.ub, m.tb, n, h, w, F, relu_res, nullptr, 0, 0, (p + ".out").c_str(), m.vb)) {
+    GemmParams g = dense(m.ub, F, p + ".out.w", n * h * w, F, F);
+    g.emode = E_STORE;
+    g.bias = w32(p + ".out.b");
+    g.out16 = m.vb;
+    g.ldo = F;
+    gemm((p + ".out").c_str(), g);
+  }
   if (!dst) return false;
   if (fold_resize) return true;
   step((p + ".resize").c_str(), [&] { return launch_resize(m.vb, dst, n, h, w, F, dpt_h(r - 2), dpt_w(r - 2), st); });
diff --git a/monocular_depth_estimation_trt_amd/csrc/engine_internal.h b/monocular_depth_estimation_trt_amd/csrc/engine_internal.h
--- a/monocular_depth_estimation_trt_amd/csrc/engine_internal.h
+++ b/monocular_depth_estimation_trt_amd/csrc/engine_internal.h
@@ -305,8 +305,9 @@
     step(name, [&] { return launch_gemm(q, st); });
   }
 
-  void rcu(const std::string& pfx, const h16* x, const h16* extra, h16* out, h16* tmp, int B, int h, int w, int F,
-           bool relu_res = false, const h16* extra_up = nullptr, int uh = 0, int uw = 0) {
+  bool rcu(const std::string& pfx, const h16* x, const h16* extra, h16* out, h16* tmp, int B, int h, int w, int F,
+           bool relu_res = false, const h16* extra_up = nullptr, int uh = 0, int uw = 0, const char* post = nullptr,
+           h16* post_out = nullptr) {
     GemmParams g1 = conv(x, B, h, w, F, pfx + ".c1.w", F, 1);
     g1.relu_in = 1;
     g1.bias = w32_opt(pfx + ".c1.b");
@@ -322,7 +323,16 @@
     g2.res1_uh = uh;
     g2.res1_uw = uw;
     g2.out16 = out;
+    const bool fused = post && conv3_takes_post1x1(g2);
+    if (fused) {
+      const std::string pw = std::string(post) + ".w";
+      g2.post_w = w16(pw);
+      g2.post_ldw = ldw(pw);
+      g2.post_bias = w32(std::string(post) + ".b");
+      g2.post_out = post_out;
+    }
     gemm((pfx + ".c2").c_str(), g2);
+    return fused;
   }
 
   void vit_block(const VitBlock& b);
diff --git a/monocular_depth_estimation_trt_amd/csrc/gemm.hip b/monocular_depth_estimation_trt_amd/csrc/gemm.hip
--- a/monocular_depth_estimation_trt_amd/csrc/gemm.hip
+++ b/monocular_depth_estimation_trt_amd/csrc/gemm.hip
@@ -611,6 +611,8 @@
 hipError_t gemm_route(const GemmParams& p, GemmRoute& r) {
   const auto take = [&r](const GemmRoute& x) { r = x; return hipSuccess; };
   if (p.M <= 0 || p.N <= 0) return take({ROUTE_NONE});
+  if (p.post_w && (p.amode != A_CONV3 || store_split_slices(p) > 1 || prefer_im2col(p) || !conv3_takes_post1x1(p)))
+    return hipErrorInvalidValue;
   if (p.res1_up) {
     if (!p.res1 || p.amode != A_CONV3 || p.emode != E_STORE || p.res1_uh <= 0 || p.res1_uw <= 0 || (p.N & 7))
       return hipErrorInvalidValue;
diff --git a/monocular_depth_estimation_trt_amd/csrc/mde_device.h b/monocular_depth_estimation_trt_amd/csrc/mde_device.h
--- a/monocular_depth_estimation_trt_amd/csrc/mde_device.h
+++ b/monocular_depth_estimation_trt_amd/csrc/mde_device.h
@@ -74,30 +74,46 @@
 }
 
 typedef f16 f16x2u __attribute__((ext_vector_type(2)));
-MDE_DEV f16x8 upsample8(const f16* __restrict__ in, int b, int ih, int iw, int C, int oh, int ow, int oy, int ox,
-                        int c0) {
+struct Up8Taps {
+  f16x8 a, b, c, d;
+  f16x2u w1;
+};
+template <class Off = size_t>
+MDE_DEV void upsample8_taps(Up8Taps& t, const f16* __restrict__ in, int b, int ih, int iw, int C, int oh, int ow,
+                            int oy, int ox, int c0) {
   int y0, y1, x0, x1;
   float ly0, ly1, lx0, lx1;
   ac_index(ac_scale(ih, oh), oy, ih, y0, y1, ly0, ly1);
   ac_index(ac_scale(iw, ow), ox, iw, x0, x1, lx0, lx1);
   (void)lx0;
   (void)ly0;
-  const f16* base = in + (size_t)b * ih * iw * C + c0;
-  const f16x8 a = *reinterpret_cast<const f16x8*>(base + ((size_t)y0 * iw + x0) * C);
-  const f16x8 bb = *reinterpret_cast<const f16x8*>(base + ((size_t)y0 * iw + x1) * C);
-  const f16x8 c = *reinterpret_cast<const f16x8*>(base + ((size_t)y1 * iw + x0) * C);
-  const f16x8 d = *reinterpret_cast<const f16x8*>(base + ((size_t)y1 * iw + x1) * C);
-  const f16x2u wx1 = {(f16)lx1, (f16)lx1}, wy1 = {(f16)ly1, (f16)ly1};
+  const char* base = reinterpret_cast<const char*>(in + (size_t)b * ih * iw * C);
+  const Off r0 = (Off)y0 * (Off)iw, r1 = (Off)y1 * (Off)iw;
+  t.a = *reinterpret_cast<const f16x8*>(base + ((r0 + (Off)x0) * (Off)C + (Off)c0) * 2);
+  t.b = *reinterpret_cast<const f16x8*>(base + ((r0 + (Off)x1) * (Off)C + (Off)c0) * 2);
+  t.c = *reinterpret_cast<const f16x8*>(base + ((r1 + (Off)x0) * (Off)C + (Off)c0) * 2);
+  t.d = *reinterpret_cast<const f16x8*>(base + ((r1 + (Off)x1) * (Off)C + (Off)c0) * 2);
+  t.w1 = f16x2u{(f16)lx1, (f16)ly1};
+}
+MDE_DEV f16x8 upsample8_blend(const Up8Taps& t) {
+  const f16x2u wx1 = {t.w1[0], t.w1[0]}, wy1 = {t.w1[1], t.w1[1]};
   f16x8 v;
 #pragma unroll
   for (int j = 0; j < 8; j += 2) {
-    const f16x2u a2 = {a[j], a[j + 1]}, b2 = {bb[j], bb[j + 1]}, c2 = {c[j], c[j + 1]}, d2 = {d[j], d[j + 1]};
+    const f16x2u a2 = {t.a[j], t.a[j + 1]}, b2 = {t.b[j], t.b[j + 1]}, c2 = {t.c[j], t.c[j + 1]},
+                 d2 = {t.d[j], t.d[j + 1]};
     const f16x2u t0 = a2 + (b2 - a2) * wx1, t1 = c2 + (d2 - c2) * wx1;
     const f16x2u r = t0 + (t1 - t0) * wy1;
     v[j] = r[0];
     v[j + 1] = r[1];
   }
   return v;
+}
+MDE_DEV f16x8 upsample8(const f16* __restrict__ in, int b, int ih, int iw, int C, int oh, int ow, int oy, int ox,
+                        int c0) {
+  Up8Taps t;
+  upsample8_taps(t, in, b, ih, iw, C, oh, ow, oy, ox, c0);
+  return upsample8_blend(t);
 }
 
 MDE_DEV int vt_pos(int t) { return (t & ~12) | ((t & 4) << 1) | ((t & 8) >> 1); }
diff --git a/monocular_depth_estimation_trt_amd/csrc/mde_ops.h b/monocular_depth_estimation_trt_amd/csrc/mde_ops.h
--- a/monocular_depth_estimation_trt_amd/csrc/mde_ops.h
+++ b/monocular_depth_estimation_trt_amd/csrc/mde_ops.h
@@ -38,6 +38,7 @@
   const h16* res0 = nullptr; const h16* res1 = nullptr;
   int res0_relu = 0; int res0_rows = 0;
   const h16* res1_up = nullptr; int res1_uh = 0, res1_uw = 0;
+  const h16* post_w = nullptr; int post_ldw = 0; const float* post_bias = nullptr; h16* post_out = nullptr;
   float* x32 = nullptr; const float* ls = nullptr;
   h16* xh = nullptr;
   h16 *q = nullptr, *k = nullptr, *vt = nullptr;
@@ -88,6 +89,7 @@
 
 bool conv_direct_supported(const GemmParams& p);
 bool conv3_takes_res1_up(const GemmParams& p);
+bool conv3_takes_post1x1(const GemmParams& p);
 hipError_t launch_conv3(const GemmParams& p, hipStream_t st);
 
 bool panel_gemm_eligible(const GemmParams& p);
diff --git a/monocular_depth_estimation_trt_amd/csrc/ops_abi.hip b/monocular_depth_estimation_trt_amd/csrc/ops_abi.hip
--- a/monocular_depth_estimation_trt_amd/csrc/ops_abi.hip
+++ b/monocular_depth_estimation_trt_amd/csrc/ops_abi.hip
@@ -288,10 +288,15 @@
   return op_status(launch_gemm(g, (hipStream_t)st), what);
 }
 
+struct Post1x1 {
+  const void* w = nullptr; int ldw = 0; const float* bias = nullptr; void* out = nullptr;
+};
+
 int conv3x3_store(const char* what, const void* in, int batch, int h, int w, int cin, const void* wt, int ldw,
                   int cout, int stride, int relu_in, const float* bias, int act, const void* res0, int res0_relu,
                   const void* res1, const void* res1_up, int res1_uh, int res1_uw, void* out, float* ws,
-                  size_t ws_floats, int* slices, int* tile_cnt, int tile_cnt_cap, size_t slot_floats, void* st) {
+                  size_t ws_floats, int* slices, int* tile_cnt, int tile_cnt_cap, size_t slot_floats, void* st,
+                  const Post1x1& post = {}) {
   if (!in || !wt || !out || (!ws && ws_floats)) return fail(MDE_ERR_ARG, "null argument");
   if (stride != 1 && stride != 2) return fail(MDE_ERR_ARG, "stride must be 1 or 2");
   if (res0_relu && !res0) return fail(MDE_ERR_ARG, "res0_relu without res0");
@@ -309,6 +314,10 @@
   g.res1_uh = res1_uh;
   g.res1_uw = res1_uw;
   g.out16 = (h16*)out;
+  g.post_w = (const h16*)post.w;
+  g.post_ldw = post.ldw;
+  g.post_bias = post.bias;
+  g.post_out = (h16*)post.out;
   set_store_split(g, ws, ws_floats, slices, tile_cnt, tile_cnt_cap, slot_floats);
   return op_status(launch_gemm(g, (hipStream_t)st), what);
 }
@@ -649,6 +658,17 @@
                        slot_floats, st);
 }
 
+int mde_op_conv3x3_post(const void* in, int batch, int h, int w, int cin, const void* wt, int ldw, int cout, int stride,
+                        int relu_in, const float* bias, int act, const void* res0, int res0_relu, const void* res1,
+                        const void* res1_up, int res1_uh, int res1_uw, void* out, const void* post_w, int post_ldw,
+                        const float* post_bias, void* post_out, void* st) {
+  if (!post_w || !post_out) return fail(MDE_ERR_ARG, "mde_op_conv3x3_post: null post_w / post_out");
+  Post1x1 post;
+  post.w = post_w, post.ldw = post_ldw, post.bias = post_bias, post.out = post_out;
+  return conv3x3_store("conv3x3_post", in, batch, h, w, cin, wt, ldw, cout, stride, relu_in, bias, act, res0, res0_relu,
+                       res1, res1_up, res1_uh, res1_uw, out, nullptr, 0, nullptr, nullptr, 0, 0, st, post);
+}
+
 int mde_op_linear_lnfold_tok(const void* x, const float* ln_partials, float eps, const void* wg, int ldw,
                              const float* c1, const float* c2, int seqs, int tokens, int n, int k, int act, void* out,
                              int ldo, void* st) {
diff --git a/monocular_depth_estimation_trt_amd/csrc/tuning.h b/monocular_depth_estimation_trt_amd/csrc/tuning.h
--- a/monocular_depth_estimation_trt_amd/csrc/tuning.h
+++ b/monocular_depth_estimation_trt_amd/csrc/tuning.h
@@ -18,6 +18,7 @@
   KNOB_SPLITK_FUSED,
   KNOB_ATTN_TAIL,
   KNOB_RESIZE_FOLD,
+  KNOB_CONVP_FUSE,
   KNOB_COUNT
 };
 
diff --git a/monocular_depth_estimation_trt_amd/csrc/tuning.hip b/monocular_depth_estimation_trt_amd/csrc/tuning.hip
--- a/monocular_depth_estimation_trt_amd/csrc/tuning.hip
+++ b/monocular_depth_estimation_trt_amd/csrc/tuning.hip
@@ -34,6 +34,7 @@
     {"splitk_fused", "MDE_SPLITK_FUSED", 0, 0, 1},
     {"attn_tail", "MDE_ATTN_TAIL", 2, 0, 2},
     {"resize_fold", "MDE_RESIZE_FOLD", 1, 0, 1},
+    {"convp_fuse", "MDE_CONVP_FUSE", 3, 0, 3},
 };
 
 std::atomic<int> g_val[KNOB_COUNT];
```
